# NoelShin/PixelPick

Hardware: AMD Instinct MI355X
Metric: train_step_throughput (higher is better)
Workload: dtype f32; 1 GPU; BASELINE configs[1]: Cityscapes 256x512, C=19, DeepLabv3+-MobileNetV2; train step per-GPU batch 4 with 20 labelled px/img + Adam; acquisition entropy top-k=20, B=256 images/launch/GPU, NCHW fp32 logits; global_batch=4

## Files before the change

### include/pixelpick_hip.h

```cpp
#ifndef PIXELPICK_HIP_H
#define PIXELPICK_HIP_H

#include <stddef.h>
#include <stdint.h>

#ifdef __cplusplus
extern "C" {
#endif

typedef void* pp_stream_t;

enum {
    PP_OK = 0,
    PP_ERR_BAD_ARG = -1,
    PP_ERR_BAD_K = -2,
    PP_ERR_WORKSPACE = -3,
    PP_ERR_UNSUPPORTED = -4,
    PP_ERR_LAUNCH = -5
};

enum { PP_ACQ_ENTROPY = 0, PP_ACQ_LEAST_CONFIDENCE = 1, PP_ACQ_MARGIN = 2 };
enum { PP_ACQ_BALD = 3 };
#define PP_ACQ_REFERENCE_ORDER 0x100

// ... 62 lines not shown
                               const uint8_t* exclude, int strategy, int64_t k,
                               int32_t* out_idx, float* out_val, float* out_map,
                               void* workspace, size_t ws_bytes, pp_stream_t stream);

int pp_acq_mean_prob_score_map(const float* prob, int64_t B, int64_t C, int64_t H, int64_t W,
                               int64_t sB, int64_t sC, int64_t sH, int64_t sW,
                               const float* mean_ent, const uint8_t* exclude, int strategy, float* out_map, pp_stream_t stream);

int pp_acq_lowres_mc_mean_topk(const float* low, int64_t ldx, int64_t B, int64_t T, int64_t C, int64_t h, int64_t w,
                               int64_t H, int64_t W, int align_corners, int64_t Hc, int64_t Wc,
                               const uint8_t* exclude, int strategy, float scale, int64_t k,
                               int32_t* out_idx, float* out_val, float* out_map,
                               void* workspace, size_t ws_bytes, pp_stream_t stream);

int pp_spread_select(const int32_t* cand, int64_t B, int64_t M, int64_t W, int64_t N, int64_t k, int64_t d,
                     const uint8_t* exclude, int32_t* out_idx, int32_t* out_pos, int32_t* out_n, pp_stream_t stream);

size_t pp_acq_region_table_words(int64_t r);
int pp_acq_region_table(int64_t r, uint32_t* host_tab);
int pp_acq_region_score_map(const uint8_t* pred, const float* unc, int64_t B, int64_t C, int64_t H, int64_t W, int64_t r, int mode,
                            int flip, const uint32_t* tab, const uint8_t* exclude, float* out_map, pp_stream_t stream);



size_t pp_conv2d_fwd_workspace_bytes(int B, int H, int W, int Cin, int Cout, int kh, int kw, int stride, int pad, int dil);
int pp_conv2d_fwd(const float* x, int64_t ldx, int B, int H, int W, int Cin, const float* w, const float* bias,
                  int kh, int kw, int stride, int pad, int dil, float* y, int64_t ldy, int Cout, void* workspace,
                  size_t ws_bytes, pp_stream_t stream);

int pp_bn_finalize_partials(const float* stats, int64_t rows, int64_t M, int C, const float* gamma, const float* beta, float eps,
                            float momentum, float* running_mean, float* running_var, float* mean, float* invstd, float* scale,
                            float* shift, pp_stream_t stream);
int64_t pp_dwconv3x3_fwd_stats_rows(int B, int H, int W, int C, int stride, int pad, int dil);
int pp_dwconv3x3_fwd_fused(const float* x, int64_t ldx, int B, int H, int W, int C, const float* w, int stride, int pad, int dil,
                           const float* in_scale, const float* in_shift, int in_act, float* y, int64_t ldy, float* stats,
                           size_t stats_floats, pp_stream_t stream);
int pp_dwconv3x3_bwd_weight_affine_in(const float* x_raw, int64_t ldx, int B, int H, int W, int C, const float* in_scale,
                                      const float* in_shift, int in_act, const float* dy, int64_t lddy, int stride, int pad, int dil,
                                      float* dw, void* workspace, size_t ws_bytes, pp_stream_t stream);
int pp_conv2d_fwd_accepts_affine_in(int B, int H, int W, int Cin, int Cout, int kh, int kw, int stride, int pad, int dil);
int pp_conv2d_fwd_affine_in(const float* x_raw, int64_t ldx, int B, int H, int W, int Cin, const float* in_scale, const float* in_shift,
                            int in_act, const float* w, const float* bias, int kh, int kw, int stride, int pad, int dil, float* y,
                            int64_t ldy, int Cout, void* workspace, size_t ws_bytes, pp_stream_t stream);

int pp_conv2d_fwd_bn_act(const float* x, int64_t ldx, int B, int H, int W, int Cin, const float* w, const float* bias,
                         int kh, int kw, int stride, int pad, int dil, const float* gamma, const float* beta,
                         const float* running_mean, const float* running_var, float eps, const float* residual,
                         int64_t ldr, int act, float* y, int64_t ldy, int Cout, void* workspace, size_t ws_bytes,
                         pp_stream_t stream);

size_t pp_conv2d_bwd_data_workspace_bytes(int B, int H, int W, int Cin, int Cout, int kh, int kw, int stride, int pad, int dil);
int pp_conv2d_bwd_data(const float* dy, int64_t lddy, int B, int Ho, int Wo, int Cout, const float* w, int kh, int kw,
                       int stride, int pad, int dil, float* dx, int64_t lddx, int H, int W, int Cin, int accumulate,
                       void* workspace, size_t ws_bytes, pp_stream_t stream);

size_t pp_conv2d_bwd_weight_workspace_bytes(int B, int H, int W, int Cin, int Cout, int kh, int kw, int stride, int pad, int dil);
int pp_conv2d_bwd_weight(const float* x, int64_t ldx, int B, int H, int W, int Cin, const float* dy, int64_t lddy,
                         int Cout, int kh, int kw, int stride, int pad, int dil, float* dw, float* dbias,
                         void* workspace, size_t ws_bytes, pp_stream_t stream);

size_t pp_conv2d_bwd_data_multi_workspace_bytes(int B, int H, int W, int Cin, int Cout, int nb, int k0, int d0, int k1, int d1, int k2, int d2,
                                                int k3, int d3);
int pp_conv2d_bwd_data_multi(const float* dy, int64_t lddy, int B, int H, int W, int Cout, int nb, const float* w0, int k0, int d0,
                             const float* w1, int k1, int d1, const float* w2, int k2, int d2, const float* w3, int k3, int d3, float* dx,
                             int64_t lddx, int Cin, int accumulate, void* workspace, size_t ws_bytes, pp_stream_t stream);

size_t pp_x3_planes_bytes(int64_t rows, int C);
int pp_x3_split(const float* x, int64_t ldx, int64_t rows, int C, void* planes, size_t planes_bytes, pp_stream_t stream);
size_t pp_conv2d_x3_planes_bytes(int which, int B, int H, int W, int Cin, int Cout, int kh, int kw, int stride, int pad, int dil);
int pp_conv2d_fwd_pre(const float* x, int64_t ldx, int B, int H, int W, int Cin, const float* w, const float* bias,
                      int kh, int kw, int stride, int pad, int dil, float* y, int64_t ldy, int Cout, void* workspace,
                      size_t ws_bytes, const void* x_planes, pp_stream_t stream);
int pp_conv2d_bwd_data_pre(const float* dy, int64_t lddy, int B, int Ho, int Wo, int Cout, const float* w, int kh, int kw,
                           int stride, int pad, int dil, float* dx, int64_t lddx, int H, int W, int Cin, int accumulate,
                           void* workspace, size_t ws_bytes, const void* dy_planes, pp_stream_t stream);
size_t pp_x3_weight_planes_bytes(int kh_kw, int Cin, int Cout, int transpose);
int pp_x3_split_weights(const float* w, int kh_kw, int Cin, int Cout, int transpose, void* planes, size_t planes_bytes, pp_stream_t stream);
int pp_conv2d_fwd_pre2(const float* x, int64_t ldx, int B, int H, int W, int Cin, const float* w, const float* bias,
                       int kh, int kw, int stride, int pad, int dil, float* y, int64_t ldy, int Cout, void* workspace,
                       size_t ws_bytes, const void* x_planes, const void* w_planes, pp_stream_t stream);
int pp_conv2d_bwd_data_pre2(const float* dy, int64_t lddy, int B, int Ho, int Wo, int Cout, const float* w, int kh, int kw,
                            int stride, int pad, int dil, float* dx, int64_t lddx, int H, int W, int Cin, int accumulate,
                            void* workspace, size_t ws_bytes, const void* dy_planes, const void* w_planes, pp_stream_t stream);
int pp_conv2d_bwd_weight_pre(const float* x, int64_t ldx, int B, int H, int W, int Cin, const float* dy, int64_t lddy,
                             int Cout, int kh, int kw, int stride, int pad, int dil, float* dw, float* dbias,
                             void* workspace, size_t ws_bytes, const void* x_planes, const void* dy_planes, pp_stream_t stream);

int pp_conv2d_fwd_bn_train_ok(int B, int H, int W, int Cin, int Cout, int kh, int kw, int stride, int pad, int dil);
size_t pp_conv2d_fwd_bn_train_xchg_bytes(int B, int H, int W, int Cin, int Cout, int kh, int kw, int stride, int pad, int dil);
int pp_conv2d_fwd_bn_train(const float* x, int64_t ldx, int B, int H, int W, int Cin, const float* w, int kh, int kw, int stride, int pad,
                           int dil, float* conv_out, int64_t ldc, const float* gamma, const float* beta, float eps, float momentum,
                           float* running_mean, float* running_var, float* mean, float* invstd, const float* residual, int64_t ldr,
                           int act, float* y, int64_t ldy, int Cout, void* xchg, size_t xchg_bytes, int32_t* sync, size_t sync_ints,
                           pp_stream_t stream);

int pp_conv2d_bwd_data_bn_bwd_ok(int B, int H, int W, int Cin, int Cout, int kh, int kw, int stride, int pad, int dil);
size_t pp_conv2d_bwd_data_bn_bwd_xchg_bytes(int B, int H, int W, int Cin, int Cout, int kh, int kw, int stride, int pad, int dil);
int pp_conv2d_bwd_data_bn_bwd(const float* dy, int64_t lddy, int B, int Ho, int Wo, int Cout, const float* w, int kh, int kw, int stride,
                              int pad, int dil, int H, int W, int Cin, const float* bn_x, int64_t ldbx, const float* mean,
                              const float* invstd, const float* gamma, const float* beta, int act, float* dgamma, float* dbeta,
                              float* dx_bn, int64_t lddx, const float* grad_in, int64_t ldgi, float* dres, int64_t lddr,
                              void* xchg, size_t xchg_bytes, int32_t* sync, size_t sync_ints, pp_stream_t stream);

typedef struct pp_reduce_job {
    const float* part;
    float* dst;
    int64_t cn;
    int32_t splits;
    int32_t ntaps;
    int32_t kind;
    uint8_t widx[12];
} pp_reduce_job;
int pp_conv2d_bwd_weight_partials(const float* x, int64_t ldx, int B, int H, int W, int Cin, const float* dy, int64_t lddy,
                                  int Cout, int kh, int kw, int stride, int pad, int dil, float* dw, float* dbias,
                                  void* workspace, size_t ws_bytes, pp_reduce_job* job, pp_stream_t stream);
int pp_dwconv3x3_bwd_weight_partials(const float* x, int64_t ldx, int B, int H, int W, int C, const float* dy, int64_t lddy,
                                     int stride, int pad, int dil, float* dw, void* workspace, size_t ws_bytes, pp_reduce_job* job,
                                     pp_stream_t stream);
int pp_wgrad_reduce_batch(const pp_reduce_job* jobs, int n, pp_stream_t stream);

size_t pp_colreduce_workspace_bytes(int64_t M, int C);

int pp_bn_train_fwd(const float* x, int64_t ldx, int64_t M, int C, const float* gamma, const float* beta, float eps,
                    float momentum, float* running_mean, float* running_var, float* mean, float* invstd, float* scale,
                    float* shift, void* workspace, size_t ws_bytes, pp_stream_t stream);

size_t pp_bn_fused_workspace_bytes(int64_t M, int C);
int pp_bn_fused_rows_cached(int64_t M, int C);
size_t pp_bn_fused_sync_ints(int C);
int pp_bn_train_fwd_fused(const float* x, int64_t ldx, int64_t M, int C, const float* gamma, const float* beta, float eps,
                          float momentum, float* running_mean, float* running_var, float* mean, float* invstd,
                          const float* residual, int64_t ldr, int act, float drop_p, uint64_t drop_seed,
                          const uint64_t* drop_seed_dev, float* y, int64_t ldy, void* workspace,
                          size_t ws_bytes, int32_t* sync, size_t sync_ints, pp_stream_t stream);

int64_t pp_conv2d_fwd_stats_rows(int B, int H, int W, int Cin, int Cout, int kh, int kw, int stride, int pad, int dil);
int pp_conv2d_fwd_stats(const float* x, int64_t ldx, int B, int H, int W, int Cin, const float* w, const float* bias,
                        int kh, int kw, int stride, int pad, int dil, float* y, int64_t ldy, int Cout, void* workspace,
                        size_t ws_bytes, float* stats, size_t stats_floats, pp_stream_t stream);
int pp_bn_train_fwd_partials(const float* x, int64_t ldx, int64_t M, int C, const float* stats, int64_t stat_rows, const float* gamma,
                             const float* beta, float eps, float momentum, float* running_mean, float* running_var, float* mean,
                             float* invstd, const float* residual, int64_t ldr, int act, float drop_p, uint64_t drop_seed,
                             const uint64_t* drop_seed_dev, float* y, int64_t ldy, pp_stream_t stream);

int pp_dwconv3x3_bn_train_fwd_fused(const float* in, int64_t ld_in, int B, int H, int W, int C, const float* w, int stride, int pad,
                                    int dil, float* x_out, int64_t ldx, const float* gamma, const float* beta, float eps,
                                    float momentum, float* running_mean, float* running_var, float* mean, float* invstd,
                                    const float* residual, int64_t ldr, int act, float* y, int64_t ldy, void* workspace,
                                    size_t ws_bytes, int32_t* sync, size_t sync_ints, pp_stream_t stream);

int pp_bn_bwd_fused(const float* x, int64_t ldx, const float* dy, int64_t lddy, const float* y_act, int64_t ldya, int act,
                    int64_t M, int C, const float* mean, const float* invstd, const float* gamma, float* dgamma,
                    float* dbeta, float* dx, int64_t lddx, float* dres, int64_t lddr, float grad_scale, const float* beta,
                    void* workspace, size_t ws_bytes, int32_t* sync, size_t sync_ints, pp_stream_t stream);

int pp_row_flags(const float* dy, int64_t lddy, int64_t M, int C, unsigned char* flags, pp_stream_t stream);
size_t pp_conv1x1_bwd_weight_sparse_workspace_bytes(int64_t M, int Cin, int Cout);
int pp_conv1x1_bwd_weight_sparse(const float* x, int64_t ldx, int64_t M, int Cin, const float* dy, int64_t lddy, int Cout,
                                 const unsigned char* row_flags, float* dw, float* dbias, void* workspace, size_t ws_bytes, pp_stream_t stream);
int pp_conv1x1_bwd_data_sparse(const float* dy, int64_t lddy, int64_t M, int Cout, const float* w, int Cin, const unsigned char* row_flags,
                             float* dx, int64_t lddx, pp_stream_t stream);
int pp_bn_bwd_fused_sparse(const float* x, int64_t ldx, const float* dy, int64_t lddy, const float* y_act, int64_t ldya, int act,
                         int64_t M, int C, const float* mean, const float* invstd, const float* gamma, float* dgamma,
                         float* dbeta, float* dx, int64_t lddx, float* dres, int64_t lddr, float grad_scale, const float* beta,
                         void* workspace, size_t ws_bytes, int32_t* sync, size_t sync_ints, const unsigned char* row_flags,
                         pp_stream_t stream);

int pp_bn_eval_affine(int C, const float* gamma, const float* beta, const float* running_mean, const float* running_var,
                      float eps, float* scale, float* shift, pp_stream_t stream);

int pp_scale_shift_act(const float* x, int64_t ldx, int64_t M, int C, const float* scale, const float* shift,
                       const float* residual, int64_t ldr, int act, float* y, int64_t ldy, pp_stream_t stream);

int pp_bn_bwd(const float* x, int64_t ldx, const float* dy, int64_t lddy, const float* y_act, int64_t ldya, int act,
              int64_t M, int C, const float* mean, const float* invstd, const float* gamma, float* dgamma, float* dbeta,
              float* dx, int64_t lddx, float* dres, int64_t lddr, void* workspace, size_t ws_bytes, pp_stream_t stream);

int pp_dwconv3x3_fwd(const float* x, int64_t ldx, int B, int H, int W, int C, const float* w, int stride, int pad, int dil,
                     float* y, int64_t ldy, pp_stream_t stream);

int pp_dwconv3x3_fwd_bn_act(const float* x, int64_t ldx, int B, int H, int W, int C, const float* w, int stride, int pad,
                            int dil, const float* gamma, const float* beta, const float* running_mean,
                            const float* running_var, float eps, const float* residual, int64_t ldr, int act, float* y,
                            int64_t ldy, pp_stream_t stream);
int pp_dwconv3x3_bwd_data(const float* dy, int64_t lddy, int B, int H, int W, int C, const float* w, int stride, int pad,
                          int dil, float* dx, int64_t lddx, pp_stream_t stream);
int pp_dwconv3x3_bwd_weight(const float* x, int64_t ldx, int B, int H, int W, int C, const float* dy, int64_t lddy,
                            int stride, int pad, int dil, float* dw, void* workspace, size_t ws_bytes, pp_stream_t stream);

size_t pp_groupnorm_workspace_bytes(int B, int64_t P, int C);
int pp_groupnorm_relu_fwd(const float* x, int64_t ldx, int B, int64_t P, int C, int G, const float* gamma, const float* beta,
                          float eps, int relu, float* y, int64_t ldy, float* mean, float* rstd, void* workspace,
                          size_t ws_bytes, pp_stream_t stream);
int pp_groupnorm_relu_bwd(const float* x, int64_t ldx, const float* dy, int64_t lddy, const float* y, int64_t ldy, int B,
                          int64_t P, int C, int G, const float* mean, const float* rstd, const float* gamma, float* dgamma,
                          float* dbeta, float* dx, int64_t lddx, void* workspace, size_t ws_bytes, pp_stream_t stream);

int pp_maxpool2d_fwd(const float* x, int64_t ldx, int B, int H, int W, int C, int ksize, int stride, int pad, float* y,
                     int64_t ldy, unsigned char* argmax, pp_stream_t stream);
int pp_maxpool2d_bwd(const float* dy, int64_t lddy, const unsigned char* argmax, int B, int H, int W, int C, int ksize, int stride,
                     int pad, float* dx, int64_t lddx, pp_stream_t stream);

int pp_pad2d(const float* x, int64_t ldx, int B, int H, int W, int C, int pad_top, int pad_left, int Hp, int Wp, float* y,
             int64_t ldy, pp_stream_t stream);
int pp_crop2d_add(const float* xp, int64_t ldxp, int B, int Hp, int Wp, int C, int pad_top, int pad_left, const float* add,
                  int64_t ldadd, float* y, int64_t ldy, int H, int W, pp_stream_t stream);

int pp_bilinear_fwd(const float* x, int64_t ldx, int B, int H, int W, int C, float* y, int64_t ldy, int Ho, int Wo,
                    int align_corners, float scale_h, float scale_w, int out_nchw, pp_stream_t stream);
size_t pp_bilinear_bwd_workspace_bytes(int B, int Ho, int W, int C);
int pp_bilinear_bwd(const float* dy, int64_t lddy, int B, int Ho, int Wo, int C, float* dx, int64_t lddx, int H, int W,
                    int align_corners, float scale_h, float scale_w, int dy_nchw, void* workspace, size_t ws_bytes,
                    pp_stream_t stream);

int pp_image_colsum(const float* x, int64_t ldx, int B, int64_t P, int C, float mul, float* out, int64_t ldo, pp_stream_t stream);
int pp_image_broadcast(const float* v, int64_t ldv, int B, int64_t P, int C, float mul, float* y, int64_t ldy, pp_stream_t stream);

int pp_dropout(const float* x, int64_t ldx, float* y, int64_t ldy, int64_t M, int C, float p, uint64_t seed,
               const uint64_t* seed_dev, pp_stream_t stream);

int pp_aug_resample_h(const uint8_t* src, int H, int W, const int32_t* bounds, const int32_t* kk, int ksize, int Wout, uint8_t* dst,
                      pp_stream_t stream);
int pp_aug_vcrop(const uint8_t* tmp, const int32_t* bounds, const int32_t* kk, int ksize, int h_rs, int w_rs, int start_h, int start_w,
                 int ch, int cw, int flip, int fill_r, int fill_g, int fill_b, uint8_t* out, pp_stream_t stream);
int pp_aug_labels(const uint8_t* y, const uint8_t* q, int W, const int32_t* ty, const int32_t* tx, const int32_t* qy, const int32_t* qx,
                  int h_rs, int w_rs, int start_h, int start_w, int ch, int cw, int flip, int ignore_index, int64_t* y_out,
                  uint8_t* q_out, pp_stream_t stream);
int pp_aug_jitter(uint8_t* img, int64_t n_pixels, int op, float factor, unsigned long long* scratch_sum, pp_stream_t stream);
int pp_aug_blur(uint8_t* img, int H, int W, const float* kernel, int ks, float* scratch, pp_stream_t stream);
int pp_aug_blur_q8(uint8_t* img, int H, int W, const uint16_t* kernel_q8, int ks, uint16_t* scratch, pp_stream_t stream);
int pp_aug_to_tensor(const uint8_t* img, int64_t n_pixels, const float* mean3, const float* std3, float* out, pp_stream_t stream);

int pp_dropout2d(const float* x, int64_t ldx, float* y, int64_t ldy, int B, int64_t P, int C, float p, uint64_t seed,
                 const uint64_t* seed_dev, pp_stream_t stream);

size_t pp_sparse_ce_workspace_bytes(void);
int pp_sparse_ce_fwd_bwd(const float* logits, int B, int C, int64_t HW, int64_t sB, int64_t sC, const int64_t* target,
                         int ignore_index, float* loss, float* count, const float* grad_out, float* dlogits, void* workspace,
                         size_t ws_bytes, pp_stream_t stream);

size_t pp_sparse_ce_lowres_workspace_bytes(void);
int pp_sparse_ce_lowres_fwd_bwd(const float* low, int64_t ldx, int B, int C, int h, int w, int H, int W, int align_corners,
                                const int64_t* target, int ignore_index, float* loss, float* count, const float* grad_out,
                                float* dlow, int64_t lddx, void* workspace, size_t ws_bytes, pp_stream_t stream);

int pp_confusion_matrix_update(const float* logits, int B, int C, int64_t HW, int64_t sB, int64_t sC, const int64_t* target,
                               int64_t* hist, pp_stream_t stream);

int pp_confusion_matrix_from_labels(const uint8_t* pred, const void* target, int target_kind, int64_t n, int C, int64_t* hist,
                                    pp_stream_t stream);

int pp_predict_lowres(const float* low, int64_t ldx, int64_t B, int64_t C, int64_t h, int64_t w, int64_t H, int64_t W,
                      int align_corners, int64_t Hc, int64_t Wc, const void* target, int target_kind, uint8_t* pred,
                      int64_t* hist, pp_stream_t stream);

size_t pp_vis_lowres_workspace_bytes(int64_t B, int64_t Hc, int64_t Wc);
int pp_vis_lowres(const float* low, int64_t ldx, int64_t B, int64_t C, int64_t h, int64_t w, int64_t H, int64_t W,
                  int align_corners, int64_t Hc, int64_t Wc, const float* image, int64_t image_sn, int64_t image_sc,
                  int64_t image_sr, const void* target, int target_kind, const uint8_t* palette, uint8_t* rgb, uint8_t* gray,
                  float* ranges, void* workspace, size_t ws_bytes, pp_stream_t stream);

int pp_adam_step_flat(float* params, const float* grads, float* exp_avg, float* exp_avg_sq, int64_t n, int64_t n_split,
                      float lr_a, float lr_b, float beta1, float beta2, float eps, float weight_decay, int64_t step,
                      float grad_scale, const float* hyper_dev, pp_stream_t stream);

int pp_sgd_step_flat(float* params, const float* grads, float* momentum_buf, int64_t n, int64_t n_split, float lr_a, float lr_b,
                     float momentum, float weight_decay, int64_t step, float grad_scale, const float* hyper_dev,
                     pp_stream_t stream);

int pp_add2d(const float* a, int64_t lda, const float* b, int64_t ldb, float* y, int64_t ldy, int64_t M, int C, pp_stream_t stream);

int pp_nchw_to_nhwc(const float* x, int B, int C, int64_t HW, float* y, int64_t ldy, pp_stream_t stream);
int pp_nhwc_to_nchw(const float* x, int64_t ldx, int B, int C, int64_t HW, float* y, pp_stream_t stream);

int pp_bn_fused_capacity(void);
int pp_yardstick_stream_read(const void* x, size_t bytes, int blocks, float* sink, pp_stream_t stream);
int pp_yardstick_mfma_stream(int data_kind, int iters, float* sink, pp_stream_t stream);

#ifdef PP_DEBUG_KNOBS
#include "pixelpick_hip_knobs.h"
#endif

typedef void* pp_plan_t;
pp_plan_t pp_plan_create(void);
void pp_plan_destroy(pp_plan_t plan);
int64_t pp_plan_size(pp_plan_t plan);
int pp_plan_entry_args(const void* fn);
int pp_plan_add_call(pp_plan_t plan, const void* fn, const uint64_t* slots, int n_slots);
int pp_plan_add_event_record(pp_plan_t plan, void* event, pp_stream_t stream);
int pp_plan_add_stream_wait(pp_plan_t plan, pp_stream_t stream, void* event);
int pp_plan_add_join(pp_plan_t plan, pp_stream_t waiting, pp_stream_t waited_for);
int pp_plan_add_host_break(pp_plan_t plan);
int pp_plan_replay(pp_plan_t plan, int64_t from, int64_t* next);

void pp_set_comm_cu_reserve(int cus);
int pp_get_comm_cu_reserve(void);
void pp_set_kernel_events(void** starts, void** stops, int n);
// ... 6 lines not shown
```

### pixelpick_amd/_lib.py

```python
import ctypes
import os
import struct

import torch

_HERE = os.path.dirname(os.path.abspath(__file__))
LIB_PATH = os.path.join(_HERE, "libpixelpick_hip.so")
KNOBS_LIB_PATH = os.path.join(_HERE, "libpixelpick_hip_knobs.so")
_use_knobs = [os.environ.get("PIXELPICK_KNOBS_BUILD", "0") not in ("", "0")]


def use_knobs_build(on: bool = True):
    if _lib is not None and _use_knobs[0] != bool(on):
        raise PixelPickHipError("use_knobs_build() after the library was loaded")
    _use_knobs[0] = bool(on)


def knobs_build() -> bool:
    return _use_knobs[0]

_i64, _p, _int, _sz, _f = ctypes.c_int64, ctypes.c_void_p, ctypes.c_int, ctypes.c_size_t, ctypes.c_float
_u64 = ctypes.c_uint64

SIGNATURES = {
    "pp_version": (_int, []),
    "pp_last_error": (ctypes.c_char_p, []),
    "pp_acq_workspace_bytes": (_sz, [_i64] * 5),
    "pp_acq_score_topk": (_int, [_p] + [_i64] * 8 + [_p, _int, _i64, _p, _p, _p, _p, _sz, _p]),
    "pp_acq_score_map": (_int, [_p] + [_i64] * 8 + [_p, _int, _p, _p]),
    "pp_acq_softmax_sum": (_int, [_p] + [_i64] * 8 + [_p, _p, _int, _f, _int, _p]),
    "pp_uncertainty_from_prob": (_int, [_p] + [_i64] * 8 + [_int, _p, _p]),
    "pp_topk_workspace_bytes": (_sz, [_i64] * 3),
    "pp_topk_select": (_int, [_p, _i64, _i64, _i64, _int, _p, _p, _p, _sz, _p]),
    "pp_acq_lowres_workspace_bytes": (_sz, [_i64] * 5),
    "pp_acq_lowres_score_topk": (_int, [_p] + [_i64] * 7 + [_int, _i64, _i64, _p, _int, _i64, _p, _p, _p, _p, _sz, _p]),
    "pp_acq_lowres_score_at": (_int, [_p] + [_i64] * 7 + [_int, _i64, _i64, _int, _p, _p, _i64, _p, _p]),
    "pp_acq_lowres_mc_score_topk": (_int, [_p] + [_i64] * 8 + [_int, _i64, _i64, _p, _int, _f, _i64, _p, _p, _p, _p, _sz, _p]),
    "pp_acq_lowres_mc_score_at": (_int, [_p] + [_i64] * 8 + [_int, _i64, _i64, _int, _f, _p, _p, _i64, _p, _p]),
    "pp_acq_vote_accumulate": (_int, [_p] + [_i64] * 8 + [_p, _int, _p]),
    "pp_acq_vote_score_map": (_int, [_p] + [_i64] * 5 + [_p, _int, _p, _p]),
    "pp_acq_lowres_mc_vote_topk": (_int, [_p] + [_i64] * 8 + [_int, _i64, _i64, _p, _int, _i64, _p, _p, _p, _p, _sz, _p]),
    "pp_acq_mean_prob_score_map": (_int, [_p] + [_i64] * 8 + [_p, _p, _int, _p, _p]),
    "pp_acq_lowres_mc_mean_topk": (_int, [_p] + [_i64] * 8 + [_int, _i64, _i64, _p, _int, _f, _i64, _p, _p, _p, _p, _sz, _p]),
    "pp_spread_select": (_int, [_p] + [_i64] * 6 + [_p, _p, _p, _p, _p]),
    "pp_acq_region_table_words": (_sz, [_i64]),
    "pp_acq_region_table": (_int, [_i64, _p]),
    "pp_acq_region_score_map": (_int, [_p, _p] + [_i64] * 5 + [_int, _int, _p, _p, _p, _p]),
    "pp_conv2d_fwd_workspace_bytes": (_sz, [_int] * 10),
    "pp_conv2d_bwd_data_workspace_bytes": (_sz, [_int] * 10),
    "pp_conv2d_fwd": (_int, [_p, _i64, _int, _int, _int, _int, _p, _p, _int, _int, _int, _int, _int, _p, _i64, _int, _p, _sz, _p]),
    "pp_conv2d_fwd_stats_rows": (_i64, [_int] * 10),
    "pp_conv2d_fwd_stats": (_int, [_p, _i64, _int, _int, _int, _int, _p, _p, _int, _int, _int, _int, _int, _p, _i64, _int, _p, _sz, _p, _sz, _p]),
    "pp_bn_train_fwd_partials": (_int, [_p, _i64, _i64, _int, _p, _i64, _p, _p, _f, _f, _p, _p, _p, _p, _p, _i64, _int, _f, _u64, _p, _p, _i64, _p]),
    "pp_conv2d_fwd_bn_act": (_int, [_p, _i64, _int, _int, _int, _int, _p, _p, _int, _int, _int, _int, _int, _p, _p, _p, _p, _f, _p, _i64, _int,
                                    _p, _i64, _int, _p, _sz, _p]),
    "pp_dwconv3x3_fwd_bn_act": (_int, [_p, _i64, _int, _int, _int, _int, _p, _int, _int, _int, _p, _p, _p, _p, _f, _p, _i64, _int, _p, _i64, _p]),
    "pp_bn_finalize_partials": (_int, [_p, _i64, _i64, _int, _p, _p, _f, _f, _p, _p, _p, _p, _p, _p, _p]),
    "pp_dwconv3x3_fwd_stats_rows": (_i64, [_int] * 7),
    "pp_dwconv3x3_fwd_fused": (_int, [_p, _i64, _int, _int, _int, _int, _p, _int, _int, _int, _p, _p, _int, _p, _i64, _p, _sz, _p]),
    "pp_dwconv3x3_bwd_weight_affine_in": (_int, [_p, _i64, _int, _int, _int, _int, _p, _p, _int, _p, _i64, _int, _int, _int, _p, _p, _sz, _p]),
    "pp_conv2d_fwd_accepts_affine_in": (_int, [_int] * 10),
    "pp_conv2d_fwd_affine_in": (_int, [_p, _i64, _int, _int, _int, _int, _p, _p, _int, _p, _p, _int, _int, _int, _int, _int, _p, _i64, _int, _p, _sz, _p]),
    "pp_conv2d_bwd_data": (_int, [_p, _i64, _int, _int, _int, _int, _p, _int, _int, _int, _int, _int, _p, _i64, _int, _int, _int, _int, _p, _sz, _p]),
    "pp_conv2d_bwd_weight_workspace_bytes": (_sz, [_int] * 10),
    "pp_conv2d_bwd_weight": (_int, [_p, _i64, _int, _int, _int, _int, _p, _i64, _int, _int, _int, _int, _int, _int, _p, _p, _p, _sz, _p]),
    "pp_conv2d_fwd_bn_train_ok": (_int, [_int] * 10),
    "pp_conv2d_fwd_bn_train_xchg_bytes": (_sz, [_int] * 10),
    "pp_conv2d_fwd_bn_train": (_int, [_p, _i64, _int, _int, _int, _int, _p, _int, _int, _int, _int, _int, _p, _i64, _p, _p, _f, _f, _p, _p, _p, _p,
                                      _p, _i64, _int, _p, _i64, _int, _p, _sz, _p, _sz, _p]),
    "pp_conv2d_bwd_data_bn_bwd_ok": (_int, [_int] * 10),
    "pp_conv2d_bwd_data_bn_bwd_xchg_bytes": (_sz, [_int] * 10),
    "pp_conv2d_bwd_data_bn_bwd": (_int, [_p, _i64, _int, _int, _int, _int, _p, _int, _int, _int, _int, _int, _int, _int, _int, _p, _i64, _p, _p, _p, _p,
                                         _int, _p, _p, _p, _i64, _p, _i64, _p, _i64, _p, _sz, _p, _sz, _p]),
    "pp_x3_planes_bytes": (_sz, [_i64, _int]),
    "pp_x3_split": (_int, [_p, _i64, _i64, _int, _p, _sz, _p]),
    "pp_conv2d_x3_planes_bytes": (_sz, [_int] * 11),
    "pp_conv2d_fwd_pre": (_int, [_p, _i64, _int, _int, _int, _int, _p, _p, _int, _int, _int, _int, _int, _p, _i64, _int, _p, _sz, _p, _p]),
    "pp_conv2d_bwd_data_multi_workspace_bytes": (_sz, [_int] * 14),
    "pp_conv2d_bwd_data_multi": (_int, [_p, _i64, _int, _int, _int, _int, _int, _p, _int, _int, _p, _int, _int, _p, _int, _int, _p, _int, _int,
                                       _p, _i64, _int, _int, _p, _sz, _p]),
    "pp_conv2d_bwd_data_pre": (_int, [_p, _i64, _int, _int, _int, _int, _p, _int, _int, _int, _int, _int, _p, _i64, _int, _int, _int, _int, _p, _sz, _p, _p]),
    "pp_x3_weight_planes_bytes": (_sz, [_int, _int, _int, _int]),
    "pp_x3_split_weights": (_int, [_p, _int, _int, _int, _int, _p, _sz, _p]),
    "pp_conv2d_fwd_pre2": (_int, [_p, _i64, _int, _int, _int, _int, _p, _p, _int, _int, _int, _int, _int, _p, _i64, _int, _p, _sz, _p, _p, _p]),
    "pp_conv2d_bwd_data_pre2": (_int, [_p, _i64, _int, _int, _int, _int, _p, _int, _int, _int, _int, _int, _p, _i64, _int, _int, _int, _int, _p, _sz, _p, _p, _p]),
    "pp_conv2d_bwd_weight_pre": (_int, [_p, _i64, _int, _int, _int, _int, _p, _i64, _int, _int, _int, _int, _int, _int, _p, _p, _p, _sz, _p, _p, _p]),
    "pp_conv2d_bwd_weight_partials": (_int, [_p, _i64, _int, _int, _int, _int, _p, _i64, _int, _int, _int, _int, _int, _int, _p, _p, _p, _sz, _p, _p]),
    "pp_wgrad_reduce_batch": (_int, [_p, _int, _p]),
    "pp_colreduce_workspace_bytes": (_sz, [_i64, _int]),
    "pp_bn_train_fwd": (_int, [_p, _i64, _i64, _int, _p, _p, _f, _f, _p, _p, _p, _p, _p, _p, _p, _sz, _p]),
    "pp_bn_eval_affine": (_int, [_int, _p, _p, _p, _p, _f, _p, _p, _p]),
    "pp_scale_shift_act": (_int, [_p, _i64, _i64, _int, _p, _p, _p, _i64, _int, _p, _i64, _p]),
    "pp_bn_bwd": (_int, [_p, _i64, _p, _i64, _p, _i64, _int, _i64, _int, _p, _p, _p, _p, _p, _p, _i64, _p, _i64, _p, _sz, _p]),
    "pp_bn_fused_workspace_bytes": (_sz, [_i64, _int]),
    "pp_bn_fused_sync_ints": (_sz, [_int]),
    "pp_bn_fused_rows_cached": (_int, [_i64, _int]),
    "pp_bn_train_fwd_fused": (_int, [_p, _i64, _i64, _int, _p, _p, _f, _f, _p, _p, _p, _p, _p, _i64, _int, _f, _u64, _p, _p, _i64, _p, _sz, _p, _sz, _p]),
    "pp_dwconv3x3_bn_train_fwd_fused": (_int, [_p, _i64, _int, _int, _int, _int, _p, _int, _int, _int, _p, _i64, _p, _p, _f, _f, _p, _p, _p, _p,
                                               _p, _i64, _int, _p, _i64, _p, _sz, _p, _sz, _p]),
    "pp_bn_bwd_fused": (_int, [_p, _i64, _p, _i64, _p, _i64, _int, _i64, _int, _p, _p, _p, _p, _p, _p, _i64, _p, _i64, _f, _p, _p, _sz, _p, _sz, _p]),
    "pp_bn_bwd_fused_sparse": (_int, [_p, _i64, _p, _i64, _p, _i64, _int, _i64, _int, _p, _p, _p, _p, _p, _p, _i64, _p, _i64, _f, _p, _p, _sz, _p, _sz, _p, _p]),
    "pp_row_flags": (_int, [_p, _i64, _i64, _int, _p, _p]),
    "pp_conv1x1_bwd_weight_sparse_workspace_bytes": (_sz, [_i64, _int, _int]),
    "pp_conv1x1_bwd_weight_sparse": (_int, [_p, _i64, _i64, _int, _p, _i64, _int, _p, _p, _p, _p, _sz, _p]),
    "pp_conv1x1_bwd_data_sparse": (_int, [_p, _i64, _i64, _int, _p, _int, _p, _p, _i64, _p]),
    "pp_dwconv3x3_fwd": (_int, [_p, _i64, _int, _int, _int, _int, _p, _int, _int, _int, _p, _i64, _p]),
    "pp_dwconv3x3_bwd_data": (_int, [_p, _i64, _int, _int, _int, _int, _p, _int, _int, _int, _p, _i64, _p]),
    "pp_dwconv3x3_bwd_weight": (_int, [_p, _i64, _int, _int, _int, _int, _p, _i64, _int, _int, _int, _p, _p, _sz, _p]),
    "pp_dwconv3x3_bwd_weight_partials": (_int, [_p, _i64, _int, _int, _int, _int, _p, _i64, _int, _int, _int, _p, _p, _sz, _p, _p]),
    "pp_groupnorm_workspace_bytes": (_sz, [_int, _i64, _int]),
    "pp_groupnorm_relu_fwd": (_int, [_p, _i64, _int, _i64, _int, _int, _p, _p, _f, _int, _p, _i64, _p, _p, _p, _sz, _p]),
    "pp_groupnorm_relu_bwd": (_int, [_p, _i64, _p, _i64, _p, _i64, _int, _i64, _int, _int, _p, _p, _p, _p, _p, _p, _i64, _p, _sz, _p]),
    "pp_maxpool2d_fwd": (_int, [_p, _i64, _int, _int, _int, _int, _int, _int, _int, _p, _i64, _p, _p]),
    "pp_maxpool2d_bwd": (_int, [_p, _i64, _p, _int, _int, _int, _int, _int, _int, _int, _p, _i64, _p]),
    "pp_pad2d": (_int, [_p, _i64, _int, _int, _int, _int, _int, _int, _int, _int, _p, _i64, _p]),
    "pp_crop2d_add": (_int, [_p, _i64, _int, _int, _int, _int, _int, _int, _p, _i64, _p, _i64, _int, _int, _p]),
    "pp_bilinear_fwd": (_int, [_p, _i64, _int, _int, _int, _int, _p, _i64, _int, _int, _int, _f, _f, _int, _p]),
    "pp_bilinear_bwd_workspace_bytes": (_sz, [_int] * 4),
    "pp_bilinear_bwd": (_int, [_p, _i64, _int, _int, _int, _int, _p, _i64, _int, _int, _int, _f, _f, _int, _p, _sz, _p]),
    "pp_image_colsum": (_int, [_p, _i64, _int, _i64, _int, _f, _p, _i64, _p]),
    "pp_image_broadcast": (_int, [_p, _i64, _int, _i64, _int, _f, _p, _i64, _p]),
    "pp_dropout": (_int, [_p, _i64, _p, _i64, _i64, _int, _f, ctypes.c_uint64, _p, _p]),
    "pp_dropout2d": (_int, [_p, _i64, _p, _i64, _int, _i64, _int, _f, ctypes.c_uint64, _p, _p]),
    "pp_aug_resample_h": (_int, [_p, _int, _int, _p, _p, _int, _int, _p, _p]),
    "pp_aug_vcrop": (_int, [_p, _p, _p] + [_int] * 11 + [_p, _p]),
    "pp_aug_labels": (_int, [_p, _p, _int, _p, _p, _p, _p] + [_int] * 8 + [_p, _p, _p]),
    "pp_aug_jitter": (_int, [_p, _i64, _int, _f, _p, _p]),
    "pp_aug_blur": (_int, [_p, _int, _int, _p, _int, _p, _p]),
    "pp_aug_blur_q8": (_int, [_p, _int, _int, _p, _int, _p, _p]),
    "pp_aug_to_tensor": (_int, [_p, _i64, ctypes.POINTER(_f), ctypes.POINTER(_f), _p, _p]),
    "pp_sparse_ce_workspace_bytes": (_sz, []),
    "pp_sparse_ce_fwd_bwd": (_int, [_p, _int, _int, _i64, _i64, _i64, _p, _int, _p, _p, _p, _p, _p, _sz, _p]),
    "pp_sparse_ce_lowres_workspace_bytes": (_sz, []),
    "pp_sparse_ce_lowres_fwd_bwd": (_int, [_p, _i64] + [_int] * 7 + [_p, _int, _p, _p, _p, _p, _i64, _p, _sz, _p]),
    "pp_confusion_matrix_update": (_int, [_p, _int, _int, _i64, _i64, _i64, _p, _p, _p]),
    "pp_predict_lowres": (_int, [_p] + [_i64] * 7 + [_int, _i64, _i64, _p, _int, _p, _p, _p]),
    "pp_confusion_matrix_from_labels": (_int, [_p, _p, _int, _i64, _int, _p, _p]),
    "pp_vis_lowres_workspace_bytes": (_sz, [_i64] * 3),
    "pp_vis_lowres": (_int, [_p] + [_i64] * 7 + [_int, _i64, _i64, _p, _i64, _i64, _i64, _p, _int, _p, _p, _p, _p, _p, _sz, _p]),
    "pp_adam_step_flat": (_int, [_p, _p, _p, _p, _i64, _i64, _f, _f, _f, _f, _f, _f, _i64, _f, _p, _p]),
    "pp_sgd_step_flat": (_int, [_p, _p, _p, _i64, _i64, _f, _f, _f, _f, _i64, _f, _p, _p]),
    "pp_add2d": (_int, [_p, _i64, _p, _i64, _p, _i64, _i64, _int, _p]),
    "pp_nhwc_to_nchw": (_int, [_p, _i64, _int, _int, _i64, _p, _p]),
    "pp_nchw_to_nhwc": (_int, [_p, _int, _int, _i64, _p, _i64, _p]),
    "pp_bn_fused_capacity": (_int, []),
    "pp_yardstick_stream_read": (_int, [_p, _sz, _int, _p, _p]),
    "pp_yardstick_mfma_stream": (_int, [_int, _int, _p, _p]),
    "pp_set_kernel_events": (None, [_p, _p, _int]),
    "pp_set_comm_cu_reserve": (None, [_int]),
    "pp_get_comm_cu_reserve": (_int, []),
    "pp_plan_create": (_p, []),
    "pp_plan_destroy": (None, [_p]),
    "pp_plan_size": (_i64, [_p]),
    "pp_plan_entry_args": (_int, [_p]),
    "pp_plan_add_call": (_int, [_p, _p, _p, _int]),
    "pp_plan_add_event_record": (_int, [_p, _p, _p]),
    "pp_plan_add_stream_wait": (_int, [_p, _p, _p]),
    "pp_plan_add_join": (_int, [_p, _p, _p]),
    "pp_plan_add_host_break": (_int, [_p]),
    "pp_plan_replay": (_int, [_p, _i64, ctypes.POINTER(_i64)]),
}

KNOB_SIGNATURES = {
    "pp_debug_set_reduce_mode": (None, [_int]),
    "pp_debug_set_exact_formula": (None, [_int]),
    "pp_debug_set_acq_tuning": (None, [_int, _int]),
    "pp_debug_set_dw_variant": (None, [_int]),
    "pp_debug_set_splitk": (None, [_int]),
    "pp_debug_set_wgrad_target": (None, [_int]),
    "pp_debug_set_bn_target": (None, [_int]),
    "pp_debug_set_bn_bytes_per_block": (None, [_int]),
    "pp_debug_set_bn_probe": (None, [_p]),
    "pp_debug_set_lsel_probe": (None, [_p]),
    "pp_debug_set_conv_thresholds": (None, [_int]),
    "pp_debug_conv_plan": (None, [_i64, _int, _int, _int, _p]),
    "pp_debug_set_conv_variant": (None, [_int]),
    "pp_debug_set_ce_stream": (None, [_int]),
    "pp_debug_set_conv_rows": (None, [_int]),
    "pp_debug_set_conv_bn_fuse": (None, [_int]),
    "pp_debug_set_x3": (None, [_int]),
    "pp_debug_set_x3f": (None, [_int]),
    "pp_debug_set_gemm_pw": (None, [_int]),
    "pp_debug_set_x3_variant": (None, [_int]),
    "pp_debug_occupy_cus": (_int, [_int, _p, _u64, _p, _p]),
    "pp_debug_launch_log": (_int, [ctypes.c_char_p, _int]),
}

_lib = None
knob_epoch = [0]


def _knob_setter(fn):
    def setter(*args):
        knob_epoch[0] += 1
        return fn(*args)
    setter.__name__ = getattr(fn, "__name__", "pp_debug_set")
    setter.__wrapped__ = fn
    return setter


class PixelPickHipError(RuntimeError):
    pass
# ... 284 lines not shown
```

### pixelpick_amd/csrc/conv_igemm.hip

```cpp
#include <atomic>
#include <type_traits>

#include "pp_common.h"
#include "bn_xchg.h"
#include "conv_types.h"

namespace pp {


static int g_conv_xcd_remap = 1;
static int g_conv_novec = 0;
static int g_conv_lds_pad = 0;
static int g_conv_variant = 0;

typedef float f32x16s __attribute__((ext_vector_type(16)));
constexpr int BK = 16;
struct __attribute__((packed, aligned(4))) StemF4 { float x, y, z, w; };
struct __attribute__((packed, aligned(4))) StemF3 { float x, y, z; };
struct __attribute__((packed, aligned(4))) StemF2 { float x, y; };


template <int TM, int TN, bool A_MK, bool B_NK, int PITCH_A, int PITCH_B, int BKT = BK>
__device__ __forceinline__ void mma_step(const float* As, const float* Bs, int a_row0, int b_col0, f32x16 (&acc)[TM][TN])
{
// ... 3108 lines not shown
            pl.splits = (int)cdiv(nk, pl.ks_per_split);
        }
    }
    return pl;
}

static bool ksplit_shape_ok(int64_t M, int Cn, int Ck, int ntaps, int stride)
{
    return g_conv_ksplit && ntaps == 1 && stride == 1 && M <= g_direct_rows_max && Ck >= g_ksplit_k_min && Cn >= 32 && Cn <= 512 &&
           Ck % 4 == 0 && Cn % 4 == 0;
}

static int64_t splitk_stats_rows_per_block(int64_t M) { return M >= 8192 ? 64 : 16; }

static int64_t conv_stats_rows(const ConvPlan& pl, int64_t M, int Cn)
{
    if (pl.splits > 1) {
        if (Cn % 4 != 0 || Cn / 4 > 256) return 0;
        return cdiv(M, splitk_stats_rows_per_block(M));
    }
    if (pl.cfg == 0) return cdiv(M, 128) * 4;
    if (pl.cfg == 1 || pl.cfg == 4) return cdiv(M, 128) * 2;
    return cdiv(M, 64) * 2;
}

static int g_conv_x3 = 1;
static int g_x3_var = 0;
struct X3Plan { bool ok, classic, f32; int Kp; int64_t rows_a, a_plane, b_rows, b_plane; size_t bytes, b_off; };
static int g_conv_x3_mid = 1;
static double g_x3_mid_flop = 16e9, g_x3w_flop = 8e9;
static int g_x3_mid_tiles = 256;
static int g_x3f = 0;
static double g_x3f_flop = 1e9;
static int g_x3f_tiles = 128, g_x3f_k = 256;
static X3Plan x3_plan(const ConvPlan& pl, int64_t M, int64_t rows_a, int Ck, int n_rows, int ntaps_w, int ntaps_live, bool vec)
{
    X3Plan x{};
    const int64_t t128 = cdiv(M, 128) * cdiv(n_rows, 128);
    const double flop = 2.0 * (double)M * n_rows * ntaps_live * Ck;
    const bool mid = g_conv_x3_mid && pl.cfg == 2 && t128 >= g_x3_mid_tiles && flop >= g_x3_mid_flop;
    if (!g_conv_x3 || !vec || ntaps_live > 32) return x;
    x.classic = (pl.cfg == 1 || mid) && pl.splits <= 1 && (int64_t)ntaps_live * Ck >= 512;
    const int64_t t64 = n_rows % 64 == 0 ? cdiv(M, 128) * (n_rows / 64) : 0;
    x.f32 = g_x3f && n_rows >= 64 && (x.classic || (flop >= g_x3f_flop && (int64_t)ntaps_live * Ck >= g_x3f_k &&
                                                    std::max(t128, t64) >= g_x3f_tiles && (pl.cfg == 1 || pl.cfg == 2 || pl.cfg == 3 || pl.cfg == 4)));
    if (!x.classic && !x.f32) return x;
    x.Kp = (int)cdiv(Ck, 16) * 16;
    x.rows_a = rows_a;
    x.a_plane = (rows_a + 1) * x.Kp;
    x.b_rows = (int64_t)ntaps_w * n_rows;
    x.b_plane = (x.b_rows + 1) * x.Kp;
    if (x.b_plane * 2 >= (1ll << 32) - 4096) { x.classic = x.f32 = false; return x; }
    if (x.a_plane * 2 >= (1ll << 32) - 4096) x.classic = false;
    if (!x.classic && !x.f32) return x;
    x.b_off = x.classic ? align_up((size_t)3 * x.a_plane * 2, 256) : 0;
    x.bytes = x.b_off + align_up((size_t)3 * x.b_plane * 2, 256);
    x.ok = true;
    return x;
}

static int g_gemm_pw = 1;
static int64_t g_gemm_pw_rows_min = 4096;
static int device_cus();
static int gemm_pw_choose(int64_t M, int N, int K)
{
    if (!g_gemm_pw || K < 64 || N < 64) return -1;
    if (g_gemm_pw >= 2) return M >= g_gemm_pw_rows_min ? g_gemm_pw - 2 : -1;
    if (M < g_gemm_pw_rows_min) return -1;
    static const double eff[6] = {0.88, 0.86, 0.85, 0.80, 0.78, 0.70}, fixed_us[6] = {10.0, 10.5, 6.0, 4.5, 4.5, 2.5};
    const int cus = device_cus();
    int best = -1;
    double best_t = 1e30;
    for (int f = 0; f < 6; ++f) {
        const int bm = gemm_pw_tile_rows(f), bn = gemm_pw_tile_cols(f);
        const int64_t tiles = cdiv(M, bm) * cdiv(N, bn);
        const double tile_us = 2.0 * bm * bn * (double)K / (4 * 64 * 2.4e3) / eff[f] + fixed_us[f];
        const double t = (double)cdiv(tiles, cus) * tile_us;
        if (t < best_t) { best_t = t; best = f; }
    }
    return best;
}

template <bool BWD>
static int launch_conv_x3(ConvParams& p, const ConvPlan& pl, const X3Plan& x, int kh_kw, void* workspace, hipStream_t st, bool f32path)
{
    const uint16_t* ap = p.a_pre ? p.a_pre : reinterpret_cast<uint16_t*>(workspace);
    uint16_t* bp = reinterpret_cast<uint16_t*>(reinterpret_cast<char*>(workspace) + x.b_off);
    if (!p.a_pre && !f32path) {
        const int64_t ta = (x.rows_a + 1) * (x.Kp / 8);
        hipLaunchKernelGGL(x3_split_kernel, dim3((unsigned)std::min<int64_t>(cdiv(ta, 256), 4096)), dim3(256), 0, st, p.x, p.ldx, x.rows_a, p.Ck,
                           reinterpret_cast<uint16_t*>(workspace), x.Kp, x.a_plane);
        if (int rc = check_launch("x3_split_kernel")) return rc;
    }
    if (p.b_pre) {
        bp = const_cast<uint16_t*>(p.b_pre);
    } else {
        const int64_t tb = (x.b_rows + 1) * (x.Kp / 8);
        hipLaunchKernelGGL(x3_split_w_kernel, dim3((unsigned)std::min<int64_t>(cdiv(tb, 256), 4096)), dim3(256), 0, st, p.w, kh_kw, p.Cin, p.Cout,
                           BWD ? 0 : 1, bp, x.Kp, x.b_plane);
        if (int rc = check_launch("x3_split_w_kernel")) return rc;
    }
    X3Operands o{ap, bp, x.a_plane, x.b_plane, x.Kp, p.Cn, (uint32_t)(x.rows_a * 32), (uint32_t)(x.b_rows * 32),
                 (uint32_t)((x.rows_a + 1) * 32), (uint32_t)((x.b_rows + 1) * 32), 0};
    p.n_tiles = pl.n_tiles;
    p.splits = 1;
    p.ks_per_split = 0;
    p.part = nullptr;
    const int full128 = p.Cn / 128, rem = p.Cn - full128 * 128;
    const bool two = rem > 0 && rem <= 64 && full128 > 0 && !(g_conv_x3 & 4);
    bool n128_only = !two && (rem == 0 || rem > 64 || (g_conv_x3 & 4));
    const int64_t mt256 = cdiv(p.M, 256);
    if (f32path && n128_only && rem == 0 && cdiv(p.M, 128) * full128 < 200 && cdiv(p.M, 128) * full128 * 2 >= 128) n128_only = false;
    auto go = [&](bool n128, int ntile, int col_base) {
        const bool m256 = !(g_conv_x3 & 2) && mt256 * ntile >= 200;
        const int64_t mtiles = m256 ? mt256 : cdiv(p.M, 128);
        o.col_base = col_base;
        p.n_tiles = ntile;
        const dim3 grid((unsigned)(mtiles * ntile));
#ifdef PP_DEBUG_KNOBS
        if (f32path) {
            (void)launch_conv_x3f(p, o, m256, n128, grid.x, st);
            return;
        }
#endif
        if (m256) {
            if (n128) {
                switch (g_x3_var) {
#ifdef PP_DEBUG_KNOBS
                    case 1: hipLaunchKernelGGL((conv_x3_kernel<256, 128, 1>), grid, dim3(512), 0, st, p, o); break;
                    case 2: hipLaunchKernelGGL((conv_x3_kernel<256, 128, 2>), grid, dim3(512), 0, st, p, o); break;
                    case 3: hipLaunchKernelGGL((conv_x3_kernel<256, 128, 3>), grid, dim3(512), 0, st, p, o); break;
                    case 4: hipLaunchKernelGGL((conv_x3_kernel<256, 128, 4>), grid, dim3(512), 0, st, p, o); break;
                    case 5: hipLaunchKernelGGL((conv_x3_kernel<256, 128, 5>), grid, dim3(512), 0, st, p, o); break;
                    case 6: hipLaunchKernelGGL((conv_x3_kernel<256, 128, 6>), grid, dim3(512), 0, st, p, o); break;
                    case 7: hipLaunchKernelGGL((conv_x3_kernel<256, 128, 7>), grid, dim3(512), 0, st, p, o); break;
                    case 8: hipLaunchKernelGGL((conv_x3_kernel<256, 128, 8>), grid, dim3(512), 0, st, p, o); break;
                    case 9: hipLaunchKernelGGL((conv_x3_kernel<256, 128, 9>), grid, dim3(512), 0, st, p, o); break;
                    case 10: hipLaunchKernelGGL((conv_x3_kernel<256, 128, 10>), grid, dim3(512), 0, st, p, o); break;
                    case 11: hipLaunchKernelGGL((conv_x3_kernel<256, 128, 11>), grid, dim3(512), 0, st, p, o); break;
#endif
                    default: hipLaunchKernelGGL((conv_x3_kernel<256, 128>), grid, dim3(512), 0, st, p, o);
                }
            } else hipLaunchKernelGGL((conv_x3_kernel<256, 64>), grid, dim3(512), 0, st, p, o);
        } else {
            if (n128) hipLaunchKernelGGL((conv_x3_kernel<128, 128>), grid, dim3(256), 0, st, p, o);
            else      hipLaunchKernelGGL((conv_x3_kernel<128, 64>), grid, dim3(256), 0, st, p, o);
        }
    };
    if (two) {
        go(true, full128, 0);
        if (int rc = check_launch("conv_x3_kernel")) return rc;
        go(false, 1, full128 * 128);
    } else {
        go(n128_only, (int)cdiv(p.Cn, n128_only ? 128 : 64), 0);
    }
    return check_launch("conv_x3_kernel");
}

static int device_cus();
static int conv_bn_capacity(int which = 0)
{
    static const int cap[3] = {
        [] { int n = 0; if (hipOccupancyMaxActiveBlocksPerMultiprocessor(&n, conv_igemm_dma_kernel<64, 64, false, true>, kThreads, 0) != hipSuccess) { (void)hipGetLastError(); return 0; } return n * device_cus(); }(),
        [] { int n = 0; if (hipOccupancyMaxActiveBlocksPerMultiprocessor(&n, conv_igemm_dma_kernel<128, 64, false, true>, kThreads, 0) != hipSuccess) { (void)hipGetLastError(); return 0; } return n * device_cus(); }(),
        [] { int n = 0; if (hipOccupancyMaxActiveBlocksPerMultiprocessor(&n, conv_igemm_kernel<128, 32, 4, 1, false, true>, kThreads, 0) != hipSuccess) { (void)hipGetLastError(); return 0; } return n * device_cus(); }()};
    return reserve_scaled(cap[which], device_cus());
}
static int g_conv_bn_fuse = 15;
static int ksplit_bn_capacity(int which)
{
    static const int cap[2] = {
        [] { int n = 0; if (hipOccupancyMaxActiveBlocksPerMultiprocessor(&n, conv1x1_ksplit_dma_kernel<1, 1, 5, false>, kThreads, 0) != hipSuccess) { (void)hipGetLastError(); return 0; } return n * device_cus(); }(),
        [] { int n = 0; if (hipOccupancyMaxActiveBlocksPerMultiprocessor(&n, conv1x1_ksplit_dma_kernel<2, 1, 3, false>, kThreads, 0) != hipSuccess) { (void)hipGetLastError(); return 0; } return n * device_cus(); }()};
    return reserve_scaled(cap[which], device_cus());
}
struct BnFusePlan { int kind; int R; int64_t blocks; KsplitCfg kc; };
static BnFusePlan bn_fuse_plan(const ConvParams& p, const ConvPlan& pl, bool vec)
{
    BnFusePlan f{0, 0, 0, {0, 0, 0}};
    if (!g_conv_bn_fuse || !vec || p.stats || p.in_scale || p.bias || p.epi.gamma || p.epi.res || p.epi.act != 0 || p.accumulate || p.bwd_stride > 1 ||
        p.Cn % 32 != 0 || (int64_t)p.B * p.H * p.W * p.ldx >= (1ll << 31) - (1ll << 24))
        return f;
    const bool ksplit = ksplit_shape_ok(p.M, p.Cn, p.Ck, p.taps.n, p.stride) && p.Cout % 4 == 0 && (int64_t)p.Cin * p.Cout < (1ll << 31) - (1ll << 24);
    if (ksplit) {
        if (!(g_conv_bn_fuse & 2)) return f;
        const KsplitCfg kc = ksplit_choose(p.M, p.Cn, false, g_conv_ksplit - 1);
        if (kc.tn != 1) return f;
        const int64_t blocks = cdiv(p.M, 32 * kc.tm) * cdiv(p.Cn, 32);
        if (blocks > ksplit_bn_capacity(kc.tm == 2 ? 1 : 0) / 2) return f;
        f.kind = 2; f.R = (int)cdiv(p.M, 32 * kc.tm); f.blocks = blocks; f.kc = kc;
        return f;
    }
    const bool dma_ok = g_conv_dma64 && p.taps.n <= 32 && (int64_t)kMaxTaps * p.Cin * p.Cout < (1ll << 31);
    if (!(g_conv_bn_fuse & 1) || pl.splits != 1) return f;
    if (pl.cfg == 2 && dma_ok && pl.tiles <= conv_bn_capacity() / 2) {
        f.kind = 1; f.R = (int)cdiv(p.M, 64); f.blocks = pl.tiles;
    } else if (pl.cfg == 2 && dma_ok && g_conv_dma && cdiv(p.M, 128) * cdiv(p.Cn, 64) <= conv_bn_capacity(1) / 2) {
        f.kind = 3; f.R = (int)cdiv(p.M, 128); f.blocks = cdiv(p.M, 128) * cdiv(p.Cn, 64);
    } else if (pl.cfg == 0 && p.Cn == 32 && pl.tiles <= conv_bn_capacity(2) / 2) {
        f.kind = 4; f.R = (int)cdiv(p.M, 128); f.blocks = pl.tiles;
    }
    return f;
}

static int conv_bn_bwd_capacity(int which = 0)
{
    static const int cap[2] = {
        [] { int n = 0; if (hipOccupancyMaxActiveBlocksPerMultiprocessor(&n, conv_igemm_dma_kernel<64, 64, true, true>, kThreads, 0) != hipSuccess) { (void)hipGetLastError(); return 0; } return n * device_cus(); }(),
        [] { int n = 0; if (hipOccupancyMaxActiveBlocksPerMultiprocessor(&n, conv_igemm_kernel<128, 32, 4, 1, true, true>, kThreads, 0) != hipSuccess) { (void)hipGetLastError(); return 0; } return n * device_cus(); }()};
    return reserve_scaled(cap[which], device_cus());
}
static int ksplit_bn_bwd_capacity(int which)
{
    static const int cap[2] = {
        [] { int n = 0; if (hipOccupancyMaxActiveBlocksPerMultiprocessor(&n, conv1x1_ksplit_dma_kernel<1, 1, 5, true>, kThreads, 0) != hipSuccess) { (void)hipGetLastError(); return 0; } return n * device_cus(); }(),
        [] { int n = 0; if (hipOccupancyMaxActiveBlocksPerMultiprocessor(&n, conv1x1_ksplit_dma_kernel<1, 2, 3, true>, kThreads, 0) != hipSuccess) { (void)hipGetLastError(); return 0; } return n * device_cus(); }()};
    return reserve_scaled(cap[which], device_cus());
}
static BnFusePlan bn_fuse_plan_bwd(const ConvParams& p, const ConvPlan& pl, bool vec)
{
    BnFusePlan f{0, 0, 0, {0, 0, 0}};
    if (!(g_conv_bn_fuse & 4) || !vec || p.stats || p.in_scale || p.bias || p.epi.gamma || p.epi.res || p.epi.act != 0 || p.accumulate || p.bwd_stride > 1 ||
        p.stride != 1 || p.Cn % 32 != 0 || (int64_t)p.B * p.H * p.W * p.ldx >= (1ll << 31) - (1ll << 24))
        return f;
    const bool ks_wide = g_conv_ksplit && (g_conv_bn_fuse & 8) && p.taps.n == 1 && p.M <= 2 * (int64_t)g_direct_rows_max && p.Ck >= 128 &&
                         p.Cn >= 32 && p.Cn <= 512 && p.Ck % 4 == 0;
    const bool ks_plain = ksplit_shape_ok(p.M, p.Cn, p.Ck, p.taps.n, p.stride);
    if (ks_plain || ks_wide) {
        const KsplitCfg kc = ksplit_choose(p.M, p.Cn, true, g_conv_ksplit - 1);
        const int64_t blocks = cdiv(p.M, 32) * cdiv(p.Cn, 32 * kc.tn);
        const bool ok = (g_conv_bn_fuse & 8) && p.Cout % 4 == 0 && (int64_t)p.Cin * p.Cout < (1ll << 31) - (1ll << 24) && kc.tm == 1 &&
                        blocks <= ksplit_bn_bwd_capacity(kc.tn == 2 ? 1 : 0) / 2;
        if (ok) { f.kind = 2; f.R = (int)cdiv(p.M, 32); f.blocks = blocks; f.kc = kc; return f; }
        if (ks_plain) return f;
    }
    const bool dma_ok = g_conv_dma64 == 1 && p.taps.n <= 32 && (int64_t)kMaxTaps * p.Cin * p.Cout < (1ll << 31);
    if (pl.cfg == 2 && (pl.splits == 1 || (g_conv_bn_fuse & 8)) && dma_ok && pl.tiles <= conv_bn_bwd_capacity() / 2) {
        f.kind = 1; f.R = (int)cdiv(p.M, 64); f.blocks = pl.tiles;
    } else if (pl.cfg == 0 && p.Cn == 32 && (g_conv_bn_fuse & 8) && pl.tiles <= conv_bn_bwd_capacity(1) / 2) {
        f.kind = 4; f.R = (int)cdiv(p.M, 128); f.blocks = pl.tiles;
    }
    return f;
}

template <bool BWD>
static int launch_conv(const ConvParams& p_in, void* workspace, size_t ws_bytes, hipStream_t st, int kh_kw = 0)
{
    EventScope ev(st);
    ConvParams p = p_in;
    p.xcd_remap = g_conv_xcd_remap;
    const bool vec = g_conv_novec == 0 && p.Ck % 4 == 0 && p.Cin % 4 == 0 && p.Cout % 4 == 0 && p.ldx % 4 == 0 &&
                     (reinterpret_cast<uintptr_t>(p.x) & 15) == 0 && (reinterpret_cast<uintptr_t>(p.w) & 15) == 0;
    ConvPlan pl = plan_conv(p.M, p.Cn, p.Ck, p.taps.n, vec);
    if (p.bn.part) {
        const BnFusePlan f = BWD ? bn_fuse_plan_bwd(p, pl, vec) : bn_fuse_plan(p, pl, vec);
        if (f.kind == 0) return fail(PP_ERR_UNSUPPORTED, "conv + BatchNorm: this shape has no fused kernel");
        p.bn.R = f.R;
        p.splits = 1; p.ks_per_split = 0; p.part = nullptr;
        if constexpr (BWD) {
            if (f.kind == 2) {
                p.n_tiles = (int)cdiv(p.Cn, 32 * f.kc.tn);
                if (f.kc.tn == 2) hipLaunchKernelGGL((conv1x1_ksplit_dma_kernel<1, 2, 3, true>), dim3((unsigned)f.blocks), dim3(kThreads), 0, st, p);
                else              hipLaunchKernelGGL((conv1x1_ksplit_dma_kernel<1, 1, 5, true>), dim3((unsigned)f.blocks), dim3(kThreads), 0, st, p);
                return check_launch("conv1x1_ksplit_dma_kernel<bn bwd>");
            }
            p.tap_inner = g_conv_tap_inner;
            p.n_tiles = pl.n_tiles;
            if (f.kind == 4) {
                hipLaunchKernelGGL((conv_igemm_kernel<128, 32, 4, 1, true, true>), dim3((unsigned)pl.tiles), dim3(kThreads), 0, st, p);
                return check_launch("conv_igemm_kernel<bn bwd>");
            }
            hipLaunchKernelGGL((conv_igemm_dma_kernel<64, 64, true, true>), dim3((unsigned)pl.tiles), dim3(kThreads), 0, st, p);
            return check_launch("conv_igemm_dma_kernel<bn bwd>");
        }
        if constexpr (!BWD) {
            if (f.kind == 2) {
                p.n_tiles = (int)cdiv(p.Cn, 32);
                if (f.kc.tm == 2) hipLaunchKernelGGL((conv1x1_ksplit_dma_kernel<2, 1, 3, false>), dim3((unsigned)f.blocks), dim3(kThreads), 0, st, p);
                else              hipLaunchKernelGGL((conv1x1_ksplit_dma_kernel<1, 1, 5, false>), dim3((unsigned)f.blocks), dim3(kThreads), 0, st, p);
                return check_launch("conv1x1_ksplit_dma_kernel<bn>");
            }
            p.tap_inner = g_conv_tap_inner;
            if (f.kind == 3) {
                p.n_tiles = (int)cdiv(p.Cn, 64);
                hipLaunchKernelGGL((conv_igemm_dma_kernel<128, 64, false, true>), dim3((unsigned)f.blocks), dim3(kThreads), 0, st, p);
            } else if (f.kind == 4) {
                p.n_tiles = pl.n_tiles;
                hipLaunchKernelGGL((conv_igemm_kernel<128, 32, 4, 1, false, true>), dim3((unsigned)pl.tiles), dim3(kThreads), 0, st, p);
            } else {
                p.n_tiles = pl.n_tiles;
                hipLaunchKernelGGL((conv_igemm_dma_kernel<64, 64, false, true>), dim3((unsigned)pl.tiles), dim3(kThreads), 0, st, p);
            }
        }
        return check_launch("conv_igemm_kernel<bn>");
    }
    if (kh_kw > 0 && !p.in_scale && p.bwd_stride <= 1) {
        const X3Plan x = x3_plan(pl, p.M, (int64_t)p.B * p.H * p.W, p.Ck, p.Cn, kh_kw, p.taps.n, vec);
#ifdef PP_DEBUG_KNOBS
        const bool f32path = x.f32 && !p.a_pre && conv_x3f_supported(p);
#else
        const bool f32path = false;
#endif
        const bool ws_ok = (workspace && ws_bytes >= x.bytes && (reinterpret_cast<uintptr_t>(workspace) & 255) == 0) ||
                           (f32path && p.b_pre != nullptr);
        if (x.ok && (f32path || x.classic) && ws_ok && (reinterpret_cast<uintptr_t>(p.b_pre) & 255) == 0)
            return launch_conv_x3<BWD>(p, pl, x, kh_kw, workspace, st, f32path);
    }
    if (pl.splits > 1 && (!workspace || ws_bytes < (size_t)pl.splits * p.M * p.Cn * 4)) {
        pl.splits = 1;
    }
    {
        const bool pw = p.taps.n == 1 && p.taps.dh[0] == 0 && p.taps.dw[0] == 0 && p.stride == 1 && vec && !p.stats && !p.in_scale && !p.epi.gamma &&
                        !p.epi.res && p.epi.act == 0 && !p.bn.part && p.bwd_stride <= 1 && !p.multi;
        if (pw) {
            const bool bt_ok = !BWD || g_gemm_pw >= 2 || (p.Ck >= 512 && 2 * p.Ck >= p.Cn) || p.Cn <= 128;
            const int form = bt_ok ? gemm_pw_choose(p.M, p.Cn, p.Ck) : -1;
            const float* w1 = p.w + (int64_t)p.taps.widx[0] * p.Cin * p.Cout;
            if (form >= 0 && gemm_pw_supported(p.x, p.ldx, w1, p.Cout, p.y, p.ldy, p.M, p.Cn, p.Ck))
                return launch_gemm_pw(p.x, p.ldx, w1, p.Cout, p.bias, p.y, p.ldy, p.M, p.Cn, p.Ck, p.accumulate, form, g_conv_xcd_remap, st, BWD ? 1 : 0);
        }
    }
    const bool use_ksplit = ksplit_shape_ok(p.M, p.Cn, p.Ck, p.taps.n, p.stride) && vec && !p.stats && p.bwd_stride <= 1 && p.Cout % 4 == 0 &&
                            p.ldx % 4 == 0 && (int64_t)p.B * p.H * p.W * p.ldx < (1ll << 31) - (1ll << 24) &&
                            (int64_t)p.Cin * p.Cout < (1ll << 31) - (1ll << 24) && !(p.in_scale && p.Ck > 2048);
    if (p.in_scale) {
        const bool pad0 = p.taps.n == 1 && p.taps.dh[0] == 0 && p.taps.dw[0] == 0 && p.stride == 1;
        if (BWD || !pad0 || !(use_ksplit || (pl.cfg == 0 && vec)))
            return fail(PP_ERR_UNSUPPORTED, "conv fwd: this shape has no input-affine kernel (ask pp_conv2d_fwd_accepts_affine_in first)");
    }
    if constexpr (!BWD) {
        const bool stem = g_conv_bwd_rows && p.Cin == 3 && p.Cout == 32 && p.Cn == 32 && kh_kw == 9 && p.taps.n == 9 && p.stride == 2 &&
                          p.taps.dh[0] == -1 && p.taps.dw[0] == -1 && p.taps.dh[8] == 1 && p.taps.dw[8] == 1 && p.W % 2 == 0 && p.H % 2 == 0 &&
                          p.Wo * 2 == p.W && p.Ho * 2 == p.H && p.ldx == 3 && !p.bias && !p.stats && !p.in_scale && !p.epi.gamma && !p.epi.res &&
                          p.epi.act == 0 && !p.accumulate && p.ldy % 4 == 0 && (reinterpret_cast<uintptr_t>(p.y) & 15) == 0 && p.M >= 16384 &&
                          (int64_t)p.B * p.H * p.W * 3 < (1ll << 31);
        if (stem) {
            hipLaunchKernelGGL(conv_stem3x3s2_fwd_kernel, dim3((unsigned)cdiv(p.M, 64)), dim3(256), 0, st, p);
            return check_launch("conv_stem3x3s2_fwd_kernel");
        }
    }
    {
        const bool plain = g_conv_bwd_rows && vec && p.taps.n == 1 && p.stride == 1 && p.bwd_stride <= 1 && !p.stats && !p.in_scale && !p.bias &&
                           !p.epi.gamma && !p.epi.res && p.epi.act == 0 && p.M >= 16384 && p.ldy % 4 == 0 &&
                           (reinterpret_cast<uintptr_t>(p.y) & 15) == 0 && (int64_t)p.B * p.H * p.W * p.ldx < (1ll << 31);
        const bool rows_ok = plain && (p.Cn == 16 || p.Cn == 24 || p.Cn == 32) && p.Ck <= 192 && p.Ck >= 16 && (BWD || p.M >= g_rows_fwd_min);
        if (rows_ok) {
            const size_t lds = (size_t)(64 * (p.Ck + 4) + 64 * p.Cn) * 4;
            const dim3 grid((unsigned)cdiv(p.M, 64));
            const unsigned inv_kq = (1u << 20) / (unsigned)(p.Ck / 4) + 1u;
#define PP_ROWS(CN_) do { if (p.Ck <= 96) hipLaunchKernelGGL((conv1x1_rows_kernel<CN_, 6, BWD>), grid, dim3(256), lds, st, p, inv_kq); \
                          else if (p.Ck <= 144) hipLaunchKernelGGL((conv1x1_rows_kernel<CN_, 9, BWD>), grid, dim3(256), lds, st, p, inv_kq); \
                          else hipLaunchKernelGGL((conv1x1_rows_kernel<CN_, 12, BWD>), grid, dim3(256), lds, st, p, inv_kq); } while (0)
            if (p.Cn == 16)      PP_ROWS(16);
            else if (p.Cn == 24) PP_ROWS(24);
            else                 PP_ROWS(32);
#undef PP_ROWS
            return check_launch("conv1x1_rows_kernel");
        }
        if constexpr (BWD) {
            const bool widen = plain && p.Cout == p.Ck && p.Ck == 24 && (p.Cn == 96 || p.Cn == 144);
            if (widen) {
                const dim3 grid((unsigned)cdiv(p.M, 64));
                if (p.Cn == 96) hipLaunchKernelGGL((conv1x1_fwd_widen_kernel<24, 96, true>), grid, dim3(256), 0, st, p);
                else            hipLaunchKernelGGL((conv1x1_fwd_widen_kernel<24, 144, true>), grid, dim3(256), 0, st, p);
                return check_launch("conv1x1_fwd_widen_kernel<bwd>");
            }
        }
        if constexpr (!BWD) {
            const bool widen = plain && !p.accumulate && ((p.Ck == 16 && p.Cn == 96) || (p.Ck == 24 && p.Cn == 144) || (p.Ck == 32 && p.Cn == 192));
            if (widen) {
                const dim3 grid((unsigned)cdiv(p.M, 64));
                if (p.Ck == 16)      hipLaunchKernelGGL((conv1x1_fwd_widen_kernel<16, 96>), grid, dim3(256), 0, st, p);
                else if (p.Ck == 24) hipLaunchKernelGGL((conv1x1_fwd_widen_kernel<24, 144>), grid, dim3(256), 0, st, p);
                else                 hipLaunchKernelGGL((conv1x1_fwd_widen_kernel<32, 192>), grid, dim3(256), 0, st, p);
                return check_launch("conv1x1_fwd_widen_kernel");
            }
        }
    }
    if (use_ksplit) {
        const KsplitCfg kc = ksplit_choose(p.M, p.Cn, BWD, g_conv_ksplit - 1);
        p.splits = 1;
        p.ks_per_split = 0;
        p.part = nullptr;
        p.n_tiles = (int)cdiv(p.Cn, 32 * kc.tn);
        const dim3 grid((unsigned)(cdiv(p.M, 32 * kc.tm) * p.n_tiles));
#define PP_KSPLIT(TM_, TN_, NST_) hipLaunchKernelGGL((conv1x1_ksplit_dma_kernel<TM_, TN_, NST_, BWD>), grid, dim3(kThreads), 0, st, p)
#define PP_KSPLIT_AFF(TM_, TN_, NST_) hipLaunchKernelGGL((conv1x1_ksplit_dma_kernel<TM_, TN_, NST_, false, true>), grid, dim3(kThreads), 0, st, p)
        if (!BWD && p.in_scale) {
            if (kc.tm == 1 && kc.tn == 1) PP_KSPLIT_AFF(1, 1, 4);
            else if (kc.tm == 2)          PP_KSPLIT_AFF(2, 1, 3);
// ... 597 lines not shown
    EventScope ev(st);
    const int64_t tb = (rows + 1) * (Kp / 8);
    hipLaunchKernelGGL(x3_split_w_kernel, dim3((unsigned)std::min<int64_t>(cdiv(tb, 256), 4096)), dim3(256), 0, st, w, kh_kw, Cin, Cout, transpose ? 1 : 0,
                       reinterpret_cast<uint16_t*>(planes), Kp, plane);
    return check_launch("x3_split_w_kernel");
}

int pp_conv2d_fwd_pre2(const float* x, int64_t ldx, int B, int H, int W, int Cin, const float* w, const float* bias,
                       int kh, int kw, int stride, int pad, int dil, float* y, int64_t ldy, int Cout, void* workspace,
                       size_t ws_bytes, const void* x_planes, const void* w_planes, pp_stream_t stream)
{
    return conv2d_fwd_impl(x, ldx, B, H, W, Cin, w, bias, kh, kw, stride, pad, dil, y, ldy, Cout, Epilogue{}, workspace,
                           ws_bytes, stream, nullptr, 0, nullptr, nullptr, 0, x_planes, w_planes);
}

static bool conv_bn_shape(ConvParams& p, ConvPlan& pl, int B, int H, int W, int Cin, int Cout, int kh, int kw, int stride, int pad, int dil,
                          int64_t ldx, int* R_out = nullptr)
{
    if (B < 1 || H < 1 || W < 1 || Cin < 1 || Cout < 1 || kh < 1 || kw < 1 || kh > kMaxTaps || kw > kMaxTaps || kh * kw > kMaxTaps || !conv_geom_sane(H, W, stride, pad, dil) || stride < 1 || dil < 1) return false;
    const int Ho = out_size(H, kh, stride, pad, dil), Wo = out_size(W, kw, stride, pad, dil);
    if (Ho < 1 || Wo < 1) return false;
    p = ConvParams{};
    p.ldx = ldx; p.B = B; p.H = H; p.W = W; p.Ho = Ho; p.Wo = Wo; p.Ck = Cin; p.Cn = Cout; p.Cin = Cin; p.Cout = Cout;
    p.stride = stride; p.M = (int64_t)B * Ho * Wo; p.bwd_stride = 1;
    build_taps(p.taps, kh, kw, stride, pad, dil, H, W, Ho, Wo, false);
    if (p.M > 0x7FFFFFFFll || p.taps.n == 0) return false;
    const bool vec = Cin % 4 == 0 && Cout % 4 == 0 && ldx % 4 == 0;
    pl = plan_conv(p.M, Cout, Cin, p.taps.n, vec);
    const BnFusePlan f = bn_fuse_plan(p, pl, vec);
    if (R_out) *R_out = f.R;
    return f.kind != 0;
}

int pp_conv2d_fwd_bn_train_ok(int B, int H, int W, int Cin, int Cout, int kh, int kw, int stride, int pad, int dil)
{
    ConvParams p; ConvPlan pl;
    return conv_bn_shape(p, pl, B, H, W, Cin, Cout, kh, kw, stride, pad, dil, Cin) ? 1 : 0;
}

size_t pp_conv2d_fwd_bn_train_xchg_bytes(int B, int H, int W, int Cin, int Cout, int kh, int kw, int stride, int pad, int dil)
{
    ConvParams p; ConvPlan pl;
    int R = 0;
    if (!conv_bn_shape(p, pl, B, H, W, Cin, Cout, kh, kw, stride, pad, dil, Cin, &R)) return 0;
    return align_up((size_t)cdiv(Cout, 32) * (size_t)R * 64 * 8, 256);
}

int pp_conv2d_fwd_bn_train(const float* x, int64_t ldx, int B, int H, int W, int Cin, const float* w, int kh, int kw, int stride, int pad,
                           int dil, float* conv_out, int64_t ldc, const float* gamma, const float* beta, float eps, float momentum,
                           float* running_mean, float* running_var, float* mean, float* invstd, const float* residual, int64_t ldr,
                           int act, float* y, int64_t ldy, int Cout, void* xchg, size_t xchg_bytes, int32_t* sync, size_t sync_ints,
                           pp_stream_t stream)
{
    if (int rc = conv_common_check(x, w, conv_out, B, H, W, Cin, Cout, kh, kw, stride, pad, dil)) return rc;
    if (!gamma || !beta || !mean || !invstd || !y || !xchg || !sync) return fail(PP_ERR_BAD_ARG, "conv fwd + BatchNorm: null");
    if (act < 0 || act > 2) return fail(PP_ERR_BAD_ARG, "conv fwd + BatchNorm: act %d", act);
    if ((reinterpret_cast<uintptr_t>(xchg) & 7) != 0 || sync_ints < 2) return fail(PP_ERR_BAD_ARG, "conv fwd + BatchNorm: exchange area");
    ConvParams p; ConvPlan pl;
    int R = 0;
    if (!conv_bn_shape(p, pl, B, H, W, Cin, Cout, kh, kw, stride, pad, dil, ldx, &R))
        return fail(PP_ERR_UNSUPPORTED, "conv fwd + BatchNorm: this shape has no fused kernel (ask pp_conv2d_fwd_bn_train_ok first)");
    const size_t need = (size_t)cdiv(Cout, 32) * (size_t)R * 64 * 8;
    if (xchg_bytes < need) return fail(PP_ERR_WORKSPACE, "conv fwd + BatchNorm: exchange area %zu < %zu", xchg_bytes, need);
    p.x = x; p.w = w; p.bias = nullptr; p.y = conv_out; p.ldy = ldc;
    p.bn = BnTrain{gamma, beta, eps, momentum, running_mean, running_var, mean, invstd, residual, ldr, act, y, ldy,
                   reinterpret_cast<xword*>(xchg), sync, 0};
    return launch_conv<false>(p, nullptr, 0, as_stream(stream), kh * kw);
}

int pp_conv2d_fwd_bn_act(const float* x, int64_t ldx, int B, int H, int W, int Cin, const float* w, const float* bias,
                         int kh, int kw, int stride, int pad, int dil, const float* gamma, const float* beta,
                         const float* running_mean, const float* running_var, float eps, const float* residual,
                         int64_t ldr, int act, float* y, int64_t ldy, int Cout, void* workspace, size_t ws_bytes,
                         pp_stream_t stream)
{
    if (gamma && (!beta || !running_mean || !running_var)) return fail(PP_ERR_BAD_ARG, "conv fwd_bn_act: incomplete BatchNorm");
    if (act < 0 || act > 2) return fail(PP_ERR_BAD_ARG, "conv fwd_bn_act: act %d", act);
    Epilogue e{gamma, beta, running_mean, running_var, eps, residual, ldr, act};
    return conv2d_fwd_impl(x, ldx, B, H, W, Cin, w, bias, kh, kw, stride, pad, dil, y, ldy, Cout, e, workspace, ws_bytes, stream);
}

static int conv2d_bwd_data_impl(const float* dy, int64_t lddy, int B, int Ho, int Wo, int Cout, const float* w, int kh, int kw,
                                int stride, int pad, int dil, float* dx, int64_t lddx, int H, int W, int Cin, int accumulate,
                                void* workspace, size_t ws_bytes, pp_stream_t stream, const void* dy_planes, const void* w_planes = nullptr)
{
    if (int rc = conv_common_check(dy, w, dx, B, H, W, Cin, Cout, kh, kw, stride, pad, dil)) return rc;
    if (Ho != out_size(H, kh, stride, pad, dil) || Wo != out_size(W, kw, stride, pad, dil))
        return fail(PP_ERR_BAD_ARG, "conv bwd_data: inconsistent sizes");
    if (bwd_phases_apply(Cin, Cout, stride, lddx) && (int64_t)B * H * W <= 0x7FFFFFFFll) {
        size_t slab_bytes = 0;
        const size_t need = bwd_phases_workspace(B, H, W, Cin, Cout, kh, kw, stride, pad, dil, Ho, Wo, &slab_bytes);
        if (workspace && ws_bytes >= need && (reinterpret_cast<uintptr_t>(workspace) & 15) == 0 && (reinterpret_cast<uintptr_t>(dx) & 15) == 0) {
            hipStream_t st = as_stream(stream);
            float* slabs = reinterpret_cast<float*>(workspace);
            char* split_ws = reinterpret_cast<char*>(workspace) + slab_bytes;
            PhaseSlabs ps{};
            size_t off = 0;
            for (int ph = 0; ph < stride; ++ph)
                for (int pw = 0; pw < stride; ++pw) {
                    const int k = ph * stride + pw;
                    PhaseGeom g;
                    bwd_phase_geom(g, ph, pw, kh, kw, stride, pad, dil, H, W, Ho, Wo);
                    ps.slab[k] = nullptr; ps.Ha[k] = g.Ha; ps.Wb[k] = g.Wb;
                    if (g.taps.n == 0 || g.Ha == 0 || g.Wb == 0) continue;
                    ConvParams q{};
                    q.x = dy; q.w = w; q.bias = nullptr; q.y = slabs + off; q.ldx = lddy; q.ldy = Cin;
                    q.B = B; q.H = Ho; q.W = Wo; q.Ho = g.Ha; q.Wo = g.Wb; q.Ck = Cout; q.Cn = Cin; q.Cin = Cin; q.Cout = Cout;
                    q.stride = 1; q.M = (int64_t)B * g.Ha * g.Wb; q.bwd_stride = 1; q.accumulate = 0;
                    q.taps = g.taps;
                    if (int rc = launch_conv<true>(q, split_ws, ws_bytes - slab_bytes, st)) return rc;
                    ps.slab[k] = slabs + off;
                    off += (size_t)q.M * Cin;
                }
            const int64_t total = (int64_t)B * H * W * (Cin / 4);
            int64_t blocks = cdiv(total, 256 * 4);
            if (blocks > 8192) blocks = 8192;
            hipLaunchKernelGGL(bwd_phase_interleave_kernel, dim3((unsigned)blocks), dim3(256), 0, st, ps, stride, B, H, W, Cin / 4, dx, lddx,
                               accumulate ? 1 : 0);
            return check_launch("bwd_phase_interleave_kernel");
        }
    }
    ConvParams p{};
    p.x = dy; p.w = w; p.bias = nullptr; p.y = dx; p.ldx = lddy; p.ldy = lddx;
    p.B = B; p.H = Ho; p.W = Wo; p.Ho = H; p.Wo = W; p.Ck = Cout; p.Cn = Cin; p.Cin = Cin; p.Cout = Cout;
    p.stride = 1; p.M = (int64_t)B * H * W; p.bwd_stride = stride; p.accumulate = accumulate ? 1 : 0;
    build_taps(p.taps, kh, kw, 1, pad, dil, Ho, Wo, H, W, true, stride);
    if (p.M > 0x7FFFFFFFll) return fail(PP_ERR_UNSUPPORTED, "conv bwd_data: more than 2^31 pixels");
    if (p.taps.n == 0) return fail(PP_ERR_BAD_ARG, "conv bwd_data: no live tap");
    p.a_pre = stride == 1 ? reinterpret_cast<const uint16_t*>(dy_planes) : nullptr;
    p.b_pre = stride == 1 ? reinterpret_cast<const uint16_t*>(w_planes) : nullptr;
    return launch_conv<true>(p, workspace, ws_bytes, as_stream(stream), kh * kw);
}

int pp_conv2d_bwd_data(const float* dy, int64_t lddy, int B, int Ho, int Wo, int Cout, const float* w, int kh, int kw,
                       int stride, int pad, int dil, float* dx, int64_t lddx, int H, int W, int Cin, int accumulate,
                       void* workspace, size_t ws_bytes, pp_stream_t stream)
{
    return conv2d_bwd_data_impl(dy, lddy, B, Ho, Wo, Cout, w, kh, kw, stride, pad, dil, dx, lddx, H, W, Cin, accumulate, workspace, ws_bytes,
                                stream, nullptr);
}

struct MultiBwd { ConvParams p; ConvPlan pl; bool ok; };
static MultiBwd multi_bwd_setup(int B, int H, int W, int Cin, int Cout, int nb, const int* k, const int* d, int64_t lddy)
{
    MultiBwd m{};
    if (B < 1 || H < 1 || W < 1 || Cin < 1 || Cout < 1 || nb < 2 || nb > 4) return m;
    ConvParams& p = m.p;
    p.ldx = lddy; p.B = B; p.H = H; p.W = W; p.Ho = H; p.Wo = W; p.Ck = Cout; p.Cn = Cin; p.Cin = Cin; p.Cout = Cout;
    p.stride = 1; p.M = (int64_t)B * H * W; p.bwd_stride = 1; p.multi = 1;
    p.taps.n = 0;
    for (int b = 0; b < nb; ++b) {
        if (k[b] < 1 || (k[b] & 1) == 0 || d[b] < 1 || k[b] * k[b] > kMaxTaps) return m;
        ConvTaps t;
        build_taps(t, k[b], k[b], 1, d[b] * (k[b] - 1) / 2, d[b], H, W, H, W, true, 1);
        for (int i = 0; i < t.n; ++i) {
            if (p.taps.n >= 32) return m;
            p.taps.dh[p.taps.n] = t.dh[i]; p.taps.dw[p.taps.n] = t.dw[i];
            p.taps.widx[p.taps.n] = (b << 8) | t.widx[i];
            p.tap_coff[p.taps.n] = b * Cout;
            ++p.taps.n;
        }
    }
    if (p.taps.n == 0 || p.M > 0x7FFFFFFFll) return m;
    const bool vec = Cin % 4 == 0 && Cout % 4 == 0 && lddy % 4 == 0;
    m.pl = plan_conv(p.M, Cin, Cout, p.taps.n, vec);
    if (m.pl.cfg == 2 && m.pl.splits > 1) {
        const int nk = p.taps.n * (int)cdiv(Cout, BK);
        int64_t sp = (int64_t)device_cus() * 4 / m.pl.tiles;
        if (sp > nk / g_splitk_min_iters) sp = nk / g_splitk_min_iters;
        if (sp > 32) sp = 32;
        if (sp > m.pl.splits) {
            m.pl.ks_per_split = (int)cdiv(nk, sp);
            m.pl.splits = (int)cdiv(nk, m.pl.ks_per_split);
        }
    }
    m.ok = vec && m.pl.cfg == 2 && g_conv_dma64 == 1 && (int64_t)B * H * W * lddy < (1ll << 31) - (1ll << 24);
    return m;
}

size_t pp_conv2d_bwd_data_multi_workspace_bytes(int B, int H, int W, int Cin, int Cout, int nb, int k0, int d0, int k1, int d1, int k2, int d2,
                                                int k3, int d3)
{
    const int k[4] = {k0, k1, k2, k3}, d[4] = {d0, d1, d2, d3};
    const MultiBwd m = multi_bwd_setup(B, H, W, Cin, Cout, nb, k, d, (int64_t)nb * Cout);
    if (!m.ok) return 0;
    return align_up(m.pl.splits > 1 ? (size_t)m.pl.splits * m.p.M * Cin * 4 : 256, 256);
}

int pp_conv2d_bwd_data_multi(const float* dy, int64_t lddy, int B, int H, int W, int Cout, int nb, const float* w0, int k0, int d0,
                             const float* w1, int k1, int d1, const float* w2, int k2, int d2, const float* w3, int k3, int d3, float* dx,
                             int64_t lddx, int Cin, int accumulate, void* workspace, size_t ws_bytes, pp_stream_t stream)
{
    const int k[4] = {k0, k1, k2, k3}, d[4] = {d0, d1, d2, d3};
    const float* w[4] = {w0, w1, w2, w3};
    if (!dy || !dx || lddy < (int64_t)nb * Cout || lddx < Cin) return fail(PP_ERR_BAD_ARG, "conv bwd_data multi: null / leading dimension");
    MultiBwd m = multi_bwd_setup(B, H, W, Cin, Cout, nb, k, d, lddy);
    if (!m.ok) return fail(PP_ERR_UNSUPPORTED, "conv bwd_data multi: not offered for this shape (ask the workspace query first)");
    const float* base = nullptr;
    for (int b = 0; b < nb; ++b) {
        if (!w[b]) return fail(PP_ERR_BAD_ARG, "conv bwd_data multi: null weight");
        if (!base || w[b] < base) base = w[b];
    }
    if ((reinterpret_cast<uintptr_t>(dy) & 15) || (reinterpret_cast<uintptr_t>(dx) & 15) || lddx % 4 != 0)
        return fail(PP_ERR_BAD_ARG, "conv bwd_data multi: dy / dx must be 16-byte aligned");
    ConvParams& p = m.p;
    for (int t = 0; t < p.taps.n; ++t) {
        const int b = p.taps.widx[t] >> 8, lt = p.taps.widx[t] & 255;
        const int64_t off = (w[b] - base) + (int64_t)lt * Cin * Cout;
        if ((reinterpret_cast<uintptr_t>(w[b]) & 15) || off + (int64_t)Cin * Cout >= (1ll << 31))
            return fail(PP_ERR_UNSUPPORTED, "conv bwd_data multi: the branch weights must be 16-byte aligned and within 8 GiB of each other");
        p.tap_woff[t] = (int)off;
        p.taps.widx[t] = 0;
    }
    const size_t need = m.pl.splits > 1 ? (size_t)m.pl.splits * p.M * Cin * 4 : 0;
// ... 408 lines not shown
```

### pixelpick_amd/csrc/nn_ops.hip

```cpp
#include "pp_common.h"
#include "bn_xchg.h"
#include "lowres_tile.h"

namespace pp {

constexpr int kT = 256;

__device__ __forceinline__ float act_fwd(float z, int act)
{
    if (act == 1) return fmaxf(z, 0.0f);
    if (act == 2) return fminf(fmaxf(z, 0.0f), 6.0f);
    return z;
}
__device__ __forceinline__ void decode_bhwq(int64_t e, int cq, int Wd, int Hd, int& q, int& w, int& h, int& b)
{
    if (e <= 0xFFFFFFFFll) {
        const unsigned u = (unsigned)e;
        const unsigned t = u / (unsigned)cq;
        q = (int)(u - t * (unsigned)cq);
        const unsigned t2 = t / (unsigned)Wd;
        w = (int)(t - t2 * (unsigned)Wd);
        const unsigned t3 = t2 / (unsigned)Hd;
        h = (int)(t2 - t3 * (unsigned)Hd);
        b = (int)t3;
// ... 2673 lines not shown
    if (!stats || !gamma || !beta || !mean || !invstd || !scale || !shift) return fail(PP_ERR_BAD_ARG, "bn_finalize_partials: null");
    if (rows < 1 || rows > 0x7FFFFFFFll || M < 1 || C < 1) return fail(PP_ERR_BAD_ARG, "bn_finalize_partials: shape");
    if (C % 4 == 0 && (reinterpret_cast<uintptr_t>(stats) & 15) == 0) {
        hipLaunchKernelGGL(bn_finalize_quad_kernel, dim3((unsigned)(C / 4)), dim3(kT), 0, as_stream(stream), stats, (int)rows, C, (double)M,
                           gamma, beta, eps, momentum, running_mean, running_var, mean, invstd, scale, shift);
        return check_launch("bn_finalize_quad_kernel");
    }
    hipLaunchKernelGGL(bn_finalize_kernel, dim3((unsigned)cdiv(C, 8)), dim3(kT), 0, as_stream(stream), stats, (int)rows, C, (double)M,
                       gamma, beta, eps, momentum, running_mean, running_var, mean, invstd, scale, shift);
    return check_launch("bn_finalize_kernel");
}

int pp_pad2d(const float* x, int64_t ldx, int B, int H, int W, int C, int pad_top, int pad_left, int Hp, int Wp, float* y,
             int64_t ldy, pp_stream_t stream)
{
    if (!x || !y) return fail(PP_ERR_BAD_ARG, "pad2d: null");
    if (int rc = need_c4(C, "pad2d")) return rc;
    hipLaunchKernelGGL(pad_kernel, dim3(grid_for((int64_t)B * Hp * Wp * (C / 4))), dim3(kT), 0, as_stream(stream), x, ldx, B,
                       H, W, C / 4, pad_top, pad_left, y, ldy, Hp, Wp);
    return check_launch("pad_kernel");
}

int pp_crop2d_add(const float* xp, int64_t ldxp, int B, int Hp, int Wp, int C, int pad_top, int pad_left, const float* add,
                  int64_t ldadd, float* y, int64_t ldy, int H, int W, pp_stream_t stream)
{
    if (!xp || !y) return fail(PP_ERR_BAD_ARG, "crop2d_add: null");
    if (int rc = need_c4(C, "crop2d_add")) return rc;
    hipLaunchKernelGGL(crop_kernel, dim3(grid_for((int64_t)B * H * W * (C / 4))), dim3(kT), 0, as_stream(stream), xp, ldxp, B,
                       Hp, Wp, C / 4, pad_top, pad_left, add, ldadd, y, ldy, H, W);
    return check_launch("crop_kernel");
}

__global__ __launch_bounds__(kT) void bilinear_bwd_sepw_kernel(const float* dy, int64_t lddy, int B, int Ho, int Wo, int cq,
                                                              float* tmp, int W, float sw, int align)
{
    const int64_t total = (int64_t)B * Ho * W * cq;
    for (int64_t e = (int64_t)blockIdx.x * kT + threadIdx.x; e < total; e += (int64_t)gridDim.x * kT) {
        const int q = (int)(e % cq);
        int64_t t = e / cq;
        const int iw = (int)(t % W);
        const int64_t row = t / W;
        int lo, hi;
        out_window(iw, W, Wo, sw, align, lo, hi);
        const float* src = dy + row * Wo * lddy + q * 4;
        float4 acc = make_float4(0.f, 0.f, 0.f, 0.f);
        for (int ow = lo; ow <= hi; ++ow) {
            const Lerp l = lerp_src(ow, W, sw, align);
            const float wgt = (l.i0 == iw ? l.l0 : 0.0f) + (l.i1 == iw ? l.l1 : 0.0f);
            if (wgt != 0.0f) {
                const float4 v = *reinterpret_cast<const float4*>(src + (int64_t)ow * lddy);
                acc.x = fmaf(wgt, v.x, acc.x); acc.y = fmaf(wgt, v.y, acc.y); acc.z = fmaf(wgt, v.z, acc.z); acc.w = fmaf(wgt, v.w, acc.w);
            }
        }
        *reinterpret_cast<float4*>(tmp + e * 4) = acc;
    }
}

__global__ __launch_bounds__(kT) void bilinear_bwd_seph_kernel(const float* tmp, int B, int Ho, int W, int cq, float* dx,
                                                              int64_t lddx, int H, float sh, int align)
{
    const int64_t total = (int64_t)B * H * W * cq;
    for (int64_t e = (int64_t)blockIdx.x * kT + threadIdx.x; e < total; e += (int64_t)gridDim.x * kT) {
        const int q = (int)(e % cq);
        int64_t t = e / cq;
        const int iw = (int)(t % W); t /= W;
        const int ih = (int)(t % H);
        const int b = (int)(t / H);
        int lo, hi;
        out_window(ih, H, Ho, sh, align, lo, hi);
        const float* src = tmp + (((int64_t)b * Ho) * W + iw) * cq * 4 + q * 4;
        float4 acc = make_float4(0.f, 0.f, 0.f, 0.f);
        for (int oh = lo; oh <= hi; ++oh) {
            const Lerp l = lerp_src(oh, H, sh, align);
            const float wgt = (l.i0 == ih ? l.l0 : 0.0f) + (l.i1 == ih ? l.l1 : 0.0f);
            if (wgt != 0.0f) {
                const float4 v = *reinterpret_cast<const float4*>(src + (int64_t)oh * W * cq * 4);
                acc.x = fmaf(wgt, v.x, acc.x); acc.y = fmaf(wgt, v.y, acc.y); acc.z = fmaf(wgt, v.z, acc.z); acc.w = fmaf(wgt, v.w, acc.w);
            }
        }
        *reinterpret_cast<float4*>(dx + (((int64_t)b * H + ih) * W + iw) * lddx + q * 4) = acc;
    }
}

static void bil_scales(int H, int W, int Ho, int Wo, int align, float scale_h, float scale_w, float& sh, float& sw)
{
    if (align) {
        sh = Ho > 1 ? (float)(H - 1) / (float)(Ho - 1) : 0.0f;
        sw = Wo > 1 ? (float)(W - 1) / (float)(Wo - 1) : 0.0f;
    } else {
        sh = scale_h > 0.0f ? 1.0f / scale_h : (float)H / (float)Ho;
        sw = scale_w > 0.0f ? 1.0f / scale_w : (float)W / (float)Wo;
    }
}

int pp_bilinear_fwd(const float* x, int64_t ldx, int B, int H, int W, int C, float* y, int64_t ldy, int Ho, int Wo,
                    int align_corners, float scale_h, float scale_w, int out_nchw, pp_stream_t stream)
{
    if (!x || !y) return fail(PP_ERR_BAD_ARG, "bilinear fwd: null");
    float sh, sw;
    bil_scales(H, W, Ho, Wo, align_corners, scale_h, scale_w, sh, sw);
    hipStream_t st = as_stream(stream);
    if (out_nchw) {
        hipLaunchKernelGGL((bilinear_fwd_kernel<true>), dim3(grid_for((int64_t)B * C * Ho * Wo)), dim3(kT), 0, st, x, ldx, B, H,
                           W, C, y, ldy, Ho, Wo, sh, sw, align_corners);
    } else {
        if (int rc = need_c4(C, "bilinear fwd (NHWC out)")) return rc;
        hipLaunchKernelGGL((bilinear_fwd_kernel<false>), dim3(grid_for((int64_t)B * Ho * Wo * (C / 4))), dim3(kT), 0, st, x, ldx,
                           B, H, W, C, y, ldy, Ho, Wo, sh, sw, align_corners);
    }
    return check_launch("bilinear_fwd_kernel");
}

size_t pp_bilinear_bwd_workspace_bytes(int B, int Ho, int W, int C)
{
    if (B < 1 || Ho < 1 || W < 1 || C < 1) return 0;
    return align_up((size_t)B * Ho * W * C * 4, 256);
}

int pp_bilinear_bwd(const float* dy, int64_t lddy, int B, int Ho, int Wo, int C, float* dx, int64_t lddx, int H, int W,
                    int align_corners, float scale_h, float scale_w, int dy_nchw, void* workspace, size_t ws_bytes,
                    pp_stream_t stream)
{
    if (!dy || !dx) return fail(PP_ERR_BAD_ARG, "bilinear bwd: null");
    float sh, sw;
    bil_scales(H, W, Ho, Wo, align_corners, scale_h, scale_w, sh, sw);
    hipStream_t st = as_stream(stream);
    const bool win_ok = sh > 0.0f && sw > 0.0f && (int)(2.0f / sw) + 6 <= kMaxWin;
    const bool up2_special = !align_corners && Ho == 2 * H && Wo == 2 * W && H >= 2 && W >= 2 &&
                             (scale_h == 0.0f || scale_h == 2.0f) && (scale_w == 0.0f || scale_w == 2.0f);
    if (!dy_nchw && C % 4 == 0 && lddy % 4 == 0 && lddx % 4 == 0 && sh > 0.0f && sw > 0.0f && Ho >= 3 * H && Wo >= 3 * W &&
        !up2_special && workspace && ws_bytes >= pp_bilinear_bwd_workspace_bytes(B, Ho, W, C) && g_bil_sep) {
        float* tmp = reinterpret_cast<float*>(workspace);
        const int cq = C / 4;
        hipLaunchKernelGGL(bilinear_bwd_sepw_kernel, dim3(grid_for((int64_t)B * Ho * W * cq)), dim3(kT), 0, st, dy, lddy, B, Ho, Wo, cq,
                           tmp, W, sw, align_corners);
        if (int rc = check_launch("bilinear_bwd_sepw_kernel")) return rc;
        hipLaunchKernelGGL(bilinear_bwd_seph_kernel, dim3(grid_for((int64_t)B * H * W * cq)), dim3(kT), 0, st, tmp, B, Ho, W, cq, dx,
                           lddx, H, sh, align_corners);
        return check_launch("bilinear_bwd_seph_kernel");
    }
    if (dy_nchw && win_ok) {
        hipLaunchKernelGGL(bilinear_bwd_planes_kernel, dim3(grid_for((int64_t)B * H * W * C)), dim3(kT), 0, st, dy, B, Ho, Wo, C,
                           dx, lddx, H, W, sh, sw, align_corners);
    } else if (dy_nchw) {
        hipLaunchKernelGGL((bilinear_bwd_kernel<true>), dim3(grid_for((int64_t)B * H * W * C)), dim3(kT), 0, st, dy, lddy, B, Ho,
                           Wo, C, dx, lddx, H, W, sh, sw, align_corners);
    } else if (C % 4 == 0 && lddy % 4 == 0 && lddx % 4 == 0 && !align_corners && Ho == 2 * H && Wo == 2 * W && H >= 2 && W >= 2 &&
               (scale_h == 0.0f || scale_h == 2.0f) && (scale_w == 0.0f || scale_w == 2.0f)) {
        hipLaunchKernelGGL(bilinear_up2_bwd4_kernel, dim3(grid_for((int64_t)B * H * W * (C / 4))), dim3(kT), 0, st, dy, lddy, B, C / 4,
                           dx, lddx, H, W);
    } else if (C % 4 == 0 && lddy % 4 == 0 && lddx % 4 == 0 && win_ok) {
        const int cq = C / 4;
        const int QB = cq >= 32 ? 32 : (cq >= 16 ? 16 : (cq >= 8 ? 8 : cq));
        const int NR = kT / QB;
        const int64_t nblk = (int64_t)B * H * W * cdiv(cq, QB);
        const int hwin = (int)(2.0f / sh) + 6;
        if (hwin >= 4 && (int64_t)B * H * W * cq <= (1 << 19))
            hipLaunchKernelGGL(bilinear_bwd4r_kernel, dim3((unsigned)nblk), dim3(kT), 0, st, dy, lddy, B, Ho, Wo, cq, dx, lddx, H, W,
                               sh, sw, align_corners, QB, NR);
        else
            hipLaunchKernelGGL(bilinear_bwd4_kernel, dim3(grid_for((int64_t)B * H * W * cq)), dim3(kT), 0, st, dy, lddy, B, Ho, Wo,
                               cq, dx, lddx, H, W, sh, sw, align_corners);
    } else {
        hipLaunchKernelGGL((bilinear_bwd_kernel<false>), dim3(grid_for((int64_t)B * H * W * C)), dim3(kT), 0, st, dy, lddy, B, Ho,
                           Wo, C, dx, lddx, H, W, sh, sw, align_corners);
    }
    return check_launch("bilinear_bwd_kernel");
}

int pp_image_colsum(const float* x, int64_t ldx, int B, int64_t P, int C, float mul, float* out, int64_t ldo, pp_stream_t stream)
{
    if (!x || !out) return fail(PP_ERR_BAD_ARG, "image_colsum: null");
    hipLaunchKernelGGL(image_colsum_kernel, dim3((unsigned)cdiv(C, 64), (unsigned)B), dim3(kT), 0, as_stream(stream), x, ldx, P,
                       C, mul, out, ldo);
    return check_launch("image_colsum_kernel");
}

int pp_image_broadcast(const float* v, int64_t ldv, int B, int64_t P, int C, float mul, float* y, int64_t ldy, pp_stream_t stream)
{
    if (!v || !y) return fail(PP_ERR_BAD_ARG, "image_broadcast: null");
    if (int rc = need_c4(C, "image_broadcast")) return rc;
    hipLaunchKernelGGL(image_broadcast_kernel, dim3(grid_for((int64_t)B * P * (C / 4))), dim3(kT), 0, as_stream(stream), v, ldv,
                       B, P, C / 4, mul, y, ldy);
    return check_launch("image_broadcast_kernel");
}

int pp_dropout(const float* x, int64_t ldx, float* y, int64_t ldy, int64_t M, int C, float p, uint64_t seed,
               const uint64_t* seed_dev, pp_stream_t stream)
{
    if (!x || !y) return fail(PP_ERR_BAD_ARG, "dropout: null");
    if (p < 0.0f || p >= 1.0f) return fail(PP_ERR_BAD_ARG, "dropout: p=%f outside [0,1)", (double)p);
    if (C % 4 == 0 && ldx % 4 == 0 && ldy % 4 == 0)
        hipLaunchKernelGGL(dropout4_kernel, dim3(grid_for(M * (C / 4))), dim3(kT), 0, as_stream(stream), x, ldx, y, ldy, M, C / 4,
                           p, 1.0f / (1.0f - p), seed, seed_dev);
    else
        hipLaunchKernelGGL(dropout_kernel, dim3(grid_for(M * C)), dim3(kT), 0, as_stream(stream), x, ldx, y, ldy, M, C, p,
                           1.0f / (1.0f - p), seed, seed_dev);
    return check_launch("dropout_kernel");
}

int pp_dropout2d(const float* x, int64_t ldx, float* y, int64_t ldy, int B, int64_t P, int C, float p, uint64_t seed,
                 const uint64_t* seed_dev, pp_stream_t stream)
{
    if (!x || !y) return fail(PP_ERR_BAD_ARG, "dropout2d: null");
    if (p < 0.0f || p >= 1.0f) return fail(PP_ERR_BAD_ARG, "dropout2d: p=%f outside [0,1)", (double)p);
    if (B <= 0 || P <= 0 || C <= 0) return fail(PP_ERR_BAD_ARG, "dropout2d: B=%d P=%lld C=%d", B, (long long)P, C);
    hipLaunchKernelGGL(dropout2d_kernel, dim3(grid_for((int64_t)B * P * C)), dim3(kT), 0, as_stream(stream), x, ldx, y, ldy, B, P, C,
                       p, 1.0f / (1.0f - p), seed, seed_dev);
    return check_launch("dropout2d_kernel");
}

size_t pp_sparse_ce_workspace_bytes(void) { return 1024 * 2 * 4 + 256; }

int pp_sparse_ce_fwd_bwd(const float* logits, int B, int C, int64_t HW, int64_t sB, int64_t sC, const int64_t* target,
                         int ignore_index, float* loss, float* count, const float* grad_out, float* dlogits, void* workspace,
                         size_t ws_bytes, pp_stream_t stream)
{
    if (!logits || !target || !loss || !count) return fail(PP_ERR_BAD_ARG, "sparse_ce: null");
    if (!workspace || ws_bytes < pp_sparse_ce_workspace_bytes()) return fail(PP_ERR_WORKSPACE, "sparse_ce: workspace");
    hipStream_t st = as_stream(stream);
    float* part = reinterpret_cast<float*>(workspace);
    int nblk = (int)cdiv((int64_t)B * HW, kT * 8);
    if (nblk > 1024) nblk = 1024;
    if (nblk < 1) nblk = 1;
    hipLaunchKernelGGL(ce_partial_kernel, dim3(nblk), dim3(kT), 0, st, logits, target, B, C, HW, sB, sC, ignore_index, part);
    if (int rc = check_launch("ce_partial_kernel")) return rc;
    hipLaunchKernelGGL(ce_finalize_wave_kernel, dim3(1), dim3(64), 0, st, part, nblk, loss, count);
    if (int rc = check_launch("ce_finalize_wave_kernel")) return rc;
    if (dlogits) {
        hipLaunchKernelGGL(ce_bwd_kernel, dim3(grid_for((int64_t)B * HW)), dim3(kT), 0, st, logits, target, B, C, HW, sB, sC,
                           ignore_index, count, grad_out, dlogits);
        if (int rc = check_launch("ce_bwd_kernel")) return rc;
    }
    return PP_OK;
}

size_t pp_sparse_ce_lowres_workspace_bytes(void) { return pp_sparse_ce_workspace_bytes(); }

int pp_sparse_ce_lowres_fwd_bwd(const float* low, int64_t ldx, int B, int C, int h, int w, int H, int W, int align_corners,
                                const int64_t* target, int ignore_index, float* loss, float* count, const float* grad_out,
                                float* dlow, int64_t lddx, void* workspace, size_t ws_bytes, pp_stream_t stream)
{
    if (!low || !target || !loss || !count) return fail(PP_ERR_BAD_ARG, "sparse_ce_lowres: null");
    if (B < 1 || C < 1 || h < 1 || w < 1 || H < 1 || W < 1 || ldx < C || (dlow && lddx < C))
        return fail(PP_ERR_BAD_ARG, "sparse_ce_lowres: bad shape B=%d C=%d %dx%d -> %dx%d ldx=%lld lddx=%lld", B, C, h, w, H, W,
                    (long long)ldx, (long long)lddx);
    if (!workspace || ws_bytes < pp_sparse_ce_lowres_workspace_bytes()) return fail(PP_ERR_WORKSPACE, "sparse_ce_lowres: workspace");
    hipStream_t st = as_stream(stream);
    float sh, sw;
    bil_scales(h, w, H, W, align_corners, 0.0f, 0.0f, sh, sw);
// ... 99 lines not shown
```

### pixelpick_amd/csrc/plan.hip

```cpp
#include "pp_common.h"

#include <cstring>
#include <type_traits>
#include <utility>
#include <vector>

namespace pp {
namespace {

template <typename T>
inline T unpack_slot(uint64_t s)
{
    if constexpr (std::is_same_v<T, float>) {
        float f;
        uint32_t lo = (uint32_t)s;
        memcpy(&f, &lo, 4);
        return f;
    } else if constexpr (std::is_same_v<T, double>) {
        double d;
        memcpy(&d, &s, 8);
        return d;
    } else if constexpr (std::is_pointer_v<T>) {
        return reinterpret_cast<T>(static_cast<uintptr_t>(s));
    } else {
        static_assert(std::is_integral_v<T>, "C-ABI arguments are integers, floats or pointers");
        return static_cast<T>(static_cast<int64_t>(s));
    }
}

template <typename F, F Fn>
struct Thunk;
template <typename... A, int (*Fn)(A...)>
struct Thunk<int (*)(A...), Fn> {
    static constexpr int kArgs = (int)sizeof...(A);
    template <size_t... I>
    static int call_impl(const uint64_t* s, std::index_sequence<I...>) { return Fn(unpack_slot<A>(s[I])...); }
    static int call(const uint64_t* s) { return call_impl(s, std::index_sequence_for<A...>{}); }
};

struct Entry {
    const void* fn;
    int (*call)(const uint64_t*);
    int nargs;
    const char* name;
};

#define PP_PLAN_ENTRY(f) Entry{reinterpret_cast<const void*>(&f), &Thunk<decltype(&f), &f>::call, Thunk<decltype(&f), &f>::kArgs, #f}

const Entry kEntries[] = {
    PP_PLAN_ENTRY(pp_acq_score_topk),
    PP_PLAN_ENTRY(pp_acq_score_map),
    PP_PLAN_ENTRY(pp_acq_softmax_sum),
    PP_PLAN_ENTRY(pp_uncertainty_from_prob),
    PP_PLAN_ENTRY(pp_topk_select),
    PP_PLAN_ENTRY(pp_acq_lowres_score_topk),
    PP_PLAN_ENTRY(pp_acq_lowres_score_at),
    PP_PLAN_ENTRY(pp_acq_lowres_mc_score_topk),
    PP_PLAN_ENTRY(pp_acq_lowres_mc_score_at),
    PP_PLAN_ENTRY(pp_acq_vote_accumulate),
    PP_PLAN_ENTRY(pp_acq_vote_score_map),
    PP_PLAN_ENTRY(pp_acq_lowres_mc_vote_topk),
    PP_PLAN_ENTRY(pp_acq_mean_prob_score_map),
    PP_PLAN_ENTRY(pp_acq_lowres_mc_mean_topk),
    PP_PLAN_ENTRY(pp_spread_select),
    PP_PLAN_ENTRY(pp_acq_region_score_map),
    PP_PLAN_ENTRY(pp_conv2d_fwd),
    PP_PLAN_ENTRY(pp_conv2d_fwd_stats),
    PP_PLAN_ENTRY(pp_bn_train_fwd_partials),
    PP_PLAN_ENTRY(pp_conv2d_fwd_bn_act),
    PP_PLAN_ENTRY(pp_dwconv3x3_fwd_bn_act),
    PP_PLAN_ENTRY(pp_bn_finalize_partials),
    PP_PLAN_ENTRY(pp_dwconv3x3_fwd_fused),
    PP_PLAN_ENTRY(pp_dwconv3x3_bwd_weight_affine_in),
    PP_PLAN_ENTRY(pp_conv2d_fwd_affine_in),
    PP_PLAN_ENTRY(pp_conv2d_bwd_data),
    PP_PLAN_ENTRY(pp_conv2d_bwd_weight),
    PP_PLAN_ENTRY(pp_conv2d_fwd_bn_train),
    PP_PLAN_ENTRY(pp_conv2d_bwd_data_bn_bwd),
    PP_PLAN_ENTRY(pp_x3_split),
    PP_PLAN_ENTRY(pp_conv2d_fwd_pre),
    PP_PLAN_ENTRY(pp_conv2d_bwd_data_pre),
    PP_PLAN_ENTRY(pp_conv2d_bwd_data_multi),
    PP_PLAN_ENTRY(pp_conv2d_fwd_pre2),
    PP_PLAN_ENTRY(pp_conv2d_bwd_data_pre2),
    PP_PLAN_ENTRY(pp_x3_split_weights),
    PP_PLAN_ENTRY(pp_conv2d_bwd_weight_pre),
    PP_PLAN_ENTRY(pp_conv2d_bwd_weight_partials),
    PP_PLAN_ENTRY(pp_wgrad_reduce_batch),
    PP_PLAN_ENTRY(pp_bn_train_fwd),
    PP_PLAN_ENTRY(pp_bn_eval_affine),
    PP_PLAN_ENTRY(pp_scale_shift_act),
    PP_PLAN_ENTRY(pp_bn_bwd),
    PP_PLAN_ENTRY(pp_bn_train_fwd_fused),
    PP_PLAN_ENTRY(pp_dwconv3x3_bn_train_fwd_fused),
    PP_PLAN_ENTRY(pp_bn_bwd_fused),
    PP_PLAN_ENTRY(pp_bn_bwd_fused_sparse),
    PP_PLAN_ENTRY(pp_row_flags),
    PP_PLAN_ENTRY(pp_conv1x1_bwd_weight_sparse),
    PP_PLAN_ENTRY(pp_conv1x1_bwd_data_sparse),
    PP_PLAN_ENTRY(pp_dwconv3x3_fwd),
    PP_PLAN_ENTRY(pp_dwconv3x3_bwd_data),
    PP_PLAN_ENTRY(pp_dwconv3x3_bwd_weight),
    PP_PLAN_ENTRY(pp_dwconv3x3_bwd_weight_partials),
    PP_PLAN_ENTRY(pp_groupnorm_relu_fwd),
    PP_PLAN_ENTRY(pp_groupnorm_relu_bwd),
    PP_PLAN_ENTRY(pp_maxpool2d_fwd),
    PP_PLAN_ENTRY(pp_maxpool2d_bwd),
    PP_PLAN_ENTRY(pp_pad2d),
    PP_PLAN_ENTRY(pp_crop2d_add),
    PP_PLAN_ENTRY(pp_bilinear_fwd),
    PP_PLAN_ENTRY(pp_bilinear_bwd),
    PP_PLAN_ENTRY(pp_image_colsum),
    PP_PLAN_ENTRY(pp_image_broadcast),
    PP_PLAN_ENTRY(pp_dropout),
    PP_PLAN_ENTRY(pp_dropout2d),
    PP_PLAN_ENTRY(pp_aug_resample_h),
    PP_PLAN_ENTRY(pp_aug_vcrop),
    PP_PLAN_ENTRY(pp_aug_labels),
    PP_PLAN_ENTRY(pp_aug_jitter),
    PP_PLAN_ENTRY(pp_aug_blur),
    PP_PLAN_ENTRY(pp_aug_blur_q8),
    PP_PLAN_ENTRY(pp_aug_to_tensor),
    PP_PLAN_ENTRY(pp_sparse_ce_fwd_bwd),
    PP_PLAN_ENTRY(pp_sparse_ce_lowres_fwd_bwd),
    PP_PLAN_ENTRY(pp_confusion_matrix_update),
    PP_PLAN_ENTRY(pp_confusion_matrix_from_labels),
    PP_PLAN_ENTRY(pp_predict_lowres),
    PP_PLAN_ENTRY(pp_vis_lowres),
    PP_PLAN_ENTRY(pp_adam_step_flat),
    PP_PLAN_ENTRY(pp_sgd_step_flat),
    PP_PLAN_ENTRY(pp_add2d),
    PP_PLAN_ENTRY(pp_nhwc_to_nchw),
    PP_PLAN_ENTRY(pp_nchw_to_nhwc),
};

const Entry* find_entry(const void* fn)
{
    for (const Entry& e : kEntries)
        if (e.fn == fn) return &e;
    return nullptr;
}

enum OpKind : int { kCall = 0, kEventRecord = 1, kStreamWait = 2, kHostBreak = 3 };

struct Op {
    int kind;
    int nargs;
    const Entry* entry;
    size_t slot0;
    void* a;
    void* b;
};

}

struct Plan {
    std::vector<Op> ops;
    std::vector<uint64_t> slots;
    std::vector<hipEvent_t> owned_events;
};

}

using pp::Plan;

extern "C" {

pp_plan_t pp_plan_create(void) { return reinterpret_cast<pp_plan_t>(new (std::nothrow) Plan()); }

void pp_plan_destroy(pp_plan_t plan)
{
    Plan* p = reinterpret_cast<Plan*>(plan);
    if (!p) return;
    for (hipEvent_t e : p->owned_events) (void)hipEventDestroy(e);
    delete p;
}

int64_t pp_plan_size(pp_plan_t plan) { return plan ? (int64_t) reinterpret_cast<Plan*>(plan)->ops.size() : 0; }

int pp_plan_entry_args(const void* fn)
{
    const pp::Entry* e = pp::find_entry(fn);
    return e ? e->nargs : -1;
}

int pp_plan_add_call(pp_plan_t plan, const void* fn, const uint64_t* slots, int n_slots)
{
    Plan* p = reinterpret_cast<Plan*>(plan);
    if (!p || !fn || (n_slots > 0 && !slots)) return pp::fail(PP_ERR_BAD_ARG, "plan_add_call: null argument");
    const pp::Entry* e = pp::find_entry(fn);
    if (!e) return pp::fail(PP_ERR_UNSUPPORTED, "plan_add_call: %p is not an entry point of this library that enqueues work", fn);
    if (n_slots != e->nargs) return pp::fail(PP_ERR_BAD_ARG, "plan_add_call: %s takes %d arguments, %d slots given", e->name, e->nargs, n_slots);
    pp::Op op{pp::kCall, n_slots, e, p->slots.size(), nullptr, nullptr};
    p->slots.insert(p->slots.end(), slots, slots + n_slots);
// ... 81 lines not shown
```

### pixelpick_amd/engine.py

```python
import contextlib
import math
import ctypes
import os
import weakref
from typing import List, Optional, Sequence

import torch

from . import _lib

ACT_NONE, ACT_RELU, ACT_RELU6 = 0, 1, 2


class Var:
    __slots__ = ("_t", "grad", "needs_grad", "_pending", "_lazy", "_bn_bwd_ctx", "_closed", "_grad_dst")

    def __init__(self, t: Optional[torch.Tensor], needs_grad: bool = True):
        self._t = t
        self.grad: Optional[torch.Tensor] = None
        self.needs_grad = needs_grad
        self._pending = None
        self._lazy = None
        self._bn_bwd_ctx = None
        self._closed = False
# ... 110 lines not shown
    if bn is None and x._t is None and x._lazy is not None:
        if kind == "dw":
            _launch_dw_fused(v, False)
            return
        raw, scale, shift, act = x._lazy
        B, H, W, Cin, ldx = _geom(raw)
        kh, kw, _, Cout = w.shape
        if conv_accepts_lazy_input(B, H, W, Cin, Cout, kh, kw, stride, pad, dil):
            v._pending = None
            y = torch.empty((B, H, W, Cout), dtype=torch.float32, device=raw.device)
            ws, wsn = _conv_ws(False, raw.device, B, H, W, Cin, Cout, kh, kw, stride, pad, dil)
            rc = _lib.lib().pp_conv2d_fwd_affine_in(raw.data_ptr(), ldx, B, H, W, Cin, scale.data_ptr(), shift.data_ptr(), act, w.data_ptr(),
                                                    bias.data_ptr() if bias is not None else None, kh, kw, stride, pad, dil, y.data_ptr(),
                                                    Cout, Cout, ws, wsn, _stream())
            _lib.check(rc, "pp_conv2d_fwd_affine_in")
            v._t = y
            return
    v._pending = None
    L = _lib.lib()
    B, H, W, Cin, ldx = _geom(x.t)
    dev = x.t.device
    g = be = rm = rv = rptr = None
    eps, act, ldr, dst = 0.0, 0, 0, None
    if bn is not None:
        gamma, beta, mean, var, eps, act, residual, dst = bn
        g, be, rm, rv = gamma.data_ptr(), beta.data_ptr(), mean.data_ptr(), var.data_ptr()
        if residual is not None:
            _, _, _, _, ldr = _geom(residual.t)
            rptr = residual.t.data_ptr()
    if kind == "conv":
        kh, kw, _, Cout = w.shape
        Ho, Wo = out_size(H, kh, stride, pad, dil), out_size(W, kw, stride, pad, dil)
        y = dst if dst is not None else torch.empty((B, Ho, Wo, Cout), dtype=torch.float32, device=dev)
        _, _, _, _, ldy = _geom(y)
        ws, wsn = _conv_ws(False, dev, B, H, W, Cin, Cout, kh, kw, stride, pad, dil)
        rc = L.pp_conv2d_fwd_bn_act(x.t.data_ptr(), ldx, B, H, W, Cin, w.data_ptr(), bias.data_ptr() if bias is not None else None,
                                    kh, kw, stride, pad, dil, g, be, rm, rv, eps, rptr, ldr, act, y.data_ptr(), ldy, Cout,
                                    ws, wsn, _stream())
        _lib.check(rc, "pp_conv2d_fwd_bn_act")
    else:
        Ho, Wo = out_size(H, 3, stride, pad, dil), out_size(W, 3, stride, pad, dil)
        y = dst if dst is not None else torch.empty((B, Ho, Wo, Cin), dtype=torch.float32, device=dev)
        _, _, _, _, ldy = _geom(y)
        rc = L.pp_dwconv3x3_fwd_bn_act(x.t.data_ptr(), ldx, B, H, W, Cin, w.data_ptr(), stride, pad, dil, g, be, rm, rv, eps,
                                       rptr, ldr, act, y.data_ptr(), ldy, _stream())
        _lib.check(rc, "pp_dwconv3x3_fwd_bn_act")
    v._t = y


_BIG_WGRAD_MAIN = os.environ.get("PIXELPICK_BIG_WGRAD_MAIN", "1") != "0"
_BIG_WGRAD_FLOP = float(os.environ.get("PIXELPICK_BIG_WGRAD_FLOP", "8e9"))
_side_streams = {}
N_SIDE_STREAMS = int(os.environ.get("PIXELPICK_SIDE_STREAMS", "1"))
SIDE_PRIORITY = int(os.environ.get("PIXELPICK_SIDE_PRIORITY", "0"))


def _side_stream(device, i: int = 0) -> "torch.cuda.Stream":
    key = (device.type, device.index if device.index is not None else torch.cuda.current_device(), i)
    st = _side_streams.get(key)
    if st is None:
        st = torch.cuda.Stream(device=device, priority=SIDE_PRIORITY)
        _side_streams[key] = st
    return st


def _MARK():
    pass


class Tape:
    overlap_wgrad = os.environ.get("PIXELPICK_OVERLAP_WGRAD", "1") != "0"
    trace = None

    def __init__(self, enabled: bool = True):
        refresh_stream()
        self.enabled = enabled
        self.nodes: List = []
        self.param_grads = {}
        self.param_grad_dst = None
        self._side = None
        self._side_rr = 0
        self._keepalive = []
        self.hooks = {}
        self._jobs_first = 0
        self._jobs_next = 0
        self._arena_off = 0

    def mark(self, name: str):
        if self.enabled:
            self.nodes.append((_MARK, name, None))

    def side_streams_in_use(self):
        return list(self._side.values()) if self._side else []

    def record(self, fn, ctx, out: Var):
        if self.enabled:
            self.nodes.append((fn, ctx, out))

    def grad_buffer_for(self, param: torch.Tensor) -> torch.Tensor:
        if self.param_grad_dst is not None:
            g = self.param_grad_dst(param)
            if g is not None:
                return g
        return torch.empty_like(param)

    def set_param_grad(self, param: torch.Tensor, g: torch.Tensor):
        key = id(param)
        if key in self.param_grads:
            self.flush_reduces(g.device)
            prev = self.param_grads[key]
            with (self.side_stream_for(prev, g) if _role[0] == 0 else _NULL_CTX):
                add2d_(prev.view(1, -1), g.view(1, -1), prev.view(1, -1))
        else:
            self.param_grads[key] = g

    def side_stream_for(self, *tensors):
        if not Tape.overlap_wgrad:
            return _NULL_CTX
        dev = tensors[0].device
        i = self._side_rr
        self._side_rr = (i + 1) % N_SIDE_STREAMS
        side = _side_stream(dev, i)
        ev = _fork_event(dev)
        _lib.plan_note(ev.record, _main_stream_obj())
        _lib.plan_note(side.wait_event, ev)
        self._keepalive.extend(tensors)
        if self._side is None:
            self._side = {}
        self._side[i] = side
        _SIDE_CTX.handle = side.cuda_stream
        _SIDE_CTX.role = 1 + i
        return _SIDE_CTX

    def defer_slot(self, nbytes: int, device):
        if not (_BATCH_REDUCE and Tape.overlap_wgrad and N_SIDE_STREAMS == 1) or nbytes > _ARENA_BYTES:
            return None
        if (self._jobs_next >= len(_JOB_POOL) or self._arena_off + nbytes > _ARENA_BYTES or self._jobs_next - self._jobs_first >= 64
                or self._arena_off >= _FLUSH_BYTES):
            self.flush_reduces(device)
            if self._jobs_next >= len(_JOB_POOL):
                return None
        return _JOB_POOL[self._jobs_next], _arena(device).data_ptr() + self._arena_off, nbytes

    def defer_commit(self, job):
        if job.kind != 0:
            used = job.splits * job.cn * 4 * (1 if job.kind == 3 else job.ntaps)
            self._arena_off = (self._arena_off + used + 255) & ~255
            self._jobs_next += 1

    def flush_reduces(self, device):
        n = self._jobs_next - self._jobs_first
        if n > 0:
            args = (ctypes.addressof(_JOB_POOL[self._jobs_first]), n)
            if _role[0] != 0:
                rc = _lib.lib().pp_wgrad_reduce_batch(*args, _stream())
            else:
                with self.side_stream_for(_arena(device)):
                    rc = _lib.lib().pp_wgrad_reduce_batch(*args, _stream())
            _lib.check(rc, "pp_wgrad_reduce_batch")
        self._jobs_first = self._jobs_next
        self._arena_off = 0

    def backward(self, out: Var, dout: torch.Tensor):
        refresh_stream()
        if Tape.trace is not None:
            Tape.trace.append(("bwd_begin", _mark()))
        out.grad = dout
        for fn, ctx, o in reversed(self.nodes):
            if fn is _MARK:
                hook = self.hooks.get(ctx)
                if hook is not None:
                    self.flush_reduces(dout.device)
                    hook(self)
                continue
            if o.grad is None:
                continue
            fn(self, o.grad, *ctx)
            o.grad = None
        self.nodes = []
        self.flush_reduces(dout.device)
        if Tape.trace is not None:
            Tape.trace.append(("bwd_main_end", _mark()))
        if self._side is not None:
            for side in self._side.values():
                _lib.plan_note(_main_stream_obj().wait_stream, side)
            self._side = None
        if Tape.trace is not None:
            Tape.trace.append(("joined", _mark()))
        self._keepalive = []


_stream_cache = [None]
_stream_obj_cache = [None]
_role = [0]
_fork_events = {}
_NULL_CTX = contextlib.nullcontext()


def refresh_stream():
    st = torch.cuda.current_stream()
    _stream_obj_cache[0] = st
    _stream_cache[0] = st.cuda_stream


def _stream():
    if _stream_cache[0] is None:
        refresh_stream()
    return _stream_cache[0]


def _main_stream_obj():
    if _stream_obj_cache[0] is None:
        refresh_stream()
    return _stream_obj_cache[0]


def _mark():
    ev = torch.cuda.Event(enable_timing=True)
    ev.record(_main_stream_obj())
    return ev


def _fork_event(device):
    key = (device.type, device.index)
    ev = _fork_events.get(key)
    if ev is None:
        ev = torch.cuda.Event()
        _fork_events[key] = ev
    return ev


class _SideCtx:
    __slots__ = ("handle", "prev", "role")

    def __enter__(self):
        self.prev = _stream_cache[0]
        _stream_cache[0] = self.handle
        _role[0] = self.role

    def __exit__(self, *exc):
        _stream_cache[0] = self.prev
        _role[0] = 0
        return False


_SIDE_CTX = _SideCtx()


def _geom(t: torch.Tensor):
    B, H, W, C = t.shape
    if t.is_contiguous():
        if t.dtype != torch.float32 or not t.is_cuda:
            raise AssertionError("NHWC float32 GPU tensor expected")
        return B, H, W, C, C
    assert t.dim() == 4 and t.dtype == torch.float32 and t.is_cuda, "NHWC float32 GPU tensor expected"
    if C > 1 and t.stride(3) != 1:
        raise ValueError("channel axis must be contiguous")
    if W > 1:
        ld = t.stride(2)
    elif H > 1:
        ld = t.stride(1)
    elif B > 1:
# ... 279 lines not shown
    key = (bwd,) + shape
    _memo_epoch()
    need = _CONV_WS_BYTES.get(key)
    if need is None:
        L = _lib.lib()
        need = int((L.pp_conv2d_bwd_data_workspace_bytes if bwd else L.pp_conv2d_fwd_workspace_bytes)(*shape))
        _CONV_WS_BYTES[key] = need
    if need == 0:
        return None, 0
    dk = (device.type, device.index)
    buf = _CONV_WS_BUF.get(dk)
    if buf is None or buf.numel() < need:
        if buf is not None:
            _SCRATCH_RETIRED.append(buf)
        buf = torch.empty(max(need, 2 * (buf.numel() if buf is not None else 0), _CONV_WS_MIN), dtype=torch.uint8, device=device)
        _CONV_WS_BUF[dk] = buf
    return buf.data_ptr(), buf.numel()


class ConvBwdGroup:

    def __init__(self, x: Var, specs, ws_bytes: int):
        B, H, W, Cin = shape_of(x)
        self.x, self.specs, self.ws_bytes = x, specs, ws_bytes
        self.n = len(specs)
        self.Cout = specs[0][0].shape[3]
        self.dbuf = torch.empty((B, H, W, self.n * self.Cout), dtype=torch.float32, device=x.t.device)
        self.arrived = [False] * self.n

    def slice(self, i: int) -> torch.Tensor:
        return self.dbuf[..., i * self.Cout:(i + 1) * self.Cout]

    @staticmethod
    def offered(x: Var, specs) -> int:
        if not (2 <= len(specs) <= 4):
            return 0
        B, H, W, Cin = shape_of(x)
        Cout = specs[0][0].shape[3]
        flat = []
        for w, k, d in specs:
            if tuple(w.shape) != (k, k, Cin, Cout) or w.data_ptr() & 15:
                return 0
            flat += [k, d]
        flat += [0, 0] * (4 - len(specs))
        ptrs = [w.data_ptr() for w, _, _ in specs]
        if max(ptrs) - min(ptrs) + max(w.numel() for w, _, _ in specs) * 4 >= (1 << 33) - (1 << 26):
            return 0
        return _wsbytes("pp_conv2d_bwd_data_multi_workspace_bytes", B, H, W, Cin, Cout, len(specs), *flat)

    def arrive(self, tape: "Tape", i: int, dy: torch.Tensor):
        if self.arrived[i]:
            raise RuntimeError("ConvBwdGroup: a branch's backward ran twice")
        sl = self.slice(i)
        if dy.data_ptr() != sl.data_ptr() or dy.stride() != sl.stride():
            sl.copy_(dy)
        self.arrived[i] = True
        if not all(self.arrived):
            return
        x = self.x
        if not x.needs_grad:
            return
        if getattr(x, "_closed", False):
            raise RuntimeError("ConvBwdGroup: the input's gradient was already consumed by a fused BatchNorm backward")
        B, H, W, Cin = shape_of(x)
        dev = self.dbuf.device
        acc_into = x.grad if (x.grad is not None and getattr(x.grad, "_pp_owned", False) and x.grad.is_contiguous()
                              and tuple(x.grad.shape) == (B, H, W, Cin)) else None
        dx = acc_into if acc_into is not None else torch.empty((B, H, W, Cin), dtype=torch.float32, device=dev)
        ws = _ws(self.ws_bytes, dev)
        args = []
        for w, k, d in self.specs:
            args += [w.data_ptr(), k, d]
        args += [None, 0, 0] * (4 - self.n)
        rc = _lib.lib().pp_conv2d_bwd_data_multi(self.dbuf.data_ptr(), self.n * self.Cout, B, H, W, self.Cout, self.n, *args, dx.data_ptr(), Cin, Cin,
                                                 1 if acc_into is not None else 0, ws.data_ptr(), ws.numel(), _stream())
        _lib.check(rc, "pp_conv2d_bwd_data_multi")
        tape._keepalive.append(self.dbuf)
        if acc_into is None:
            dx._pp_owned = True
            _acc(x, dx)


def conv2d(tape: Tape, x: Var, w: torch.Tensor, bias: Optional[torch.Tensor], stride=1, pad=0, dil=1,
           dst: Optional[torch.Tensor] = None, bwd_group=None) -> Var:
    B, H, W, Cin = shape_of(x)
    kh, kw, wcin, Cout = w.shape
    assert wcin == Cin, f"conv2d: Cin {Cin} vs weight {tuple(w.shape)}"
    if _FUSE_EVAL and not tape.enabled and dst is None:
        out = Var(None, needs_grad=False)
        out._pending = ("conv", x, w, bias, stride, pad, dil)
        return out
    if (tape.enabled and dst is None and (_CONV_BN_STATS or _BN_ON_LOAD or
                                           (_CONV_BN_FUSE and bias is None and _conv_bn_fusable(B, H, W, Cin, Cout, kh, kw, stride, pad, dil)))):
        out = Var(None)
        out._pending = ("conv", x, w, bias, stride, pad, dil)
        if bwd_group is not None:
            out._grad_dst = bwd_group[0].slice(bwd_group[1])
        tape.record(_conv2d_bwd, (x, w, bias, stride, pad, dil, None, bwd_group), out)
        return out
    _, _, _, _, ldx = _geom(x.t)
    Ho, Wo = out_size(H, kh, stride, pad, dil), out_size(W, kw, stride, pad, dil)
    y = dst if dst is not None else torch.empty((B, Ho, Wo, Cout), dtype=torch.float32, device=x.t.device)
    _, _, _, _, ldy = _geom(y)
    ws, wsn = _conv_ws(False, x.t.device, B, H, W, Cin, Cout, kh, kw, stride, pad, dil)
    xp = None
    if (tape.enabled and w.requires_grad and _x3_planes(0, B, H, W, Cin, Cout, kh, kw, stride, pad, dil)
            and _x3_planes(2, B, H, W, Cin, Cout, kh, kw, stride, pad, dil)):
        xp = _x3_split(x.t, ldx, B * H * W, Cin)
    if xp is not None or (tape.enabled and w.requires_grad and _x3_planes(3, B, H, W, Cin, Cout, kh, kw, stride, pad, dil)):
        wp = _weight_planes(w, 1)
        _register_weight_planes(w, 1)
        rc = _lib.lib().pp_conv2d_fwd_pre2(x.t.data_ptr(), ldx, B, H, W, Cin, w.data_ptr(), bias.data_ptr() if bias is not None else None,
                                           kh, kw, stride, pad, dil, y.data_ptr(), ldy, Cout, ws, wsn, xp.data_ptr() if xp is not None else None, wp, _stream())
    else:
        rc = _lib.lib().pp_conv2d_fwd(x.t.data_ptr(), ldx, B, H, W, Cin, w.data_ptr(), bias.data_ptr() if bias is not None else None,
                                      kh, kw, stride, pad, dil, y.data_ptr(), ldy, Cout, ws, wsn, _stream())
    _lib.check(rc, "pp_conv2d_fwd")
    out = Var(y)
    if bwd_group is not None and tape.enabled:
        out._grad_dst = bwd_group[0].slice(bwd_group[1])
    tape.record(_conv2d_bwd, (x, w, bias, stride, pad, dil, xp, bwd_group), out)
    return out


def _conv2d_bwd(tape: Tape, dy: torch.Tensor, x: Var, w, bias, stride, pad, dil, xp=None, bwd_group=None):
    L = _lib.lib()
    lazy_in = x._lazy if (x._t is None and x._lazy is not None) else None
    B, H, W, Cin, ldx = _geom(lazy_in[0] if lazy_in is not None else x.t)
    if lazy_in is not None:
        ldx = Cin
    _, Ho, Wo, Cout, lddy = _geom(dy)
    kh, kw = w.shape[0], w.shape[1]
    dev = dy.device
    dyp = None
    if (w.requires_grad and x.needs_grad and lazy_in is None and _x3_planes(1, B, H, W, Cin, Cout, kh, kw, stride, pad, dil)
            and _x3_planes(2, B, H, W, Cin, Cout, kh, kw, stride, pad, dil)):
        dyp = _x3_split(dy, lddy, B * Ho * Wo, Cout)
    big = _BIG_WGRAD_MAIN and 2.0 * B * Ho * Wo * Cin * Cout * kh * kw >= _BIG_WGRAD_FLOP

    def _issue_wgrad():
        dw = tape.grad_buffer_for(w)
        db = tape.grad_buffer_for(bias) if (bias is not None and bias.requires_grad) else None
        with (_NULL_CTX if big else tape.side_stream_for(lazy_in[0] if lazy_in is not None else x.t, dy, dw, db)):
            if lazy_in is not None:
                tape._keepalive.append(x.t)
            nws = _wsbytes("pp_conv2d_bwd_weight_workspace_bytes", B, H, W, Cin, Cout, kh, kw, stride, pad, dil)
            slot = tape.defer_slot(nws, dev) if (not big and db is None) else None
            flags = getattr(dy, "_pp_rowflags", None) if (_SPARSE_ROWS and _SPARSE_WGRAD) else None
            nsp = (_wsbytes("pp_conv1x1_bwd_weight_sparse_workspace_bytes", B * H * W, Cin, Cout)
                   if (flags is not None and kh == 1 and kw == 1 and stride == 1 and pad == 0 and lazy_in is None and xp is None and dyp is None
                       and flags.numel() == B * H * W) else 0)
            if nsp:
                ws = _ws(nsp, dev)
                rc = L.pp_conv1x1_bwd_weight_sparse(x.t.data_ptr(), ldx, B * H * W, Cin, dy.data_ptr(), lddy, Cout, flags.data_ptr(),
                                                    dw.data_ptr(), db.data_ptr() if db is not None else None, ws.data_ptr(), ws.numel(), _stream())
                tape._keepalive.append(flags)
            elif slot is not None:
                job, wptr, _ = slot
                rc = L.pp_conv2d_bwd_weight_partials(x.t.data_ptr(), ldx, B, H, W, Cin, dy.data_ptr(), lddy, Cout, kh, kw, stride, pad, dil,
                                                     dw.data_ptr(), None, wptr, nws, ctypes.addressof(job), _stream())
                tape.defer_commit(job)
            elif xp is not None or dyp is not None:
                ws = _ws(nws, dev)
                tape._keepalive.extend(t for t in (xp, dyp) if t is not None)
                rc = L.pp_conv2d_bwd_weight_pre(x.t.data_ptr(), ldx, B, H, W, Cin, dy.data_ptr(), lddy, Cout, kh, kw, stride, pad, dil,
                                                dw.data_ptr(), db.data_ptr() if db is not None else None, ws.data_ptr(), ws.numel(),
                                                xp.data_ptr() if xp is not None else None, dyp.data_ptr() if dyp is not None else None, _stream())
            else:
                ws = _ws(nws, dev)
                rc = L.pp_conv2d_bwd_weight(x.t.data_ptr(), ldx, B, H, W, Cin, dy.data_ptr(), lddy, Cout, kh, kw, stride, pad, dil,
                                            dw.data_ptr(), db.data_ptr() if db is not None else None, ws.data_ptr(), ws.numel(),
                                            _stream())
        _lib.check(rc, "pp_conv2d_bwd_weight")
        tape.set_param_grad(w, dw)
        if db is not None:
            tape.set_param_grad(bias, db)
    def _issue_dx():
        if x._closed:
            raise RuntimeError("a second convolution's backward reached a BatchNorm output whose backward already ran (wrong `consumers` hint)")
        bctx = x._bn_bwd_ctx if (x.needs_grad and _CONV_BN_FUSE_BWD and lazy_in is None) else None
        if bctx is not None:
            have = x.grad is not None
            if bctx[7] != (2 if have else 1) or (have and not (x.grad.is_contiguous() and tuple(x.grad.shape) == (B, H, W, Cin))):
                bctx = None
        if (bctx is not None and bctx[0].needs_grad and not ((dy.data_ptr() | w.data_ptr()) & 15) and lddy % 4 == 0
                and _conv_bn_bwd_fusable(B, H, W, Cin, Cout, kh, kw, stride, pad, dil) and _bn_exchange_ok(dev)):
            bin_, g_, b_, mean_, invstd_, act_, res_, _ = bctx
            _, _, _, _, ldb = _geom(bin_.t)
            dxbn = torch.empty((B, H, W, Cin), dtype=torch.float32, device=dev)
            dres = torch.empty((B, H, W, Cin), dtype=torch.float32, device=dev) if (res_ is not None and res_.needs_grad) else None
            gin = x.grad
            dg_, db_ = tape.grad_buffer_for(g_), tape.grad_buffer_for(b_)
            sync, xws = _bn_exchange(dev)
            rc = L.pp_conv2d_bwd_data_bn_bwd(dy.data_ptr(), lddy, B, Ho, Wo, Cout, w.data_ptr(), kh, kw, stride, pad, dil, H, W, Cin,
                                             bin_.t.data_ptr(), ldb, mean_.data_ptr(), invstd_.data_ptr(), g_.data_ptr(), b_.data_ptr(), act_,
                                             dg_.data_ptr(), db_.data_ptr(), dxbn.data_ptr(), Cin,
                                             gin.data_ptr() if gin is not None else None, Cin, dres.data_ptr() if dres is not None else None, Cin,
                                             xws.data_ptr(), xws.numel(), sync.data_ptr(), sync.numel(), _stream())
            _lib.check(rc, "pp_conv2d_bwd_data_bn_bwd")
            tape.set_param_grad(g_, dg_)
            tape.set_param_grad(b_, db_)
            if gin is not None:
                tape._keepalive.append(gin)
            x.grad = None
            x._closed = True
            dxbn._pp_owned = True
            _acc(bin_, dxbn)
            if dres is not None:
                dres._pp_owned = True
                _acc(res_, dres)
        elif x.needs_grad:
            acc_into = x.grad if (x.grad is not None and getattr(x.grad, "_pp_owned", False) and x.grad.is_contiguous()
                                  and tuple(x.grad.shape) == (B, H, W, Cin)) else None
            flags = getattr(dy, "_pp_rowflags", None) if _SPARSE_ROWS else None
            if (flags is not None and kh == 1 and kw == 1 and stride == 1 and pad == 0 and acc_into is None and lazy_in is None and Cin % 4 == 0
                    and flags.numel() == B * H * W and dyp is None):
                dx = torch.empty((B, H, W, Cin), dtype=torch.float32, device=dev)
                rc = L.pp_conv1x1_bwd_data_sparse(dy.data_ptr(), lddy, B * H * W, Cout, w.data_ptr(), Cin, flags.data_ptr(), dx.data_ptr(), Cin, _stream())
                _lib.check(rc, "pp_conv1x1_bwd_data_sparse")
                dx._pp_rowflags = flags
                _acc(x, dx)
                return
            dx = acc_into if acc_into is not None else torch.empty((B, H, W, Cin), dtype=torch.float32, device=dev)
            ws, wsn = _conv_ws(True, dev, B, H, W, Cin, Cout, kh, kw, stride, pad, dil)
            if dyp is not None or (stride == 1 and w.requires_grad and _x3_planes(4, B, H, W, Cin, Cout, kh, kw, stride, pad, dil)):
                wp = _weight_planes(w, 0) if stride == 1 else None
                if stride == 1:
                    _register_weight_planes(w, 0)
                rc = L.pp_conv2d_bwd_data_pre2(dy.data_ptr(), lddy, B, Ho, Wo, Cout, w.data_ptr(), kh, kw, stride, pad, dil,
                                               dx.data_ptr(), Cin, H, W, Cin, 1 if acc_into is not None else 0, ws, wsn,
                                               dyp.data_ptr() if dyp is not None else None, wp, _stream())
            else:
                rc = L.pp_conv2d_bwd_data(dy.data_ptr(), lddy, B, Ho, Wo, Cout, w.data_ptr(), kh, kw, stride, pad, dil,
                                          dx.data_ptr(), Cin, H, W, Cin, 1 if acc_into is not None else 0, ws, wsn, _stream())
            _lib.check(rc, "pp_conv2d_bwd_data")
            if acc_into is None:
                dx._pp_owned = True
                _acc(x, dx)

    if bwd_group is not None:
        if w.requires_grad:
            _issue_wgrad()
        bwd_group[0].arrive(tape, bwd_group[1], dy)
        return
    if w.requires_grad and (big or not _WGRAD_LATE):
        _issue_wgrad()
        _issue_dx()
    else:
        _issue_dx()
        if w.requires_grad:
            _issue_wgrad()


def dwconv3x3(tape: Tape, x: Var, w: torch.Tensor, stride=1, pad=0, dil=1) -> Var:
    if _FUSE_EVAL and not tape.enabled:
        out = Var(None, needs_grad=False)
        out._pending = ("dw", x, w, None, stride, pad, dil)
        return out
    if tape.enabled and (_BN_ON_LOAD or (_FUSE_DW_BN and _dw_bn_fusable(*_dw_out_rows(x, stride, pad, dil)))):
        out = Var(None)
        out._pending = ("dw", x, w, None, stride, pad, dil)
        tape.record(_dwconv_bwd, (x, w, stride, pad, dil), out)
        return out
    B, H, W, C, ldx = _geom(x.t)
    Ho, Wo = out_size(H, 3, stride, pad, dil), out_size(W, 3, stride, pad, dil)
    y = torch.empty((B, Ho, Wo, C), dtype=torch.float32, device=x.t.device)
    rc = _lib.lib().pp_dwconv3x3_fwd(x.t.data_ptr(), ldx, B, H, W, C, w.data_ptr(), stride, pad, dil, y.data_ptr(), C, _stream())
    _lib.check(rc, "pp_dwconv3x3_fwd")
    out = Var(y)
    tape.record(_dwconv_bwd, (x, w, stride, pad, dil), out)
    return out


def _dwconv_bwd(tape: Tape, dy, x: Var, w, stride, pad, dil):
    L = _lib.lib()
    lazy_in = x._lazy if (x._t is None and x._lazy is not None) else None
    B, H, W, C, ldx = _geom(lazy_in[0] if lazy_in is not None else x.t)
    if lazy_in is not None and not _DW_WGRAD_AFFINE:
        with tape.side_stream_for(lazy_in[0], dy):
            tape._keepalive.append(x.t)
        lazy_in, ldx = None, C
    _, Ho, Wo, _, lddy = _geom(dy)
    dev = dy.device
    if w.requires_grad:
        dw = tape.grad_buffer_for(w)
        if lazy_in is not None:
            raw, scale, shift, act = lazy_in
            with tape.side_stream_for(raw, dy, dw):
                ws = _ws(_wsbytes("pp_colreduce_workspace_bytes", B * Ho * Wo, C), dev)
                rc = L.pp_dwconv3x3_bwd_weight_affine_in(raw.data_ptr(), ldx, B, H, W, C, scale.data_ptr(), shift.data_ptr(), act,
                                                         dy.data_ptr(), lddy, stride, pad, dil, dw.data_ptr(), ws.data_ptr(), ws.numel(),
                                                         _stream())
            _lib.check(rc, "pp_dwconv3x3_bwd_weight_affine_in")
        else:
            with tape.side_stream_for(x.t, dy, dw):
                nws = _wsbytes("pp_colreduce_workspace_bytes", B * Ho * Wo, C)
                slot = tape.defer_slot(nws, dev)
                if slot is not None:
                    job, wptr, _ = slot
                    rc = L.pp_dwconv3x3_bwd_weight_partials(x.t.data_ptr(), ldx, B, H, W, C, dy.data_ptr(), lddy, stride, pad, dil,
                                                            dw.data_ptr(), wptr, nws, ctypes.addressof(job), _stream())
                    tape.defer_commit(job)
                else:
                    ws = _ws(nws, dev)
                    rc = L.pp_dwconv3x3_bwd_weight(x.t.data_ptr(), ldx, B, H, W, C, dy.data_ptr(), lddy, stride, pad, dil, dw.data_ptr(),
                                                   ws.data_ptr(), ws.numel(), _stream())
            _lib.check(rc, "pp_dwconv3x3_bwd_weight")
        tape.set_param_grad(w, dw)
    if x.needs_grad:
        dx = torch.empty((B, H, W, C), dtype=torch.float32, device=dev)
        rc = L.pp_dwconv3x3_bwd_data(dy.data_ptr(), lddy, B, H, W, C, w.data_ptr(), stride, pad, dil, dx.data_ptr(), C, _stream())
        _lib.check(rc, "pp_dwconv3x3_bwd_data")
        _acc(x, dx)


def _dw_bn_train_fused(tape: Tape, x: Var, gamma, beta, running_mean, running_var, act, residual, eps, momentum, dst):
    _, xin, w, _, stride, pad, dil = x._pending
    B, H, W, C, ld_in = _geom(xin.t)
    Ho, Wo = out_size(H, 3, stride, pad, dil), out_size(W, 3, stride, pad, dil)
    M = B * Ho * Wo
    if M > _BN_FUSED_MAXM or M >= (1 << 31) or C > 65536 or C % 4 or ld_in % 4:
        return None
    dev = xin.t.device
    xbuf = torch.empty((B, Ho, Wo, C), dtype=torch.float32, device=dev)
    mean = torch.empty(C, dtype=torch.float32, device=dev)
    invstd = torch.empty(C, dtype=torch.float32, device=dev)
    y = dst if dst is not None else torch.empty((B, Ho, Wo, C), dtype=torch.float32, device=dev)
    _, _, _, _, ldy = _geom(y)
    rptr, ldr = (None, 0)
    if residual is not None:
        _, _, _, _, ldr = _geom(residual.t)
        rptr = residual.t.data_ptr()
    sync, ws = _bn_exchange(dev)
    rc = _lib.lib().pp_dwconv3x3_bn_train_fwd_fused(
# ... 346 lines not shown
    _lib.check(rc, "pp_bilinear_fwd")
    out = Var(y)
    tape.record(_bilinear_bwd, (x, (Ho, Wo), align_corners, scale_factor, out_nchw), out)
    return out


def _bilinear_bwd(tape: Tape, dy, x: Var, size, align_corners, scale_factor, out_nchw):
    if not x.needs_grad:
        return
    B, H, W, C, _ = _geom(x.t)
    Ho, Wo = size
    if out_nchw:
        dy = dy.contiguous()
        lddy = 0
    else:
        _, _, _, _, lddy = _geom(dy)
    dx = torch.empty((B, H, W, C), dtype=torch.float32, device=dy.device)
    ws_ptr, ws_n = None, 0
    if not out_nchw and Ho >= 3 * H and Wo >= 3 * W:
        ws = _ws(_wsbytes("pp_bilinear_bwd_workspace_bytes", B, Ho, W, C), dy.device)
        ws_ptr, ws_n = ws.data_ptr(), ws.numel()
    rc = _lib.lib().pp_bilinear_bwd(dy.data_ptr(), lddy, B, Ho, Wo, C, dx.data_ptr(), C, H, W, int(align_corners),
                                    float(scale_factor), float(scale_factor), int(out_nchw), ws_ptr, ws_n, _stream())
    _lib.check(rc, "pp_bilinear_bwd")
    _acc(x, dx)


def global_avg_pool(tape: Tape, x: Var) -> Var:
    B, H, W, C, ldx = _geom(x.t)
    y = torch.empty((B, 1, 1, C), dtype=torch.float32, device=x.t.device)
    rc = _lib.lib().pp_image_colsum(x.t.data_ptr(), ldx, B, H * W, C, 1.0 / (H * W), y.data_ptr(), C, _stream())
    _lib.check(rc, "pp_image_colsum")
    out = Var(y)
    tape.record(_gap_bwd, (x,), out)
    return out


def _gap_bwd(tape: Tape, dy, x: Var):
    if not x.needs_grad:
        return
    B, H, W, C, _ = _geom(x.t)
    dx = torch.empty((B, H, W, C), dtype=torch.float32, device=dy.device)
    rc = _lib.lib().pp_image_broadcast(dy.data_ptr(), C, B, H * W, C, 1.0 / (H * W), dx.data_ptr(), C, _stream())
    _lib.check(rc, "pp_image_broadcast")
    _acc(x, dx)


def broadcast_hw(tape: Tape, v: Var, H: int, W: int, dst: Optional[torch.Tensor] = None) -> Var:
    B, _, _, C, ldv = _geom(v.t)
    y = dst if dst is not None else torch.empty((B, H, W, C), dtype=torch.float32, device=v.t.device)
    _, _, _, _, ldy = _geom(y)
    rc = _lib.lib().pp_image_broadcast(v.t.data_ptr(), ldv, B, H * W, C, 1.0, y.data_ptr(), ldy, _stream())
    _lib.check(rc, "pp_image_broadcast")
    out = Var(y)
    tape.record(_broadcast_bwd, (v, H, W), out)
    return out


def _broadcast_bwd(tape: Tape, dy, v: Var, H, W):
    B, _, _, C, _ = _geom(v.t)
    _, _, _, _, lddy = _geom(dy)
    dv = torch.empty((B, 1, 1, C), dtype=torch.float32, device=dy.device)
    rc = _lib.lib().pp_image_colsum(dy.data_ptr(), lddy, B, H * W, C, 1.0, dv.data_ptr(), C, _stream())
    _lib.check(rc, "pp_image_colsum")
    _acc(v, dv)


_dropout_counter = [0]
_dropout_seed_dev = [None]


def set_dropout_seed(seed: int):
    _dropout_counter[0] = int(seed) * 1000003


def set_dropout_device_seed(t: Optional[torch.Tensor]):
    _dropout_seed_dev[0] = t


def begin_step():
    if _dropout_seed_dev[0] is not None:
        _dropout_counter[0] = 0
    _STEP_EPOCH[0] += 1
    if _X3_WPRE and _X3_WPL:
        _prefetch_weight_planes()


def end_step():
    _STEP_EPOCH[0] += 1


_X3_WPRE = os.environ.get("PIXELPICK_X3_WEIGHT_PREFETCH", "1") != "0"
_STEP_EPOCH = [0]
_X3_WPL = {}
_X3_WPL_EVENT = {}


def _register_weight_planes(w: torch.Tensor, transpose: int):
    if not _X3_WPRE or w.dim() != 4:
        return
    ent = _X3_WPL.get(id(w))
    if ent is None or ent["w"]() is not w:
        ent = _X3_WPL[id(w)] = {"w": weakref.ref(w), "planes": {}, "epoch": -1}
    ent["used"] = _STEP_EPOCH[0]
    if transpose not in ent["planes"]:
        kh, kw, Cin, Cout = w.shape
        nb = int(_lib.lib().pp_x3_weight_planes_bytes(kh * kw, Cin, Cout, transpose))
        ent["planes"][transpose] = torch.empty(nb, dtype=torch.uint8, device=w.device)
        ent["epoch"] = -1


def _prefetch_weight_planes():
    L = _lib.lib()
    by_dev = {}
    for key, ent in list(_X3_WPL.items()):
        w = ent["w"]()
        if w is None or not w.is_cuda:
            del _X3_WPL[key]
            continue
        if ent.get("used", -10) < _STEP_EPOCH[0] - 3:
            continue
        by_dev.setdefault(w.device, []).append((ent, w))
    for dev, ents in by_dev.items():
        main = _main_stream_obj()
        side = _side_stream(dev, 0)
        ev = _fork_event(dev)
        _lib.plan_note(ev.record, main)
        _lib.plan_note(side.wait_event, ev)
        for ent, w in ents:
            kh, kw, Cin, Cout = w.shape
            for tr, planes in ent["planes"].items():
                _lib.check(L.pp_x3_split_weights(w.data_ptr(), kh * kw, Cin, Cout, tr, planes.data_ptr(), planes.numel(), side.cuda_stream),
                           "pp_x3_split_weights")
            ent["epoch"] = _STEP_EPOCH[0]
        dk = (dev.type, dev.index)
        rec = _X3_WPL_EVENT.get(dk)
        done = rec[0] if rec is not None else torch.cuda.Event()
        _lib.plan_note(done.record, side)
        _X3_WPL_EVENT[dk] = [done, _STEP_EPOCH[0], -1]


def _weight_planes(w: torch.Tensor, transpose: int):
    ent = _X3_WPL.get(id(w))
    if ent is not None and ent["w"]() is w:
        ent["used"] = _STEP_EPOCH[0]
    if ent is None or ent["w"]() is not w or ent["epoch"] != _STEP_EPOCH[0] or transpose not in ent["planes"]:
        return None
    rec = _X3_WPL_EVENT.get((w.device.type, w.device.index))
    if rec is None or rec[1] != _STEP_EPOCH[0]:
        return None
    if rec[2] != _STEP_EPOCH[0]:
        _lib.plan_note(_main_stream_obj().wait_event, rec[0])
        rec[2] = _STEP_EPOCH[0]
    return ent["planes"][transpose].data_ptr()


def dropout(tape: Tape, x: Var, p: float, training: bool) -> Var:
    if not training or p <= 0.0:
        return x
    B, H, W, C, ldx = _geom(x.t)
    _dropout_counter[0] += 1
    seed = (_dropout_counter[0] * 0x9E3779B97F4A7C15) & 0xFFFFFFFFFFFFFFFF
    y = torch.empty((B, H, W, C), dtype=torch.float32, device=x.t.device)
    sd = _dropout_seed_dev[0]
    rc = _lib.lib().pp_dropout(x.t.data_ptr(), ldx, y.data_ptr(), C, B * H * W, C, float(p), seed,
                               sd.data_ptr() if sd is not None else None, _stream())
    _lib.check(rc, "pp_dropout")
    out = Var(y)
    tape.record(_dropout_bwd, (x, p, seed), out)
    return out


def _dropout_bwd(tape: Tape, dy, x: Var, p, seed):
    if not x.needs_grad:
        return
    B, H, W, C, _ = _geom(x.t)
    _, _, _, _, lddy = _geom(dy)
    dx = torch.empty((B, H, W, C), dtype=torch.float32, device=dy.device)
    sd = _dropout_seed_dev[0]
    rc = _lib.lib().pp_dropout(dy.data_ptr(), lddy, dx.data_ptr(), C, B * H * W, C, float(p), seed,
                               sd.data_ptr() if sd is not None else None, _stream())
    _lib.check(rc, "pp_dropout")
    _acc(x, dx)


def dropout2d(tape: Tape, x: Var, p: float, training: bool) -> Var:
    if not training or p <= 0.0:
        return x
    B, H, W, C, ldx = _geom(x.t)
    _dropout_counter[0] += 1
    seed = (_dropout_counter[0] * 0x9E3779B97F4A7C15) & 0xFFFFFFFFFFFFFFFF
    y = torch.empty((B, H, W, C), dtype=torch.float32, device=x.t.device)
    sd = _dropout_seed_dev[0]
    rc = _lib.lib().pp_dropout2d(x.t.data_ptr(), ldx, y.data_ptr(), C, B, H * W, C, float(p), seed,
                                 sd.data_ptr() if sd is not None else None, _stream())
    _lib.check(rc, "pp_dropout2d")
    out = Var(y, needs_grad=x.needs_grad)
    tape.record(_dropout2d_bwd, (x, p, seed), out)
    return out


def _dropout2d_bwd(tape: Tape, dy, x: Var, p, seed):
    if not x.needs_grad:
        return
    B, H, W, C, _ = _geom(x.t)
    _, _, _, _, lddy = _geom(dy)
    dx = torch.empty((B, H, W, C), dtype=torch.float32, device=dy.device)
    sd = _dropout_seed_dev[0]
    rc = _lib.lib().pp_dropout2d(dy.data_ptr(), lddy, dx.data_ptr(), C, B, H * W, C, float(p), seed,
                                 sd.data_ptr() if sd is not None else None, _stream())
    _lib.check(rc, "pp_dropout2d")
    _acc(x, dx)


def concat_alias(tape: Tape, buf: torch.Tensor, parts: Sequence[Var]) -> Var:
    off = 0
    for p in parts:
        c = p.t.shape[3]
        assert p.t.data_ptr() == buf[..., off:off + c].data_ptr(), "concat_alias: part not produced in place"
        off += c
    assert off == buf.shape[3]
    out = Var(buf)
    tape.record(_concat_bwd, (tuple(parts),), out)
    return out


def _concat_bwd(tape: Tape, dy, parts):
    off = 0
    for p in parts:
        c = p.t.shape[3]
        _acc(p, dy[..., off:off + c])
        off += c


def cross_entropy_nchw(logits: torch.Tensor, target: torch.Tensor, ignore_index: int, want_grad: bool = True, sparse: bool = True):
    assert logits.is_cuda and logits.dtype == torch.float32 and logits.dim() == 4
    B, C, H, W = logits.shape
# ... 41 lines not shown
```

### pixelpick_amd/networks/decoders.py

```python
import math

import torch
import torch.nn as nn

from .. import engine as E
from .layers import BatchNorm2d, Conv2d, Dropout, ReLU


class GroupNorm(nn.Module):

    def __init__(self, num_groups, num_channels, eps=1e-5):
        super().__init__()
        self.num_groups, self.num_channels, self.eps = num_groups, num_channels, eps
        self.weight = nn.Parameter(torch.ones(num_channels))
        self.bias = nn.Parameter(torch.zeros(num_channels))

    def run(self, tape, x, relu=True):
        return E.group_norm_relu(tape, x, self.weight, self.bias, self.num_groups, relu, self.eps)

    def forward(self, x):
        raise RuntimeError("pixelpick_amd layers execute through run(tape, x)")


class UpsampleBlock(nn.Module):
# ... 1 lines not shown
    def __init__(self, in_channels, out_channels=128, kernel_size=3, padding=1, n_groups=32, scale_factor=2):
        super().__init__()
        self.block = nn.Sequential(Conv2d(in_channels, out_channels, kernel_size, padding=padding),
                                   GroupNorm(n_groups, out_channels), ReLU(inplace=True))
        self.scale_factor = scale_factor

    def run(self, tape, x, upsample=True):
        h = self.block[1].run(tape, self.block[0].run(tape, x), relu=True)
        if not upsample:
            return h
        _, H, W, _ = h.t.shape
        return E.bilinear(tape, h, (int(math.floor(H * self.scale_factor)), int(math.floor(W * self.scale_factor))), False,
                          float(self.scale_factor))


class FPNDecoder(nn.Module):

    def __init__(self, args):
        super().__init__()
        n_classes, wm = args.n_classes, args.width_multiplier
        if args.n_layers in [18, 34]:
            chans = [int(512 * wm), int(256 * wm), int(128 * wm), int(64 * wm)]
        elif args.n_layers in [50, 101]:
            chans = [int(2048 * wm), int(1024 * wm), int(512 * wm), int(256 * wm)]
        else:
            raise ValueError(args.n_layers)
        self.lat_layer_0 = Conv2d(chans[0], 256, 1)
        self.lat_layer_1 = Conv2d(chans[1], 256, 1)
        self.lat_layer_2 = Conv2d(chans[2], 256, 1)
        self.lat_layer_3 = Conv2d(chans[3], 256, 1)
        self.upsample_blocks_0 = nn.Sequential(UpsampleBlock(256, 128), UpsampleBlock(128, 128), UpsampleBlock(128, 128))
        self.upsample_blocks_1 = nn.Sequential(UpsampleBlock(256, 128), UpsampleBlock(128, 128), UpsampleBlock(128, 128))
        self.upsample_blocks_2 = nn.Sequential(UpsampleBlock(256, 128), UpsampleBlock(128, 128), UpsampleBlock(128, 128))
        self.upsample_blocks_3 = nn.Sequential(UpsampleBlock(256, 128), UpsampleBlock(128, 128))
        self.classifier = Conv2d(128, n_classes, 1)
        for m in self.modules():
            if isinstance(m, Conv2d):
                fan_in = m.in_channels * m.kernel_size * m.kernel_size
                with torch.no_grad():
                    m.weight.normal_(0, math.sqrt(2.0 / fan_in))

    @staticmethod
    def _upsample_add(tape, x, y):
        _, h, w, _ = y.t.shape
        return E.add(tape, E.bilinear(tape, x, (h, w), False, 0.0), y)

    @staticmethod
    def _seq(tape, seq, x, last_upsample=True):
        n = len(seq)
        for i, blk in enumerate(seq):
            x = blk.run(tape, x, upsample=last_upsample or i + 1 < n)
        return x

    def run(self, tape, feats, lowres=False):
        c2, c3, c4, c5 = feats
        c5 = self.lat_layer_0.run(tape, c5)
        c4 = self.lat_layer_1.run(tape, c4)
        c3 = self.lat_layer_2.run(tape, c3)
        c2 = self.lat_layer_3.run(tape, c2)
        p5 = c5
        p4 = self._upsample_add(tape, p5, c4)
        p3 = self._upsample_add(tape, p4, c3)
        p2 = self._upsample_add(tape, p3, c2)
        p5 = self._seq(tape, self.upsample_blocks_0, p5, not lowres)
        p4 = self._seq(tape, self.upsample_blocks_1, p4, not lowres)
        p3 = self._seq(tape, self.upsample_blocks_2, p3, not lowres)
        p2 = self._seq(tape, self.upsample_blocks_3, p2, not lowres)
        emb = E.add(tape, E.add(tape, E.add(tape, p2, p3), p4), p5)
        if lowres:
            return {"emb": None, "pred": self.classifier.run(tape, emb)}
        return {"emb": emb, "pred": self.classifier.run(tape, emb)}


class SegmentHead(nn.Module):
    def __init__(self, args, openset=False):
        super().__init__()
        self.segment_head = nn.Sequential(Conv2d(304, 256, kernel_size=3, stride=1, padding=1, bias=False),
                                          BatchNorm2d(256), ReLU(), Dropout(0.5),
                                          Conv2d(256, 256, kernel_size=3, stride=1, padding=1, bias=False),
                                          BatchNorm2d(256), ReLU(), Dropout(args.mc_dropout_p))
        self.classifier = Conv2d(256, args.n_classes, 1)
        self.n_classes = args.n_classes

    def run(self, tape, x):
        s = self.segment_head
        h = s[1].run(tape, s[0].run(tape, x), E.ACT_RELU, dropout=s[3])
        emb = s[5].run(tape, s[4].run(tape, h), E.ACT_RELU, dropout=s[7])
        pred = self.classifier.run(tape, emb)
        return {"emb": emb, "pred": pred}
```

### pixelpick_amd/networks/deeplab.py

```python
import torch
import torch.nn as nn

from .. import engine as E
from .aspp import ASPP
from .decoders import SegmentHead
from .layers import BatchNorm2d, Conv2d, Dropout, ReLU
from .mobilenet_v2 import MobileNetV2


class _LazyOutputs(dict):

    def __init__(self, pred, emb_low, size):
        super().__init__(pred=pred)
        self._emb_low, self._size = emb_low, size

    def _emb(self):
        if not dict.__contains__(self, "emb"):
            v = E.bilinear(E.Tape(False), E.Var(self._emb_low), self._size, True, 0.0, out_nchw=True)
            dict.__setitem__(self, "emb", v.t)
        return dict.__getitem__(self, "emb")

    def __getitem__(self, k):
        return self._emb() if k == "emb" else dict.__getitem__(self, k)

# ... 1 lines not shown
        return k == "emb" or dict.__contains__(self, k)

    def keys(self):
        return ["pred", "emb"]


class _NetFunction(torch.autograd.Function):

    @staticmethod
    def forward(ctx, inputs, model, *params):
        tape = E.Tape(enabled=True)
        pred, emb_low = model._run(tape, inputs)
        ctx.tape, ctx.pred_var, ctx.params = tape, pred, params
        ctx.model = model
        model._last_emb_low = emb_low.t
        return pred.t

    @staticmethod
    def backward(ctx, dpred):
        tape = ctx.tape
        tape.backward(ctx.pred_var, dpred.contiguous())
        grads = tuple(tape.param_grads.get(id(p)) if p.requires_grad else None for p in ctx.params)
        ctx.tape = None
        return (None, None) + grads


class DeepLab(nn.Module):
    LOWRES_LOGITS = True
    LOWRES_ALIGN_CORNERS = True
    LOWRES_EXACT = True

    def __init__(self, args, backbone='mobilenet', output_stride=16):
        super().__init__()
        self._resnet = backbone == 'resnet'
        if self._resnet:
            from .backbones.resnet_backbone import ResNetBackbone
            if output_stride != 8:
                raise NotImplementedError("the dilated ResNet backbone has output stride 8 (resnet_backbone.py:53-58)")
            self.backbone = ResNetBackbone(backbone='resnet50_dilated8', pretrained=None)
            low_level_inplanes = 256
        else:
            self.backbone = MobileNetV2(output_stride, BatchNorm2d, mc_dropout=args.use_mc_dropout,
                                        pretrained=getattr(args, "weight_type", None) != "random")
            low_level_inplanes = 24
        self.aspp = ASPP(backbone, output_stride, BatchNorm2d)
        self.low_level_conv = nn.Sequential(Conv2d(low_level_inplanes, 48, 1, bias=False), BatchNorm2d(48), ReLU())
        self.seg_head = SegmentHead(args)
        self.return_features = False
        self.return_attention = False
        self._last_emb_low = None

    def turn_on_dropout(self):
        for m in self.modules():
            if isinstance(m, Dropout):
                m.train()

    def turn_off_dropout(self):
        for m in self.modules():
            if isinstance(m, Dropout):
                m.eval()

    def set_return_features(self, return_features):
        self.return_features = return_features

    def set_return_attention(self, return_attention):
        self.return_attention = return_attention

    def _run(self, tape, inputs, upsample=True):
        B, _, H, W = inputs.shape
        x = E.nchw_to_nhwc(inputs)
        if self._resnet:
            feats = self.backbone.run(tape, x)
            high, low = feats[3], feats[0]
        else:
            high, low = self.backbone.run(tape, x)
        tape.mark("encoder_done")
        a = self.aspp.run(tape, high)
        _, Hl, Wl, _ = low.t.shape
        cat_buf = torch.empty((B, Hl, Wl, 304), dtype=torch.float32, device=inputs.device)
        up = E.bilinear(tape, a, (Hl, Wl), True, 0.0, dst=cat_buf[..., 0:256])
        llc = self.low_level_conv
        low_ = llc[1].run(tape, llc[0].run(tape, low), E.ACT_RELU, dst=cat_buf[..., 256:304])
        cat = E.concat_alias(tape, cat_buf, [up, low_])
        outs = self.seg_head.run(tape, cat)
        if not upsample:
            return outs["pred"], outs["emb"]
        pred = E.bilinear(tape, outs["pred"], (H, W), True, 0.0, out_nchw=True)
        return pred, outs["emb"]

    def forward_lowres(self, inputs):
        if not inputs.is_cuda:
            raise RuntimeError("pixelpick_amd.DeepLab runs on the GPU only (no CPU fallback)")
        pred_v, _ = self._run(E.Tape(enabled=False), inputs.to(torch.float32), upsample=False)
        return pred_v.t, tuple(inputs.shape[2:])

    @torch.no_grad()
    def predict(self, inputs):
        from ..predict import predict_lowres
        low, size = self.forward_lowres(inputs)
        return predict_lowres(low, size, align_corners=self.LOWRES_ALIGN_CORNERS)[0]

    def forward(self, inputs):
        if not inputs.is_cuda:
            raise RuntimeError("pixelpick_amd.DeepLab runs on the GPU only (no CPU fallback); move the model and "
                               "inputs to cuda")
        inputs = inputs.to(torch.float32)
        params = [p for p in self.parameters()]
        if torch.is_grad_enabled() and any(p.requires_grad for p in params):
            pred = _NetFunction.apply(inputs, self, *params)
            emb_low = self._last_emb_low
        else:
            pred_v, emb_v = self._run(E.Tape(enabled=False), inputs)
            pred, emb_low = pred_v.t, emb_v.t
        return _LazyOutputs(pred, emb_low, tuple(inputs.shape[2:]))
```

### pixelpick_amd/networks/layers.py

```python
import math

import torch
import torch.nn as nn

from .. import _lib
from .. import engine as E


def _bump_nbt(d):
    d["_nbt_pending"] += 1


def _kaiming_normal_oihw(cout, cin_per_group, kh, kw, nonlinearity_gain=math.sqrt(2.0)):
    fan_in = cin_per_group * kh * kw
    std = nonlinearity_gain / math.sqrt(fan_in)
    return torch.randn(cout, cin_per_group, kh, kw) * std


class Conv2d(nn.Module):

    def __init__(self, in_channels, out_channels, kernel_size, stride=1, padding=0, dilation=1, groups=1, bias=True):
        super().__init__()
        assert groups in (1, in_channels), "only dense and depthwise convolutions occur in the reference"
        self.in_channels, self.out_channels = in_channels, out_channels
        self.kernel_size, self.stride, self.padding, self.dilation, self.groups = kernel_size, stride, padding, dilation, groups
        self.depthwise = groups != 1
        k = kernel_size
        if self.depthwise:
            assert k == 3 and in_channels == out_channels
            w = _kaiming_normal_oihw(out_channels, 1, k, k)[:, 0].permute(1, 2, 0).contiguous()
        else:
            w = _kaiming_normal_oihw(out_channels, in_channels, k, k).permute(2, 3, 1, 0).contiguous()
        self.weight = nn.Parameter(w)
        if bias:
            bound = 1.0 / math.sqrt(in_channels // groups * k * k)
            self.bias = nn.Parameter(torch.empty(out_channels).uniform_(-bound, bound))
        else:
            self.register_parameter("bias", None)

    def weight_oihw(self) -> torch.Tensor:
        w = self.weight.detach()
        if self.depthwise:
            return w.permute(2, 0, 1).unsqueeze(1).contiguous()
        return w.permute(3, 2, 0, 1).contiguous()

    def _save_to_state_dict(self, destination, prefix, keep_vars):
        destination[prefix + "weight"] = self.weight_oihw()
        if self.bias is not None:
            destination[prefix + "bias"] = self.bias if keep_vars else self.bias.detach()

    def _load_from_state_dict(self, state_dict, prefix, local_metadata, strict, missing_keys, unexpected_keys, error_msgs):
        key = prefix + "weight"
        if key in state_dict:
            w = state_dict[key]
            if w.dim() == 4 and not self.depthwise and tuple(w.shape) == (self.out_channels, self.in_channels, self.kernel_size, self.kernel_size):
                w = w.permute(2, 3, 1, 0).contiguous()
            elif w.dim() == 4 and self.depthwise and tuple(w.shape) == (self.out_channels, 1, 3, 3):
                w = w[:, 0].permute(1, 2, 0).contiguous()
            elif tuple(w.shape) != tuple(self.weight.shape):
                error_msgs.append(f"size mismatch for {key}: got {tuple(w.shape)}")
                w = None
            if w is not None:
                with torch.no_grad():
                    self.weight.copy_(w)
        elif strict:
            missing_keys.append(key)
        bkey = prefix + "bias"
        if self.bias is not None:
            if bkey in state_dict:
                with torch.no_grad():
                    self.bias.copy_(state_dict[bkey])
            elif strict:
                missing_keys.append(bkey)
        elif bkey in state_dict and strict:
            unexpected_keys.append(bkey)

    def accepts_lazy_input(self, in_shape, extra_pad: int = 0) -> bool:
        if self.depthwise:
            return True
        B, H, W, C = in_shape
        k = self.kernel_size
        return E.conv_accepts_lazy_input(B, H, W, C, self.out_channels, k, k, self.stride, self.padding + extra_pad, self.dilation)

    def run(self, tape, x, dst=None, extra_pad: int = 0, bwd_group=None):
        if self.depthwise:
            return E.dwconv3x3(tape, x, self.weight, self.stride, self.padding + extra_pad, self.dilation)
        return E.conv2d(tape, x, self.weight, self.bias, self.stride, self.padding + extra_pad, self.dilation, dst=dst, bwd_group=bwd_group)

    def forward(self, x):
        raise RuntimeError("pixelpick_amd layers execute through run(tape, x); call the network's forward()")

    def extra_repr(self):
        return (f"{self.in_channels}, {self.out_channels}, kernel_size={self.kernel_size}, stride={self.stride}, "
                f"padding={self.padding}, dilation={self.dilation}, groups={self.groups}, bias={self.bias is not None}")


class BatchNorm2d(nn.Module):

    def __init__(self, num_features, eps=1e-5, momentum=0.1):
        super().__init__()
        self.num_features, self.eps, self.momentum = num_features, eps, momentum
        self.weight = nn.Parameter(torch.ones(num_features))
        self.bias = nn.Parameter(torch.zeros(num_features))
        self.register_buffer("running_mean", torch.zeros(num_features))
        self.register_buffer("running_var", torch.ones(num_features))
        self.register_buffer("num_batches_tracked", torch.tensor(0, dtype=torch.long))
        self._nbt_pending = 0

    def _save_to_state_dict(self, destination, prefix, keep_vars):
        if self._nbt_pending:
            self.num_batches_tracked += self._nbt_pending
            self._nbt_pending = 0
        super()._save_to_state_dict(destination, prefix, keep_vars)

    def run(self, tape, x, act=E.ACT_NONE, residual=None, dst=None, dropout=None, lazy_ok=False, single_consumer=False, consumers=0):
        training = self.training
        if training:
            B, H, W, _ = E.shape_of(x)
            if B * H * W <= 1:
                raise ValueError(f"Expected more than 1 value per channel when training, got input size {tuple(x.t.shape)}")
            _lib.plan_note_host(_bump_nbt, self.__dict__)
        drop_p = dropout.p if (dropout is not None and dropout.training and dropout.p > 0.0) else 0.0
        return E.batch_norm_act(tape, x, self.weight, self.bias, self.running_mean, self.running_var, training, act,
                                residual, self.eps, self.momentum, dst=dst, dropout_p=drop_p, lazy_ok=lazy_ok,
                                single_consumer=single_consumer, consumers=consumers)

    def forward(self, x):
        raise RuntimeError("pixelpick_amd layers execute through run(tape, x)")

    def extra_repr(self):
        return f"{self.num_features}, eps={self.eps}, momentum={self.momentum}"


class _Placeholder(nn.Module):

    def forward(self, x):
        return x


class ReLU(_Placeholder):
    def __init__(self, inplace=False):
        super().__init__()


class ReLU6(_Placeholder):
    def __init__(self, inplace=False):
        super().__init__()


class Dropout2d(nn.Module):

    def __init__(self, p=0.5):
        super().__init__()
        self.p = p

    def run(self, tape, x):
        return E.dropout2d(tape, x, self.p, self.training)

    def forward(self, x):
        return x

    def extra_repr(self):
        return f"p={self.p}"


class Dropout(nn.Module):

    def __init__(self, p=0.5):
        super().__init__()
        self.p = p
# ... 10 lines not shown
```

Baseline: 763.7 images/s.

## Compute decoder conv grad for upsampled ASPP branch at low resolution via bilinear-adjoint taps

Adds a backward path for the first seg-head 3x3 conv, whose input concatenates a bilinearly upsampled ASPP output with low-level features. The upsample is linear, so the gradient for the upsampled channels is computed at low resolution. A separable bilinear-backward kernel produces per-tap 3x3 gradients, and a 1x1 GEMM against tap-packed weights (cached and prefetched each step) finishes the job. The remaining low-level channels use a new column-restricted bwd-data launch. Large weight-gradient work is also deferred to a tail queue to overlap with later work. This trades full-resolution dx and bilinear backward for extra packing kernels, more complex scheduling, and some rounding-order differences.

```diff
diff --git a/include/pixelpick_hip.h b/include/pixelpick_hip.h
--- a/include/pixelpick_hip.h
+++ b/include/pixelpick_hip.h
@@ -168,6 +168,10 @@
 int pp_conv2d_bwd_data_pre2(const float* dy, int64_t lddy, int B, int Ho, int Wo, int Cout, const float* w, int kh, int kw,
                             int stride, int pad, int dil, float* dx, int64_t lddx, int H, int W, int Cin, int accumulate,
                             void* workspace, size_t ws_bytes, const void* dy_planes, const void* w_planes, pp_stream_t stream);
+int pp_conv2d_bwd_data_cols_ok(int B, int H, int W, int Cin, int Cout, int kh, int kw, int stride, int pad, int dil, int c0, int n);
+int pp_conv2d_bwd_data_cols(const float* dy, int64_t lddy, int B, int Ho, int Wo, int Cout, const float* w, int kh, int kw, int stride, int pad,
+                            int dil, float* dx, int64_t lddx, int H, int W, int Cin, int c0, int n, void* workspace, size_t ws_bytes,
+                            const void* dy_planes, const void* w_planes, pp_stream_t stream);
 int pp_conv2d_bwd_weight_pre(const float* x, int64_t ldx, int B, int H, int W, int Cin, const float* dy, int64_t lddy,
                              int Cout, int kh, int kw, int stride, int pad, int dil, float* dw, float* dbias,
                              void* workspace, size_t ws_bytes, const void* x_planes, const void* dy_planes, pp_stream_t stream);
@@ -299,6 +303,12 @@
                     int align_corners, float scale_h, float scale_w, int dy_nchw, void* workspace, size_t ws_bytes,
                     pp_stream_t stream);
 
+size_t pp_bilinear_bwd_taps3x3_workspace_bytes(int B, int Ho, int W, int C);
+int pp_bilinear_bwd_taps3x3(const float* dy, int64_t lddy, int B, int Ho, int Wo, int C, float* g, int H, int W, int align_corners,
+                            float scale_h, float scale_w, void* workspace, size_t ws_bytes, pp_stream_t stream);
+
+int pp_tap_pack(float* w, int ntaps, int Cin, int Cout, int c0, int n, float* packed, int tap_major, int inverse, pp_stream_t stream);
+
 int pp_image_colsum(const float* x, int64_t ldx, int B, int64_t P, int C, float mul, float* out, int64_t ldo, pp_stream_t stream);
 int pp_image_broadcast(const float* v, int64_t ldv, int B, int64_t P, int C, float mul, float* y, int64_t ldy, pp_stream_t stream);
 
diff --git a/pixelpick_amd/_lib.py b/pixelpick_amd/_lib.py
--- a/pixelpick_amd/_lib.py
+++ b/pixelpick_amd/_lib.py
@@ -84,6 +84,9 @@
     "pp_x3_split_weights": (_int, [_p, _int, _int, _int, _int, _p, _sz, _p]),
     "pp_conv2d_fwd_pre2": (_int, [_p, _i64, _int, _int, _int, _int, _p, _p, _int, _int, _int, _int, _int, _p, _i64, _int, _p, _sz, _p, _p, _p]),
     "pp_conv2d_bwd_data_pre2": (_int, [_p, _i64, _int, _int, _int, _int, _p, _int, _int, _int, _int, _int, _p, _i64, _int, _int, _int, _int, _p, _sz, _p, _p, _p]),
+    "pp_conv2d_bwd_data_cols_ok": (_int, [_int] * 12),
+    "pp_conv2d_bwd_data_cols": (_int, [_p, _i64, _int, _int, _int, _int, _p, _int, _int, _int, _int, _int, _p, _i64, _int, _int, _int, _int, _int, _p, _sz,
+                                      _p, _p, _p]),
     "pp_conv2d_bwd_weight_pre": (_int, [_p, _i64, _int, _int, _int, _int, _p, _i64, _int, _int, _int, _int, _int, _int, _p, _p, _p, _sz, _p, _p, _p]),
     "pp_conv2d_bwd_weight_partials": (_int, [_p, _i64, _int, _int, _int, _int, _p, _i64, _int, _int, _int, _int, _int, _int, _p, _p, _p, _sz, _p, _p]),
     "pp_wgrad_reduce_batch": (_int, [_p, _int, _p]),
@@ -118,6 +121,9 @@
     "pp_bilinear_fwd": (_int, [_p, _i64, _int, _int, _int, _int, _p, _i64, _int, _int, _int, _f, _f, _int, _p]),
     "pp_bilinear_bwd_workspace_bytes": (_sz, [_int] * 4),
     "pp_bilinear_bwd": (_int, [_p, _i64, _int, _int, _int, _int, _p, _i64, _int, _int, _int, _f, _f, _int, _p, _sz, _p]),
+    "pp_bilinear_bwd_taps3x3_workspace_bytes": (_sz, [_int] * 4),
+    "pp_bilinear_bwd_taps3x3": (_int, [_p, _i64, _int, _int, _int, _int, _p, _int, _int, _int, _f, _f, _p, _sz, _p]),
+    "pp_tap_pack": (_int, [_p, _int, _int, _int, _int, _int, _p, _int, _int, _p]),
     "pp_image_colsum": (_int, [_p, _i64, _int, _i64, _int, _f, _p, _i64, _p]),
     "pp_image_broadcast": (_int, [_p, _i64, _int, _i64, _int, _f, _p, _i64, _p]),
     "pp_dropout": (_int, [_p, _i64, _p, _i64, _i64, _int, _f, ctypes.c_uint64, _p, _p]),
diff --git a/pixelpick_amd/csrc/conv_igemm.hip b/pixelpick_amd/csrc/conv_igemm.hip
--- a/pixelpick_amd/csrc/conv_igemm.hip
+++ b/pixelpick_amd/csrc/conv_igemm.hip
@@ -3214,7 +3214,8 @@
 }
 
 template <bool BWD>
-static int launch_conv_x3(ConvParams& p, const ConvPlan& pl, const X3Plan& x, int kh_kw, void* workspace, hipStream_t st, bool f32path)
+static int launch_conv_x3(ConvParams& p, const ConvPlan& pl, const X3Plan& x, int kh_kw, void* workspace, hipStream_t st, bool f32path,
+                          int col_lo = 0, int col_n = 0)
 {
     const uint16_t* ap = p.a_pre ? p.a_pre : reinterpret_cast<uint16_t*>(workspace);
     uint16_t* bp = reinterpret_cast<uint16_t*>(reinterpret_cast<char*>(workspace) + x.b_off);
@@ -3279,9 +3280,13 @@
             else      hipLaunchKernelGGL((conv_x3_kernel<128, 64>), grid, dim3(256), 0, st, p, o);
         }
     };
+    if (col_n > 0 && !(two && col_lo == full128 * 128 && col_n == rem))
+        return fail(PP_ERR_UNSUPPORTED, "conv: columns [%d, %d) are not a launch of their own at width %d", col_lo, col_lo + col_n, p.Cn);
     if (two) {
-        go(true, full128, 0);
-        if (int rc = check_launch("conv_x3_kernel")) return rc;
+        if (col_n == 0) {
+            go(true, full128, 0);
+            if (int rc = check_launch("conv_x3_kernel")) return rc;
+        }
         go(false, 1, full128 * 128);
     } else {
         go(n128_only, (int)cdiv(p.Cn, n128_only ? 128 : 64), 0);
@@ -3376,7 +3381,7 @@
 }
 
 template <bool BWD>
-static int launch_conv(const ConvParams& p_in, void* workspace, size_t ws_bytes, hipStream_t st, int kh_kw = 0)
+static int launch_conv(const ConvParams& p_in, void* workspace, size_t ws_bytes, hipStream_t st, int kh_kw = 0, int col_lo = 0, int col_n = 0)
 {
     EventScope ev(st);
     ConvParams p = p_in;
@@ -3436,8 +3441,9 @@
         const bool ws_ok = (workspace && ws_bytes >= x.bytes && (reinterpret_cast<uintptr_t>(workspace) & 255) == 0) ||
                            (f32path && p.b_pre != nullptr);
         if (x.ok && (f32path || x.classic) && ws_ok && (reinterpret_cast<uintptr_t>(p.b_pre) & 255) == 0)
-            return launch_conv_x3<BWD>(p, pl, x, kh_kw, workspace, st, f32path);
-    }
+            return launch_conv_x3<BWD>(p, pl, x, kh_kw, workspace, st, f32path, col_lo, col_n);
+    }
+    if (col_n > 0) return fail(PP_ERR_UNSUPPORTED, "conv: a column range needs the two-launch bf16x3 plan (ask pp_conv2d_bwd_data_cols_ok first)");
     if (pl.splits > 1 && (!workspace || ws_bytes < (size_t)pl.splits * p.M * p.Cn * 4)) {
         pl.splits = 1;
     }
@@ -4201,9 +4207,11 @@
 
 static int conv2d_bwd_data_impl(const float* dy, int64_t lddy, int B, int Ho, int Wo, int Cout, const float* w, int kh, int kw,
                                 int stride, int pad, int dil, float* dx, int64_t lddx, int H, int W, int Cin, int accumulate,
-                                void* workspace, size_t ws_bytes, pp_stream_t stream, const void* dy_planes, const void* w_planes = nullptr)
+                                void* workspace, size_t ws_bytes, pp_stream_t stream, const void* dy_planes, const void* w_planes = nullptr,
+                                int col_lo = 0, int col_n = 0)
 {
     if (int rc = conv_common_check(dy, w, dx, B, H, W, Cin, Cout, kh, kw, stride, pad, dil)) return rc;
+    if (col_n > 0 && (stride != 1 || accumulate || col_lo < 0 || col_lo + col_n > Cin)) return fail(PP_ERR_BAD_ARG, "conv bwd_data: column range");
     if (Ho != out_size(H, kh, stride, pad, dil) || Wo != out_size(W, kw, stride, pad, dil))
         return fail(PP_ERR_BAD_ARG, "conv bwd_data: inconsistent sizes");
     if (bwd_phases_apply(Cin, Cout, stride, lddx) && (int64_t)B * H * W <= 0x7FFFFFFFll) {
@@ -4248,7 +4256,33 @@
     if (p.taps.n == 0) return fail(PP_ERR_BAD_ARG, "conv bwd_data: no live tap");
     p.a_pre = stride == 1 ? reinterpret_cast<const uint16_t*>(dy_planes) : nullptr;
     p.b_pre = stride == 1 ? reinterpret_cast<const uint16_t*>(w_planes) : nullptr;
-    return launch_conv<true>(p, workspace, ws_bytes, as_stream(stream), kh * kw);
+    return launch_conv<true>(p, workspace, ws_bytes, as_stream(stream), kh * kw, col_lo, col_n);
+}
+
+int pp_conv2d_bwd_data_cols_ok(int B, int H, int W, int Cin, int Cout, int kh, int kw, int stride, int pad, int dil, int c0, int n)
+{
+    if (B < 1 || H < 1 || W < 1 || Cin < 1 || Cout < 1 || kh < 1 || kw < 1 || kh > kMaxTaps || kw > kMaxTaps || kh * kw > kMaxTaps || !conv_geom_sane(H, W, stride, pad, dil) || stride != 1 || dil < 1) return 0;
+    const int Ho = out_size(H, kh, stride, pad, dil), Wo = out_size(W, kw, stride, pad, dil);
+    if (Ho < 1 || Wo < 1) return 0;
+    ConvTaps t;
+    build_taps(t, kh, kw, 1, pad, dil, Ho, Wo, H, W, true, stride);
+    const int64_t M = (int64_t)B * H * W;
+    const bool vec = g_conv_novec == 0 && Cin % 4 == 0 && Cout % 4 == 0;
+    if (t.n == 0 || M > 0x7FFFFFFFll) return 0;
+    const ConvPlan pl = plan_conv(M, Cin, Cout, t.n, vec);
+    const X3Plan xb = x3_plan(pl, M, (int64_t)B * Ho * Wo, Cout, Cin, kh * kw, t.n, vec);
+    const int full128 = Cin / 128, rem = Cin - full128 * 128;
+    return xb.ok && xb.classic && rem > 0 && rem <= 64 && full128 > 0 && !(g_conv_x3 & 4) && c0 == full128 * 128 && n == rem ? 1 : 0;
+}
+
+int pp_conv2d_bwd_data_cols(const float* dy, int64_t lddy, int B, int Ho, int Wo, int Cout, const float* w, int kh, int kw, int stride, int pad,
+                            int dil, float* dx, int64_t lddx, int H, int W, int Cin, int c0, int n, void* workspace, size_t ws_bytes,
+                            const void* dy_planes, const void* w_planes, pp_stream_t stream)
+{
+    if (!dx || n < 1 || c0 < 0) return fail(PP_ERR_BAD_ARG, "conv bwd_data cols: null / empty range");
+    if ((c0 & 3) || (reinterpret_cast<uintptr_t>(dx) & 15) || lddx % 4 != 0) return fail(PP_ERR_BAD_ARG, "conv bwd_data cols: alignment");
+    return conv2d_bwd_data_impl(dy, lddy, B, Ho, Wo, Cout, w, kh, kw, stride, pad, dil, dx - c0, lddx, H, W, Cin, 0, workspace, ws_bytes, stream,
+                                dy_planes, w_planes, c0, n);
 }
 
 int pp_conv2d_bwd_data(const float* dy, int64_t lddy, int B, int Ho, int Wo, int Cout, const float* w, int kh, int kw,
diff --git a/pixelpick_amd/csrc/nn_ops.hip b/pixelpick_amd/csrc/nn_ops.hip
--- a/pixelpick_amd/csrc/nn_ops.hip
+++ b/pixelpick_amd/csrc/nn_ops.hip
@@ -2779,6 +2779,94 @@
     }
 }
 
+__global__ __launch_bounds__(kT) void bilinear_bwd_taps_sepw_kernel(const float* dy, int64_t lddy, int B, int Ho, int Wo, int cq,
+                                                                   float* tmp, int W, float sw, int align)
+{
+    const int64_t total = (int64_t)B * Ho * W * cq;
+    const float4 zero = make_float4(0.f, 0.f, 0.f, 0.f);
+    for (int64_t e = (int64_t)blockIdx.x * kT + threadIdx.x; e < total; e += (int64_t)gridDim.x * kT) {
+        const int q = (int)(e % cq);
+        int64_t t = e / cq;
+        const int iw = (int)(t % W);
+        const int64_t row = t / W;
+        int lo, hi;
+        out_window(iw, W, Wo, sw, align, lo, hi);
+        const float* src = dy + row * Wo * lddy + q * 4;
+        float4 acc0 = zero, acc1 = zero, acc2 = zero;
+        float4 vm = (lo >= 1 && lo <= hi) ? *reinterpret_cast<const float4*>(src + (int64_t)(lo - 1) * lddy) : zero;
+        float4 vc = lo <= hi ? *reinterpret_cast<const float4*>(src + (int64_t)lo * lddy) : zero;
+        for (int ow = lo; ow <= hi; ++ow) {
+            const bool has_p = ow + 1 < Wo;
+            const float4 vp = has_p ? *reinterpret_cast<const float4*>(src + (int64_t)(ow + 1) * lddy) : zero;
+            const Lerp l = lerp_src(ow, W, sw, align);
+            const float wgt = (l.i0 == iw ? l.l0 : 0.0f) + (l.i1 == iw ? l.l1 : 0.0f);
+            if (wgt != 0.0f) {
+                if (has_p) { acc0.x = fmaf(wgt, vp.x, acc0.x); acc0.y = fmaf(wgt, vp.y, acc0.y); acc0.z = fmaf(wgt, vp.z, acc0.z); acc0.w = fmaf(wgt, vp.w, acc0.w); }
+                acc1.x = fmaf(wgt, vc.x, acc1.x); acc1.y = fmaf(wgt, vc.y, acc1.y); acc1.z = fmaf(wgt, vc.z, acc1.z); acc1.w = fmaf(wgt, vc.w, acc1.w);
+                if (ow >= 1) { acc2.x = fmaf(wgt, vm.x, acc2.x); acc2.y = fmaf(wgt, vm.y, acc2.y); acc2.z = fmaf(wgt, vm.z, acc2.z); acc2.w = fmaf(wgt, vm.w, acc2.w); }
+            }
+            vm = vc; vc = vp;
+        }
+        *reinterpret_cast<float4*>(tmp + e * 4) = acc0;
+        *reinterpret_cast<float4*>(tmp + (total + e) * 4) = acc1;
+        *reinterpret_cast<float4*>(tmp + (2 * total + e) * 4) = acc2;
+    }
+}
+
+__global__ __launch_bounds__(kT) void bilinear_bwd_taps_seph_kernel(const float* tmp, int B, int Ho, int W, int cq, float* g, int H,
+                                                                   float sh, int align)
+{
+    const int64_t per_tw = (int64_t)B * H * W * cq, plane = (int64_t)B * Ho * W * cq * 4;
+    const int64_t total = 3 * per_tw, ldg = (int64_t)9 * cq * 4;
+    const float4 zero = make_float4(0.f, 0.f, 0.f, 0.f);
+    for (int64_t e = (int64_t)blockIdx.x * kT + threadIdx.x; e < total; e += (int64_t)gridDim.x * kT) {
+        const int tw = (int)(e / per_tw);
+        int64_t t = e - tw * per_tw;
+        const int q = (int)(t % cq); t /= cq;
+        const int iw = (int)(t % W); t /= W;
+        const int ih = (int)(t % H);
+        const int b = (int)(t / H);
+        int lo, hi;
+        out_window(ih, H, Ho, sh, align, lo, hi);
+        const float* src = tmp + tw * plane + (((int64_t)b * Ho) * W + iw) * cq * 4 + q * 4;
+        const int64_t rs = (int64_t)W * cq * 4;
+        float4 acc0 = zero, acc1 = zero, acc2 = zero;
+        float4 vm = (lo >= 1 && lo <= hi) ? *reinterpret_cast<const float4*>(src + (int64_t)(lo - 1) * rs) : zero;
+        float4 vc = lo <= hi ? *reinterpret_cast<const float4*>(src + (int64_t)lo * rs) : zero;
+        for (int oh = lo; oh <= hi; ++oh) {
+            const bool has_p = oh + 1 < Ho;
+            const float4 vp = has_p ? *reinterpret_cast<const float4*>(src + (int64_t)(oh + 1) * rs) : zero;
+            const Lerp l = lerp_src(oh, H, sh, align);
+            const float wgt = (l.i0 == ih ? l.l0 : 0.0f) + (l.i1 == ih ? l.l1 : 0.0f);
+            if (wgt != 0.0f) {
+                if (has_p) { acc0.x = fmaf(wgt, vp.x, acc0.x); acc0.y = fmaf(wgt, vp.y, acc0.y); acc0.z = fmaf(wgt, vp.z, acc0.z); acc0.w = fmaf(wgt, vp.w, acc0.w); }
+                acc1.x = fmaf(wgt, vc.x, acc1.x); acc1.y = fmaf(wgt, vc.y, acc1.y); acc1.z = fmaf(wgt, vc.z, acc1.z); acc1.w = fmaf(wgt, vc.w, acc1.w);
+                if (oh >= 1) { acc2.x = fmaf(wgt, vm.x, acc2.x); acc2.y = fmaf(wgt, vm.y, acc2.y); acc2.z = fmaf(wgt, vm.z, acc2.z); acc2.w = fmaf(wgt, vm.w, acc2.w); }
+            }
+            vm = vc; vc = vp;
+        }
+        float* dst = g + (((int64_t)b * H + ih) * W + iw) * ldg + (int64_t)tw * cq * 4 + q * 4;
+        *reinterpret_cast<float4*>(dst) = acc0;
+        *reinterpret_cast<float4*>(dst + (int64_t)3 * cq * 4) = acc1;
+        *reinterpret_cast<float4*>(dst + (int64_t)6 * cq * 4) = acc2;
+    }
+}
+
+__global__ __launch_bounds__(kT) void tap_pack_kernel(float* w, int T, int Cin, int coq, int c0, int n, float* packed, int tap_major, int inverse)
+{
+    const int64_t total = (int64_t)T * n * coq;
+    for (int64_t e = (int64_t)blockIdx.x * kT + threadIdx.x; e < total; e += (int64_t)gridDim.x * kT) {
+        const int q = (int)(e % coq);
+        int64_t r = e / coq;
+        const int ci = (int)(r % n);
+        const int t = (int)(r / n);
+        float4* pw = reinterpret_cast<float4*>(w + (((int64_t)t * Cin + c0 + ci) * coq + q) * 4);
+        float4* pk = reinterpret_cast<float4*>(packed + ((tap_major ? (int64_t)t * n + ci : (int64_t)ci * T + t) * coq + q) * 4);
+        if (inverse) *pw = *pk;
+        else         *pk = *pw;
+    }
+}
+
 static void bil_scales(int H, int W, int Ho, int Wo, int align, float scale_h, float scale_w, float& sh, float& sw)
 {
     if (align) {
@@ -2825,7 +2913,7 @@
     const bool win_ok = sh > 0.0f && sw > 0.0f && (int)(2.0f / sw) + 6 <= kMaxWin;
     const bool up2_special = !align_corners && Ho == 2 * H && Wo == 2 * W && H >= 2 && W >= 2 &&
                              (scale_h == 0.0f || scale_h == 2.0f) && (scale_w == 0.0f || scale_w == 2.0f);
-    if (!dy_nchw && C % 4 == 0 && lddy % 4 == 0 && lddx % 4 == 0 && sh > 0.0f && sw > 0.0f && Ho >= 3 * H && Wo >= 3 * W &&
+    if (!dy_nchw && C % 4 == 0 && lddy % 4 == 0 && lddx % 4 == 0 && sh > 0.0f && sw > 0.0f && Ho >= 2 * H && Wo >= 2 * W &&
         !up2_special && workspace && ws_bytes >= pp_bilinear_bwd_workspace_bytes(B, Ho, W, C) && g_bil_sep) {
         float* tmp = reinterpret_cast<float*>(workspace);
         const int cq = C / 4;
@@ -2863,6 +2951,47 @@
                            Wo, C, dx, lddx, H, W, sh, sw, align_corners);
     }
     return check_launch("bilinear_bwd_kernel");
+}
+
+size_t pp_bilinear_bwd_taps3x3_workspace_bytes(int B, int Ho, int W, int C)
+{
+    if (B < 1 || Ho < 1 || W < 1 || C < 1) return 0;
+    return align_up((size_t)3 * B * Ho * W * C * 4, 256);
+}
+
+int pp_bilinear_bwd_taps3x3(const float* dy, int64_t lddy, int B, int Ho, int Wo, int C, float* g, int H, int W, int align_corners,
+                            float scale_h, float scale_w, void* workspace, size_t ws_bytes, pp_stream_t stream)
+{
+    if (!dy || !g || !workspace) return fail(PP_ERR_BAD_ARG, "bilinear bwd taps3x3: null");
+    if (B < 1 || H < 1 || W < 1 || Ho < 1 || Wo < 1 || C < 1) return fail(PP_ERR_BAD_ARG, "bilinear bwd taps3x3: empty");
+    if (int rc = need_c4(C, "bilinear bwd taps3x3")) return rc;
+    if (lddy % 4 != 0 || lddy < C || ((reinterpret_cast<uintptr_t>(dy) | reinterpret_cast<uintptr_t>(g) | reinterpret_cast<uintptr_t>(workspace)) & 15))
+        return fail(PP_ERR_BAD_ARG, "bilinear bwd taps3x3: lddy must be a multiple of 4, dy / g / workspace 16-byte aligned");
+    if (Ho < 2 * H || Wo < 2 * W) return fail(PP_ERR_UNSUPPORTED, "bilinear bwd taps3x3: up-sampling factors >= 2 only");
+    if (ws_bytes < pp_bilinear_bwd_taps3x3_workspace_bytes(B, Ho, W, C)) return fail(PP_ERR_WORKSPACE, "bilinear bwd taps3x3: workspace");
+    float sh, sw;
+    bil_scales(H, W, Ho, Wo, align_corners, scale_h, scale_w, sh, sw);
+    if (!(sh > 0.0f && sw > 0.0f)) return fail(PP_ERR_UNSUPPORTED, "bilinear bwd taps3x3: a one-pixel source axis");
+    hipStream_t st = as_stream(stream);
+    float* tmp = reinterpret_cast<float*>(workspace);
+    const int cq = C / 4;
+    hipLaunchKernelGGL(bilinear_bwd_taps_sepw_kernel, dim3(grid_for((int64_t)B * Ho * W * cq)), dim3(kT), 0, st, dy, lddy, B, Ho, Wo, cq,
+                       tmp, W, sw, align_corners);
+    if (int rc = check_launch("bilinear_bwd_taps_sepw_kernel")) return rc;
+    hipLaunchKernelGGL(bilinear_bwd_taps_seph_kernel, dim3(grid_for((int64_t)3 * B * H * W * cq)), dim3(kT), 0, st, tmp, B, Ho, W, cq, g,
+                       H, sh, align_corners);
+    return check_launch("bilinear_bwd_taps_seph_kernel");
+}
+
+int pp_tap_pack(float* w, int ntaps, int Cin, int Cout, int c0, int n, float* packed, int tap_major, int inverse, pp_stream_t stream)
+{
+    if (!w || !packed) return fail(PP_ERR_BAD_ARG, "tap_pack: null");
+    if (ntaps < 1 || Cin < 1 || Cout < 1 || c0 < 0 || n < 1 || c0 + n > Cin) return fail(PP_ERR_BAD_ARG, "tap_pack: rows [%d, %d) of %d", c0, c0 + n, Cin);
+    if (int rc = need_c4(Cout, "tap_pack")) return rc;
+    if ((reinterpret_cast<uintptr_t>(w) | reinterpret_cast<uintptr_t>(packed)) & 15) return fail(PP_ERR_BAD_ARG, "tap_pack: 16-byte alignment");
+    hipLaunchKernelGGL(tap_pack_kernel, dim3(grid_for((int64_t)ntaps * n * (Cout / 4))), dim3(kT), 0, as_stream(stream), w, ntaps, Cin, Cout / 4,
+                       c0, n, packed, tap_major ? 1 : 0, inverse ? 1 : 0);
+    return check_launch("tap_pack_kernel");
 }
 
 int pp_image_colsum(const float* x, int64_t ldx, int B, int64_t P, int C, float mul, float* out, int64_t ldo, pp_stream_t stream)
diff --git a/pixelpick_amd/csrc/plan.hip b/pixelpick_amd/csrc/plan.hip
--- a/pixelpick_amd/csrc/plan.hip
+++ b/pixelpick_amd/csrc/plan.hip
@@ -83,6 +83,7 @@
     PP_PLAN_ENTRY(pp_conv2d_bwd_data_multi),
     PP_PLAN_ENTRY(pp_conv2d_fwd_pre2),
     PP_PLAN_ENTRY(pp_conv2d_bwd_data_pre2),
+    PP_PLAN_ENTRY(pp_conv2d_bwd_data_cols),
     PP_PLAN_ENTRY(pp_x3_split_weights),
     PP_PLAN_ENTRY(pp_conv2d_bwd_weight_pre),
     PP_PLAN_ENTRY(pp_conv2d_bwd_weight_partials),
@@ -110,6 +111,8 @@
     PP_PLAN_ENTRY(pp_crop2d_add),
     PP_PLAN_ENTRY(pp_bilinear_fwd),
     PP_PLAN_ENTRY(pp_bilinear_bwd),
+    PP_PLAN_ENTRY(pp_bilinear_bwd_taps3x3),
+    PP_PLAN_ENTRY(pp_tap_pack),
     PP_PLAN_ENTRY(pp_image_colsum),
     PP_PLAN_ENTRY(pp_image_broadcast),
     PP_PLAN_ENTRY(pp_dropout),
diff --git a/pixelpick_amd/engine.py b/pixelpick_amd/engine.py
--- a/pixelpick_amd/engine.py
+++ b/pixelpick_amd/engine.py
@@ -216,6 +216,7 @@
         self._side_rr = 0
         self._keepalive = []
         self.hooks = {}
+        self._tail_jobs = []
         self._jobs_first = 0
         self._jobs_next = 0
         self._arena_off = 0
@@ -295,6 +296,11 @@
         self._jobs_first = self._jobs_next
         self._arena_off = 0
 
+    def run_tail_jobs(self):
+        jobs, self._tail_jobs = self._tail_jobs, []
+        for job in jobs:
+            job()
+
     def backward(self, out: Var, dout: torch.Tensor):
         refresh_stream()
         if Tape.trace is not None:
@@ -302,6 +308,7 @@
         out.grad = dout
         for fn, ctx, o in reversed(self.nodes):
             if fn is _MARK:
+                self.run_tail_jobs()
                 hook = self.hooks.get(ctx)
                 if hook is not None:
                     self.flush_reduces(dout.device)
@@ -312,6 +319,7 @@
             fn(self, o.grad, *ctx)
             o.grad = None
         self.nodes = []
+        self.run_tail_jobs()
         self.flush_reduces(dout.device)
         if Tape.trace is not None:
             Tape.trace.append(("bwd_main_end", _mark()))
@@ -757,7 +765,7 @@
 
 
 def conv2d(tape: Tape, x: Var, w: torch.Tensor, bias: Optional[torch.Tensor], stride=1, pad=0, dil=1,
-           dst: Optional[torch.Tensor] = None, bwd_group=None) -> Var:
+           dst: Optional[torch.Tensor] = None, bwd_group=None, upcat=None, wgrad_to_tail: bool = False) -> Var:
     B, H, W, Cin = shape_of(x)
     kh, kw, wcin, Cout = w.shape
     assert wcin == Cin, f"conv2d: Cin {Cin} vs weight {tuple(w.shape)}"
@@ -771,7 +779,7 @@
         out._pending = ("conv", x, w, bias, stride, pad, dil)
         if bwd_group is not None:
             out._grad_dst = bwd_group[0].slice(bwd_group[1])
-        tape.record(_conv2d_bwd, (x, w, bias, stride, pad, dil, None, bwd_group), out)
+        tape.record(_conv2d_bwd, (x, w, bias, stride, pad, dil, None, bwd_group, upcat, wgrad_to_tail), out)
         return out
     _, _, _, _, ldx = _geom(x.t)
     Ho, Wo = out_size(H, kh, stride, pad, dil), out_size(W, kw, stride, pad, dil)
@@ -794,11 +802,106 @@
     out = Var(y)
     if bwd_group is not None and tape.enabled:
         out._grad_dst = bwd_group[0].slice(bwd_group[1])
-    tape.record(_conv2d_bwd, (x, w, bias, stride, pad, dil, xp, bwd_group), out)
+    tape.record(_conv2d_bwd, (x, w, bias, stride, pad, dil, xp, bwd_group, upcat, wgrad_to_tail), out)
     return out
 
 
-def _conv2d_bwd(tape: Tape, dy: torch.Tensor, x: Var, w, bias, stride, pad, dil, xp=None, bwd_group=None):
+_HEAD_LOWRES_BWD = os.environ.get("PIXELPICK_HEAD_LOWRES_BWD", "0") != "0"
+_HEAD_WGRAD_TAIL = os.environ.get("PIXELPICK_HEAD_WGRAD_TAIL", "1") != "0"
+
+
+def _upcat_lowres_ok(dy, x: Var, w, bias, stride, pad, dil, bwd_group, upcat) -> bool:
+    if not _HEAD_LOWRES_BWD or upcat is None or bwd_group is not None or bias is not None:
+        return False
+    a, other = upcat[0], upcat[1]
+    if tuple(w.shape[:2]) != (3, 3) or (stride, pad, dil) != (1, 1, 1) or not (w.requires_grad and a.needs_grad):
+        return False
+    if x._t is None or x._bn_bwd_ctx is not None or a._t is None or not a._t.is_contiguous():
+        return False
+    B, H, W, Cin = x._t.shape
+    Ba, h, wl, Ca = a._t.shape
+    Co = other._t.shape[3] if other._t is not None else -1
+    Cout = w.shape[3]
+    return (Ba == B and Ca + Co == Cin and H >= 2 * h and W >= 2 * wl and h >= 2 and wl >= 2 and Ca % 4 == 0 and Co % 4 == 0 and Cout % 4 == 0
+            and Co > 0 and _geom(dy)[4] % 4 == 0 and not ((dy.data_ptr() | w.data_ptr() | x._t.data_ptr()) & 15))
+
+
+def _conv_upcat_bwd(tape: Tape, dy: torch.Tensor, x: Var, w, upcat):
+    L = _lib.lib()
+    a, other, align, scale = upcat[:4]
+    B, H, W, Cin, ldx = _geom(x.t)
+    _, _, _, Cout, lddy = _geom(dy)
+    _, h, wl, Ca, _ = _geom(a.t)
+    Co = Cin - Ca
+    dev = dy.device
+    geom = (B, H, W, Cin, Cout, 3, 3, 1, 1, 1)
+    cols = other.needs_grad and bool(_wsbytes("pp_conv2d_bwd_data_cols_ok", *geom, Ca, Co))
+    dyp = _x3_split(dy, lddy, B * H * W, Cout) if (cols and _x3_planes(1, *geom)) else None
+    G = torch.empty((B, h, wl, 9 * Cout), dtype=torch.float32, device=dev)
+    ws = _ws(_wsbytes("pp_bilinear_bwd_taps3x3_workspace_bytes", B, H, wl, Cout), dev)
+    rc = L.pp_bilinear_bwd_taps3x3(dy.data_ptr(), lddy, B, H, W, Cout, G.data_ptr(), h, wl, int(align), float(scale), float(scale),
+                                   ws.data_ptr(), ws.numel(), _stream())
+    _lib.check(rc, "pp_bilinear_bwd_taps3x3")
+    def _issue_wgrads():
+        dw = tape.grad_buffer_for(w)
+        dwa = torch.empty((Ca, 9 * Cout), dtype=torch.float32, device=dev)
+        dwo = torch.empty((9, Co, Cout), dtype=torch.float32, device=dev)
+        with tape.side_stream_for(x.t, a.t, dy, G, dw, dwa, dwo):
+            st = _stream()
+            nws = _wsbytes("pp_conv2d_bwd_weight_workspace_bytes", B, h, wl, Ca, 9 * Cout, 1, 1, 1, 0, 1)
+            ws = _ws(nws, dev)
+            rc = L.pp_conv2d_bwd_weight(a.t.data_ptr(), Ca, B, h, wl, Ca, G.data_ptr(), 9 * Cout, 9 * Cout, 1, 1, 1, 0, 1, dwa.data_ptr(), None,
+                                        ws.data_ptr(), ws.numel(), st)
+            _lib.check(rc, "pp_conv2d_bwd_weight")
+            _lib.check(L.pp_tap_pack(dw.data_ptr(), 9, Cin, Cout, 0, Ca, dwa.data_ptr(), 0, 1, st), "pp_tap_pack")
+            nws = _wsbytes("pp_conv2d_bwd_weight_workspace_bytes", B, H, W, Co, Cout, 3, 3, 1, 1, 1)
+            ws = _ws(nws, dev)
+            rc = L.pp_conv2d_bwd_weight(x.t.data_ptr() + 4 * Ca, ldx, B, H, W, Co, dy.data_ptr(), lddy, Cout, 3, 3, 1, 1, 1, dwo.data_ptr(), None,
+                                        ws.data_ptr(), ws.numel(), st)
+            _lib.check(rc, "pp_conv2d_bwd_weight")
+            _lib.check(L.pp_tap_pack(dw.data_ptr(), 9, Cin, Cout, Ca, Co, dwo.data_ptr(), 1, 1, st), "pp_tap_pack")
+        tape.set_param_grad(w, dw)
+
+    wpk = _tap_packed(w, Ca)
+    acc_into = a.grad if (a.grad is not None and getattr(a.grad, "_pp_owned", False) and a.grad.is_contiguous()
+                          and tuple(a.grad.shape) == (B, h, wl, Ca)) else None
+    da = acc_into if acc_into is not None else torch.empty((B, h, wl, Ca), dtype=torch.float32, device=dev)
+    cws, cwsn = _conv_ws(True, dev, B, h, wl, Ca, 9 * Cout, 1, 1, 1, 0, 1)
+    rc = L.pp_conv2d_bwd_data(G.data_ptr(), 9 * Cout, B, h, wl, 9 * Cout, wpk.data_ptr(), 1, 1, 1, 0, 1, da.data_ptr(), Ca, h, wl, Ca,
+                              1 if acc_into is not None else 0, cws, cwsn, _stream())
+    _lib.check(rc, "pp_conv2d_bwd_data")
+    tape._keepalive.append(wpk)
+    if acc_into is None:
+        da._pp_owned = True
+        _acc(a, da)
+    if not other.needs_grad:
+        _issue_wgrads()
+        return
+    cws, cwsn = _conv_ws(True, dev, *geom)
+    if cols:
+        dother = torch.empty((B, H, W, Co), dtype=torch.float32, device=dev)
+        wp = _weight_planes(w, 0)
+        _register_weight_planes(w, 0)
+        if dyp is not None:
+            tape._keepalive.append(dyp)
+        rc = L.pp_conv2d_bwd_data_cols(dy.data_ptr(), lddy, B, H, W, Cout, w.data_ptr(), 3, 3, 1, 1, 1, dother.data_ptr(), Co, H, W, Cin, Ca, Co,
+                                       cws, cwsn, dyp.data_ptr() if dyp is not None else None, wp, _stream())
+        _lib.check(rc, "pp_conv2d_bwd_data_cols")
+    else:
+        dx = torch.empty((B, H, W, Cin), dtype=torch.float32, device=dev)
+        rc = L.pp_conv2d_bwd_data(dy.data_ptr(), lddy, B, H, W, Cout, w.data_ptr(), 3, 3, 1, 1, 1, dx.data_ptr(), Cin, H, W, Cin, 0, cws, cwsn,
+                                  _stream())
+        _lib.check(rc, "pp_conv2d_bwd_data")
+        dother = dx[..., Ca:]
+    _acc(other, dother)
+    _issue_wgrads()
+
+
+def _conv2d_bwd(tape: Tape, dy: torch.Tensor, x: Var, w, bias, stride, pad, dil, xp=None, bwd_group=None, upcat=None, to_tail=False):
+    if _upcat_lowres_ok(dy, x, w, bias, stride, pad, dil, bwd_group, upcat):
+        _conv_upcat_bwd(tape, dy, x, w, upcat)
+        tape.run_tail_jobs()
+        return
     L = _lib.lib()
     lazy_in = x._lazy if (x._t is None and x._lazy is not None) else None
     B, H, W, Cin, ldx = _geom(lazy_in[0] if lazy_in is not None else x.t)
@@ -812,6 +915,10 @@
             and _x3_planes(2, B, H, W, Cin, Cout, kh, kw, stride, pad, dil)):
         dyp = _x3_split(dy, lddy, B * Ho * Wo, Cout)
     big = _BIG_WGRAD_MAIN and 2.0 * B * Ho * Wo * Cin * Cout * kh * kw >= _BIG_WGRAD_FLOP
+    tail = big and upcat is not None and len(upcat) > 4 and upcat[4] and _HEAD_WGRAD_TAIL and x.needs_grad and bwd_group is None
+    held = big and to_tail and not tail and _HEAD_WGRAD_TAIL and w.requires_grad and x.needs_grad and bwd_group is None
+    if tail or held:
+        big = False
 
     def _issue_wgrad():
         dw = tape.grad_buffer_for(w)
@@ -918,13 +1025,18 @@
             _issue_wgrad()
         bwd_group[0].arrive(tape, bwd_group[1], dy)
         return
-    if w.requires_grad and (big or not _WGRAD_LATE):
+    if held:
+        _issue_dx()
+        tape._tail_jobs.append(_issue_wgrad)
+    elif w.requires_grad and (big or not _WGRAD_LATE) and not tail:
         _issue_wgrad()
         _issue_dx()
     else:
         _issue_dx()
         if w.requires_grad:
             _issue_wgrad()
+        if tail:
+            tape.run_tail_jobs()
 
 
 def dwconv3x3(tape: Tape, x: Var, w: torch.Tensor, stride=1, pad=0, dil=1) -> Var:
@@ -1437,7 +1549,7 @@
     if _dropout_seed_dev[0] is not None:
         _dropout_counter[0] = 0
     _STEP_EPOCH[0] += 1
-    if _X3_WPRE and _X3_WPL:
+    if _X3_WPRE and (_X3_WPL or _TAP_PACKS):
         _prefetch_weight_planes()
 
 
@@ -1449,6 +1561,7 @@
 _STEP_EPOCH = [0]
 _X3_WPL = {}
 _X3_WPL_EVENT = {}
+_TAP_PACKS = {}
 
 
 def _register_weight_planes(w: torch.Tensor, transpose: int):
@@ -1476,6 +1589,12 @@
         if ent.get("used", -10) < _STEP_EPOCH[0] - 3:
             continue
         by_dev.setdefault(w.device, []).append((ent, w))
+    for key, ent in list(_TAP_PACKS.items()):
+        w = ent["w"]()
+        if w is None or not w.is_cuda:
+            del _TAP_PACKS[key]
+        elif ent.get("used", -10) >= _STEP_EPOCH[0] - 3:
+            by_dev.setdefault(w.device, []).append((ent, w))
     for dev, ents in by_dev.items():
         main = _main_stream_obj()
         side = _side_stream(dev, 0)
@@ -1484,6 +1603,10 @@
         _lib.plan_note(side.wait_event, ev)
         for ent, w in ents:
             kh, kw, Cin, Cout = w.shape
+            if "buf" in ent:
+                _lib.check(L.pp_tap_pack(w.data_ptr(), kh * kw, Cin, Cout, 0, ent["ca"], ent["buf"].data_ptr(), 0, 0, side.cuda_stream), "pp_tap_pack")
+                ent["epoch"] = _STEP_EPOCH[0]
+                continue
             for tr, planes in ent["planes"].items():
                 _lib.check(L.pp_x3_split_weights(w.data_ptr(), kh * kw, Cin, Cout, tr, planes.data_ptr(), planes.numel(), side.cuda_stream),
                            "pp_x3_split_weights")
@@ -1508,6 +1631,24 @@
         _lib.plan_note(_main_stream_obj().wait_event, rec[0])
         rec[2] = _STEP_EPOCH[0]
     return ent["planes"][transpose].data_ptr()
+
+
+def _tap_packed(w: torch.Tensor, ca: int) -> torch.Tensor:
+    kh, kw, Cin, Cout = w.shape
+    ent = _TAP_PACKS.get(id(w))
+    if ent is None or ent["w"]() is not w or ent["ca"] != ca:
+        ent = _TAP_PACKS[id(w)] = {"w": weakref.ref(w), "ca": ca, "epoch": -1,
+                                   "buf": torch.empty((ca, kh * kw * Cout), dtype=torch.float32, device=w.device)}
+    ent["used"] = _STEP_EPOCH[0]
+    rec = _X3_WPL_EVENT.get((w.device.type, w.device.index))
+    if _X3_WPRE and ent["epoch"] == _STEP_EPOCH[0] and rec is not None and rec[1] == _STEP_EPOCH[0]:
+        if rec[2] != _STEP_EPOCH[0]:
+            _lib.plan_note(_main_stream_obj().wait_event, rec[0])
+            rec[2] = _STEP_EPOCH[0]
+        return ent["buf"]
+    buf = torch.empty((ca, kh * kw * Cout), dtype=torch.float32, device=w.device)
+    _lib.check(_lib.lib().pp_tap_pack(w.data_ptr(), kh * kw, Cin, Cout, 0, ca, buf.data_ptr(), 0, 0, _stream()), "pp_tap_pack")
+    return buf
 
 
 def dropout(tape: Tape, x: Var, p: float, training: bool) -> Var:
diff --git a/pixelpick_amd/networks/decoders.py b/pixelpick_amd/networks/decoders.py
--- a/pixelpick_amd/networks/decoders.py
+++ b/pixelpick_amd/networks/decoders.py
@@ -107,9 +107,10 @@
         self.classifier = Conv2d(256, args.n_classes, 1)
         self.n_classes = args.n_classes
 
-    def run(self, tape, x):
+    def run(self, tape, x, upcat=None):
         s = self.segment_head
-        h = s[1].run(tape, s[0].run(tape, x), E.ACT_RELU, dropout=s[3])
-        emb = s[5].run(tape, s[4].run(tape, h), E.ACT_RELU, dropout=s[7])
+        h = s[1].run(tape, s[0].run(tape, x, upcat=upcat), E.ACT_RELU, dropout=s[3])
+        last_big = upcat is not None and len(upcat) > 4 and bool(upcat[4])
+        emb = s[5].run(tape, s[4].run(tape, h, wgrad_to_tail=last_big), E.ACT_RELU, dropout=s[7])
         pred = self.classifier.run(tape, emb)
         return {"emb": emb, "pred": pred}
diff --git a/pixelpick_amd/networks/deeplab.py b/pixelpick_amd/networks/deeplab.py
--- a/pixelpick_amd/networks/deeplab.py
+++ b/pixelpick_amd/networks/deeplab.py
@@ -107,7 +107,7 @@
         llc = self.low_level_conv
         low_ = llc[1].run(tape, llc[0].run(tape, low), E.ACT_RELU, dst=cat_buf[..., 256:304])
         cat = E.concat_alias(tape, cat_buf, [up, low_])
-        outs = self.seg_head.run(tape, cat)
+        outs = self.seg_head.run(tape, cat, upcat=(a, low_, True, 0.0, not self._resnet))
         if not upsample:
             return outs["pred"], outs["emb"]
         pred = E.bilinear(tape, outs["pred"], (H, W), True, 0.0, out_nchw=True)
diff --git a/pixelpick_amd/networks/layers.py b/pixelpick_amd/networks/layers.py
--- a/pixelpick_amd/networks/layers.py
+++ b/pixelpick_amd/networks/layers.py
@@ -82,10 +82,11 @@
         k = self.kernel_size
         return E.conv_accepts_lazy_input(B, H, W, C, self.out_channels, k, k, self.stride, self.padding + extra_pad, self.dilation)
 
-    def run(self, tape, x, dst=None, extra_pad: int = 0, bwd_group=None):
+    def run(self, tape, x, dst=None, extra_pad: int = 0, bwd_group=None, upcat=None, wgrad_to_tail=False):
         if self.depthwise:
             return E.dwconv3x3(tape, x, self.weight, self.stride, self.padding + extra_pad, self.dilation)
-        return E.conv2d(tape, x, self.weight, self.bias, self.stride, self.padding + extra_pad, self.dilation, dst=dst, bwd_group=bwd_group)
+        return E.conv2d(tape, x, self.weight, self.bias, self.stride, self.padding + extra_pad, self.dilation, dst=dst, bwd_group=bwd_group,
+                        upcat=upcat, wgrad_to_tail=wgrad_to_tail)
 
     def forward(self, x):
         raise RuntimeError("pixelpick_amd layers execute through run(tape, x); call the network's forward()")
```

Result: no change. 758.4 images/s (-0.7%).
